# MachinaIO/mxx

Measured on AMD Instinct MI355X. Metric: dcrt_ring_ops_per_s, higher is better.
Workload: dtype u32

## Files before the change

include/gpupoly.h:

```cpp
#ifndef GPUPOLY_H
#define GPUPOLY_H

#include <stddef.h>
#include <stdint.h>

#ifdef __cplusplus
extern "C" {
#endif

typedef struct GpuContext GpuContext;
typedef struct GpuMatrix GpuMatrix;
typedef struct GpuEventSet GpuEventSet;
typedef struct GpuP1CovarianceCache GpuP1CovarianceCache;
typedef struct GpuComm GpuComm;

typedef struct GpuRngSeed {
    uint64_t words[4];
} GpuRngSeed;

#define GPU_POLY_FORMAT_COEFF 0
#define GPU_POLY_FORMAT_EVAL 1
#define GPU_MATRIX_DIST_UNIFORM 0
#define GPU_MATRIX_DIST_GAUSS 1
#define GPU_MATRIX_DIST_BIT 2
// ... 119 lines not shown
int gpupoly_matrix_decompose_rows(const GpuMatrix *src, uint32_t base_bits, int small, size_t row_start, GpuMatrix *out);
int gpupoly_matrix_sample_decomposed_window(GpuMatrix *out, int dist_type, double sigma, GpuRngSeed seed,
                                            uint32_t base_bits, int small, size_t src_rows, size_t full_ncol,
                                            size_t col_offset, size_t row_start);
int gpupoly_timer_start(GpuContext *ctx);
int gpupoly_timer_stop(GpuContext *ctx, float *out_ms);
int gpupoly_timer_mark(GpuContext *ctx, uint32_t slot);
int gpupoly_timer_elapsed(GpuContext *ctx, uint32_t slot_begin, uint32_t slot_end, float *out_ms);
int gpupoly_matrix_device_ptr(const GpuMatrix *mat, void **out_ptr, size_t *out_bytes);
int gpupoly_matrix_layout(const GpuMatrix *mat, int *out);
int gpupoly_matrix_copy_to_context(GpuContext *dst_ctx, const GpuMatrix *src, GpuMatrix **out);
int gpupoly_context_device(const GpuContext *ctx, int *out_device);
int gpupoly_context_word_bytes(const GpuContext *ctx, int *out_bytes);
const char *gpupoly_context_last_kernel(const GpuContext *ctx);
int gpupoly_context_stream(const GpuContext *ctx, void **out_stream);
int gpupoly_comm_create(GpuContext *const *ctxs, size_t n, GpuComm **out_comm);
void gpupoly_comm_destroy(GpuComm *comm);
int gpupoly_comm_size(const GpuComm *comm, int *out_size);
const char *gpupoly_comm_backend(const GpuComm *comm);
int gpupoly_matrix_all_gather_columns(GpuComm *comm, const GpuMatrix *const *local_blocks, GpuMatrix *const *full);
int gpupoly_matrix_sample_distribution_segments(GpuMatrix *out, int dist_type, double sigma, const GpuRngSeed *seeds,
                                                const size_t *seg_cols, size_t nseg);
int gpupoly_matrix_sample_p1_full_cached_segments(const GpuP1CovarianceCache *cache, const GpuMatrix *tp2,
                                                  const GpuRngSeed *seeds, const size_t *seg_cols, size_t nseg,
                                                  GpuMatrix *out);
int gpupoly_matrix_gauss_samp_gq_arb_base_segments(GpuMatrix *src, uint32_t base_bits, double c, double dgg_stddev,
                                                   const GpuRngSeed *seeds, const size_t *seg_cols, size_t nseg,
                                                   GpuMatrix *out);
#define GPUPOLY_BLOCKS_STACKED 0
#define GPUPOLY_BLOCKS_COLUMNS 1
int gpupoly_matrix_sample_distribution_blocks(GpuMatrix *out, int dist_type, const GpuRngSeed *seeds, size_t nblk,
                                              int layout, const size_t *seg_cols);
#define GPUPOLY_HASH_KECCAK256 0
#define GPUPOLY_HASH_SHA3_256 1
#define GPUPOLY_TAGS_TABLE 0
#define GPUPOLY_TAGS_INDEXED_LE64 1
#define GPUPOLY_TAGS_INDEXED_DECIMAL 2
typedef struct GpuHashTags {
    int hash;
    int form;
    uint8_t key[32];
    const uint8_t *tags;
    const size_t *tag_offsets;
    size_t prefix_len;
    uint64_t first_index;
} GpuHashTags;
int gpupoly_hash_seeds(GpuContext *ctx, const GpuHashTags *tags, size_t ntags, GpuRngSeed *seeds_out);
int gpupoly_matrix_sample_hash_blocks(GpuMatrix *out, int dist_type, const GpuHashTags *tags, size_t nblk, int layout,
                                      const size_t *seg_cols);
int gpupoly_matrix_sample_gauss_blocks(GpuMatrix *out, double sigma, const GpuRngSeed *seeds, size_t nblk, int layout,
                                       const size_t *seg_cols);
int gpupoly_matrix_sample_hash_gauss_blocks(GpuMatrix *out, double sigma, const GpuHashTags *tags, size_t nblk, int layout,
                                            const size_t *seg_cols);
int gpupoly_matrix_concat_columns(GpuMatrix *out, const GpuMatrix *const *blocks, size_t n);
int gpupoly_matrix_split_columns(const GpuMatrix *src, GpuMatrix *const *blocks, size_t n);
int gpupoly_trapdoor_preimage_many(const GpuMatrix *re, const GpuP1CovarianceCache *cache, const GpuMatrix *public_matrix,
                                   uint32_t base_bits, const GpuMatrix *const *targets, size_t n, const GpuRngSeed *seeds,
                                   GpuMatrix *const *outs);
int gpupoly_trapdoor_preimage_keyed(const GpuMatrix *const *res, const GpuP1CovarianceCache *const *caches,
                                    const GpuMatrix *const *public_matrices, size_t nkeys, uint32_t base_bits,
                                    const uint32_t *key_of, const GpuMatrix *const *targets, size_t n,
                                    const GpuRngSeed *seeds, GpuMatrix *const *outs);
int gpupoly_matrix_sample_decomposed_blocks(GpuMatrix *out, int dist_type, const GpuRngSeed *seeds, size_t nblk,
                                            uint32_t base_bits, int small, size_t src_rows, size_t full_ncol,
                                            size_t col_offset);
int gpupoly_matrix_sample_hash_decomposed_blocks(GpuMatrix *out, int dist_type, const GpuHashTags *tags, size_t nblk,
                                                 uint32_t base_bits, int small, size_t src_rows, size_t full_ncol,
                                                 size_t col_offset);
int gpupoly_matrix_lut_targets(GpuMatrix *const *outs, size_t nrows_T, const GpuMatrix *w_identity, const GpuMatrix *w_gy,
                               const GpuMatrix *w_v, const GpuMatrix *w_vx, size_t col_start, uint32_t base_bits,
                               const uint64_t *y_words, size_t words_per_y, const uint64_t *idx, const GpuHashTags *tags);
int gpupoly_matrix_lut_targets_combine(GpuMatrix *const *outs, size_t nrows_T, const GpuMatrix *w_identity,
                                       const GpuMatrix *w_gy, const GpuMatrix *product, size_t col_start, uint32_t base_bits,
                                       const uint64_t *y_words, size_t words_per_y, const uint64_t *idx);
int gpupoly_matrix_lwe_targets(GpuMatrix *const *outs, size_t nrows_T, const GpuMatrix *a_z, const GpuMatrix *a_lt,
                               size_t col_start, uint32_t base_bits, const uint64_t *y_words, size_t words_per_y,
                               const uint64_t *x, const GpuHashTags *tags);
int gpupoly_matrix_lwe_targets_combine(GpuMatrix *const *outs, size_t nrows_T, const GpuMatrix *a_lt,
                                       const GpuMatrix *digits, const GpuMatrix *product, size_t col_start,
                                       uint32_t base_bits, const uint64_t *y_words, size_t words_per_y, const uint64_t *x);
int gpupoly_matrix_wee25_targets(GpuMatrix *const *outs, size_t nblocks_T, size_t nparts_P, const GpuMatrix *t_bottom,
                                 size_t part_start, size_t secret_size, uint32_t base_bits, const uint64_t *idx,
                                 const GpuHashTags *tags);
int gpupoly_matrix_wee25_targets_product(GpuMatrix *const *outs, size_t nblocks_T, size_t nparts_P, const GpuMatrix *w_stacked,
                                         const GpuMatrix *t_bottom, size_t part_start, size_t secret_size,
                                         uint32_t base_bits, const uint64_t *idx);
int gpupoly_matrix_ggh15_lookup(GpuMatrix *const *outs, size_t nslots_S, const GpuMatrix *mid_identity,
                                const GpuMatrix *mid_gy, const GpuMatrix *mid_v, const GpuMatrix *mid_vx,
                                const GpuMatrix *mid_rand, const GpuMatrix *mid_gate1,
                                const GpuMatrix *const *lut_preimages, const GpuMatrix *const *xs, size_t col_start,
                                uint32_t base_bits, const uint64_t *y_words, size_t words_per_y, const GpuHashTags *tags);
int gpupoly_matrix_ggh15_lookup_combine(GpuMatrix *const *outs, size_t nslots_S, const GpuMatrix *mid_identity,
                                        const GpuMatrix *mid_gy, const GpuMatrix *mid_v, const GpuMatrix *mid_vx,
                                        const GpuMatrix *mid_rand, const GpuMatrix *mid_gate1,
                                        const GpuMatrix *const *lut_preimages, const GpuMatrix *const *xs, size_t col_start,
                                        uint32_t base_bits, const uint64_t *y_words, size_t words_per_y,
                                        const GpuMatrix *digits);
int gpupoly_matrix_lwe_lookup(GpuMatrix *const *outs, size_t nslots_S, size_t dst_col, const GpuMatrix *const *c_bs,
                              const GpuMatrix *const *k_highs, const GpuMatrix *const *c_zs, size_t col_start,
                              uint32_t base_bits, const GpuHashTags *tags);
int gpupoly_matrix_lwe_lookup_combine(GpuMatrix *const *outs, size_t nslots_S, size_t dst_col,
                                      const GpuMatrix *const *c_bs, const GpuMatrix *const *k_highs,
                                      const GpuMatrix *const *c_zs, size_t col_start, uint32_t base_bits,
                                      const GpuMatrix *digits);
typedef struct {
    const GpuMatrix *c_in;
    const GpuMatrix *mid;
    uint64_t shift;
    uint64_t scalar;
} GpuSlotTerm;
int gpupoly_matrix_slot_transfer_eval(GpuMatrix *const *outs, size_t nouts_S, size_t dst_col, const GpuMatrix *c_b0,
                                      const GpuMatrix *const *gate_preimages, const GpuMatrix *const *b1_preimages,
                                      const GpuSlotTerm *terms, const size_t *term_offsets, const uint64_t *mu_words,
                                      size_t words_per_mu, size_t col_start, uint32_t base_bits, const GpuHashTags *tags);
int gpupoly_matrix_slot_transfer_eval_combine(GpuMatrix *const *outs, size_t nouts_S, size_t dst_col, const GpuMatrix *c_b0,
                                              const GpuMatrix *const *gate_preimages,
                                              const GpuMatrix *const *b1_preimages, const GpuSlotTerm *terms,
                                              const size_t *term_offsets, const uint64_t *mu_words, size_t words_per_mu,
                                              size_t col_start, uint32_t base_bits, const GpuMatrix *digits);
int gpupoly_matrix_bgg_encode_slots(GpuMatrix *const *outs, size_t ninputs_P, const GpuMatrix *secrets,
                                    const GpuMatrix *const *pubkeys, const GpuMatrix *plaintexts, uint32_t base_bits,
                                    double sigma, const GpuRngSeed *seeds);
int gpupoly_matrix_bgg_encode_slots_combine(GpuMatrix *const *outs, size_t ninputs_P, const GpuMatrix *secrets,
                                            const GpuMatrix *const *pubkeys, const GpuMatrix *plaintexts,
                                            uint32_t base_bits, const GpuMatrix *errors);
int gpupoly_matrix_scale_round(GpuMatrix *out, const GpuMatrix *in, uint64_t t, int round_half);
int gpupoly_matrix_crt_recompose_rounded(GpuMatrix *out, const GpuMatrix *const *terms, const int *signs,
                                         size_t terms_per_level, size_t num_slots);
int gpupoly_matrix_nested_rns_decompose(GpuMatrix *out, const GpuMatrix *src, const uint64_t *p_moduli, size_t p_count,
                                        uint64_t scale, size_t level_offset, size_t active_levels, int out_format);
int gpupoly_matrix_fill_nested_rns_gadget(GpuMatrix *out, const uint64_t *p_moduli, size_t p_count, uint64_t scale,
                                          size_t level_offset, size_t active_levels, int out_format);
int gpupoly_matrix_nested_rns_residues(GpuMatrix *out, const GpuMatrix *src, const uint64_t *p_moduli, size_t p_count,
                                       size_t level_offset, size_t active_levels);
int gpupoly_matrix_store_coeff_words(const GpuMatrix *mat, uint64_t *out, size_t words_per_coeff);
int gpupoly_matrix_load_coeff_words(GpuMatrix *mat, const uint64_t *words, size_t words_per_coeff, size_t coeffs_per_poly,
                                    int out_format);
int gpupoly_matrix_centered_max_abs(const GpuMatrix *mat, uint64_t *out, size_t words_per_value);
int gpupoly_matrix_extract_bits(const GpuMatrix *mat, const uint64_t *lo, const uint64_t *hi, size_t words_per_bound,
                                uint8_t *out, size_t bytes_per_poly);
int gpupoly_matrix_store_coeff_ints(const GpuMatrix *mat, void *out, int elem_bytes, int centred, size_t coeffs_per_poly,
                                    uint64_t *out_misfit_count, uint64_t *out_first_misfit);
int gpupoly_matrix_store_compact_bytes_many(GpuMatrix *const *mats, size_t n, uint8_t *payload_out, size_t payload_capacity,
                                            uint16_t *out_max_coeff_bits, uint16_t *out_bytes_per_coeff,
                                            size_t *out_payload_offsets, size_t *out_payload_lens, size_t *out_total_len);
int gpupoly_matrix_load_compact_bytes_many(GpuMatrix *const *mats, size_t n, const uint8_t *const *payloads,
                                           const size_t *payload_lens, const uint16_t *max_coeff_bits);
int gpupoly_matrix_fill_monomial(GpuMatrix *out, uint64_t shift, int format);
int gpupoly_matrix_mul_monomial(GpuMatrix *out, const GpuMatrix *in, uint64_t shift);
int gpupoly_matrix_monomial_sum(GpuMatrix *out, const GpuMatrix *addend, const GpuMatrix *const *mats,
                                const uint64_t *shifts, size_t n, int negate);
int gpupoly_matrix_mul_sum(GpuMatrix *out, size_t dst_col, size_t cols, const GpuMatrix *addend,
                           const GpuMatrix *const *lhss, const GpuMatrix *const *rhss, size_t n, int negate);
int gpupoly_matrix_mul_acc(GpuMatrix *out, const GpuMatrix *lhs, const GpuMatrix *rhs, int negate);
int gpupoly_matrix_mul_gadget(GpuMatrix *out, size_t dst_col, const GpuMatrix *lhs, const GpuMatrix *scalar_1x1,
                              size_t gadget_col, size_t cols, const GpuMatrix *addend, int negate, uint32_t base_bits,
                              int small);
int gpupoly_matrix_gadget_mul(GpuMatrix *out, const GpuMatrix *rhs, const GpuMatrix *addend, int negate,
                              uint32_t base_bits, int small);
int gpupoly_matrix_mul_decompose_gadget_scalar_many(GpuMatrix *const *outs, const GpuMatrix *const *lhss,
                                                    const GpuMatrix *const *addends, size_t n, const GpuMatrix *scalar_1x1,
                                                    int negate, uint32_t base_bits);
int gpupoly_matrix_mul_decompose_gadget_const_many(GpuMatrix *const *outs, const GpuMatrix *const *lhss,
                                                   const GpuMatrix *const *addends, size_t n, const uint64_t *const_words,
                                                   size_t words_per_const, int negate, uint32_t base_bits);
uint64_t gpupoly_launch_count(void);
int gpupoly_detmath_eval(GpuContext *ctx, int fn, const double *host_in, double *host_out, size_t n);
int gpupoly_device_can_access_peer(int device, int peer, int *out_can);
int gpupoly_marker_launch(GpuContext *ctx, uint32_t id);
int gpupoly_trace_begin(void);
const char *gpupoly_trace_end(void);
const char *gpupoly_version(void);
int gpupoly_reload_env(void);

#ifdef __cplusplus
}
#endif
#endif
```

mxx_amd/_ffi.py:

```python
from __future__ import annotations

import ctypes as C
import os

_HERE = os.path.dirname(os.path.abspath(__file__))
LIB_PATH = os.environ.get("MXX_GPUPOLY_LIB") or os.path.join(_HERE, "libgpupoly.so")

GPU_POLY_FORMAT_COEFF = 0
GPU_POLY_FORMAT_EVAL = 1
GPU_MATRIX_DIST_UNIFORM = 0
GPU_MATRIX_DIST_GAUSS = 1
GPU_MATRIX_DIST_BIT = 2
GPU_MATRIX_DIST_TERNARY = 3
GPUPOLY_BLOCKS_STACKED = 0
GPUPOLY_BLOCKS_COLUMNS = 1
GPUPOLY_HASH_KECCAK256 = 0
GPUPOLY_HASH_SHA3_256 = 1
GPUPOLY_TAGS_TABLE = 0
GPUPOLY_TAGS_INDEXED_LE64 = 1
GPUPOLY_TAGS_INDEXED_DECIMAL = 2


class GpuPolyError(RuntimeError):
    """Raised where the reference's Rust wrapper panics (`check_status`, gpu.rs:259-263)."""
# ... 28 lines not shown


class GpuBatchOp(C.Structure):

    _fields_ = [("kind", C.c_int), ("out", C.c_void_p), ("lhs", C.c_void_p), ("rhs", C.c_void_p)]


GPUPOLY_OP_MUL, GPUPOLY_OP_ADD, GPUPOLY_OP_SUB, GPUPOLY_OP_MUL_SCALAR, GPUPOLY_OP_NEG, GPUPOLY_OP_DECOMPOSE, GPUPOLY_OP_MUL_DECOMPOSE = range(7)

_vp = C.c_void_p
_sz = C.c_size_t
_u8p = C.POINTER(C.c_uint8)

SIGNATURES = {
    "gpu_context_create": (C.c_int, [C.c_uint32, C.c_uint32, C.c_uint32, C.POINTER(C.c_uint64), _sz, C.POINTER(C.c_int), _sz, C.POINTER(_vp)]),
    "gpu_context_destroy": (None, [_vp]),
    "gpu_context_get_N": (C.c_int, [_vp, C.POINTER(C.c_int)]),
    "gpu_event_set_wait": (C.c_int, [_vp]),
    "gpu_event_set_destroy": (None, [_vp]),
    "gpu_device_count": (C.c_int, [C.POINTER(C.c_int)]),
    "gpu_device_mem_info": (C.c_int, [C.c_int, C.POINTER(_sz), C.POINTER(_sz)]),
    "gpu_device_synchronize": (C.c_int, []),
    "gpu_device_reset": (C.c_int, []),
    "gpu_last_error": (C.c_char_p, []),
    "gpu_set_last_error": (C.c_int, [C.c_char_p]),
    "gpu_pinned_alloc": (_vp, [_sz]),
    "gpu_pinned_free": (None, [_vp]),
    "gpu_matrix_create": (C.c_int, [_vp, C.c_int, _sz, _sz, C.c_int, C.POINTER(_vp)]),
    "gpu_matrix_destroy": (None, [_vp]),
    "gpu_matrix_copy": (C.c_int, [_vp, _vp]),
    "gpu_matrix_copy_block": (C.c_int, [_vp, _vp, _sz, _sz, _sz, _sz, _sz, _sz]),
    "gpu_matrix_add": (C.c_int, [_vp, _vp, _vp]),
    "gpu_matrix_sub": (C.c_int, [_vp, _vp, _vp]),
    "gpu_matrix_add_block": (C.c_int, [_vp, _vp, _sz, _sz, _sz, _sz, _sz, _sz]),
    "gpu_matrix_mul": (C.c_int, [_vp, _vp, _vp]),
    "gpu_matrix_mul_scalar": (C.c_int, [_vp, _vp, _vp]),
    "gpu_matrix_equal": (C.c_int, [_vp, _vp, C.POINTER(C.c_int)]),
    "gpu_matrix_ntt_all": (C.c_int, [_vp]),
    "gpu_matrix_intt_all": (C.c_int, [_vp]),
    "gpu_matrix_fill_gadget": (C.c_int, [_vp, C.c_uint32]),
    "gpu_matrix_fill_small_gadget": (C.c_int, [_vp, C.c_uint32]),
    "gpu_matrix_fill_small_decomposed_identity_chunk": (C.c_int, [_vp, _vp, _sz]),
    "gpu_matrix_decompose_base": (C.c_int, [_vp, C.c_uint32, _vp]),
    "gpu_matrix_decompose_base_small": (C.c_int, [_vp, C.c_uint32, _vp]),
    "gpu_matrix_sample_distribution": (C.c_int, [_vp, C.c_int, C.c_double, GpuRngSeed]),
    "gpu_matrix_sample_distribution_columns": (C.c_int, [_vp, C.c_int, C.c_double, GpuRngSeed, _sz, _sz]),
    "gpu_matrix_gauss_samp_gq_arb_base": (C.c_int, [_vp, C.c_uint32, C.c_double, C.c_double, GpuRngSeed, _vp]),
    "gpu_matrix_sample_p1_full": (C.c_int, [_vp, _vp, _vp, _vp, C.c_double, C.c_double, C.c_double, GpuRngSeed, _vp]),
    "gpu_matrix_create_p1_covariance_cache": (C.c_int, [_vp, _vp, _vp, C.c_double, C.c_double, C.c_double, C.POINTER(_vp)]),
    "gpu_matrix_destroy_p1_covariance_cache": (None, [_vp]),
    "gpu_matrix_sample_p1_full_cached": (C.c_int, [_vp, _vp, GpuRngSeed, _vp]),
    "gpu_matrix_load_rns_batch": (C.c_int, [_vp, _vp, _sz, C.c_int, C.POINTER(_vp)]),
    "gpu_matrix_store_rns_batch": (C.c_int, [_vp, _vp, _sz, C.c_int, C.POINTER(_vp)]),
    "gpu_matrix_store_const_coeff_batch": (C.c_int, [_vp, _vp, _sz, C.POINTER(_vp)]),
    "gpu_matrix_store_compact_bytes": (C.c_int, [_vp, _vp, _sz, C.POINTER(C.c_uint16), C.POINTER(C.c_uint16), C.POINTER(_sz)]),
    "gpu_matrix_load_compact_bytes": (C.c_int, [_vp, _vp, _sz, C.c_uint16]),
    "gpu_poly_store_compact_bytes": (C.c_int, [_vp, _vp, _sz, C.POINTER(C.c_uint16), C.POINTER(C.c_uint16), C.POINTER(_sz)]),
    "gpu_poly_load_compact_bytes": (C.c_int, [_vp, _vp, _sz, C.c_uint16]),
    "gpupoly_matrix_mul_decompose": (C.c_int, [_vp, _vp, _vp, C.c_uint32]),
    "gpupoly_matrix_mul_decompose_many": (C.c_int, [C.POINTER(C.c_void_p), C.POINTER(C.c_void_p), C.POINTER(C.c_void_p), C.POINTER(C.c_void_p), C.c_size_t, _vp, C.c_uint32]),
    "gpupoly_matrix_mul_decompose_pairs": (C.c_int, [C.POINTER(C.c_void_p), C.POINTER(C.c_void_p), C.POINTER(C.c_void_p), C.POINTER(C.c_void_p), C.POINTER(C.c_void_p), _sz, _sz, C.c_uint32, C.c_int]),
    "gpupoly_matrix_mul_batch":(C.c_int, [C.POINTER(C.c_void_p), C.POINTER(C.c_void_p), C.POINTER(C.c_void_p), C.c_size_t]),
    "gpupoly_batch": (C.c_int, [C.POINTER(GpuBatchOp), C.c_size_t, C.c_uint32]),
    "gpupoly_matrix_mul_decompose_small": (C.c_int, [_vp, _vp, _vp, C.c_uint32]),
    "gpupoly_matrix_mul_tensor_identity": (C.c_int, [_vp, _vp, _vp, C.c_size_t]),
    "gpupoly_matrix_mul_tensor_identity_decompose": (C.c_int, [_vp, _vp, _vp, C.c_size_t, C.c_uint32]),
    "gpupoly_matrix_mul_scalar_intt": (C.c_int, [_vp, _vp, _vp]),
    "gpupoly_matrix_transpose": (C.c_int, [_vp, _vp]),
    "gpupoly_matrix_tensor": (C.c_int, [_vp, _vp, _vp]),
    "gpupoly_matrix_add_rows": (C.c_int, [_vp, C.c_size_t, _vp, _vp]),
    "gpupoly_matrix_ntt_add_rows": (C.c_int, [_vp, C.c_size_t, _vp, _vp, C.c_int]),
    "gpupoly_matrix_row_view": (C.c_int, [_vp, C.c_size_t, C.c_size_t, C.POINTER(C.c_void_p)]),
    "gpupoly_matrix_reshape_view": (C.c_int, [_vp, C.c_size_t, C.c_size_t, C.POINTER(C.c_void_p)]),
    "gpupoly_matrix_neg": (C.c_int, [_vp, _vp]),
    "gpupoly_matrix_fill_zero": (C.c_int, [_vp]),
    "gpupoly_matrix_fill_identity": (C.c_int, [_vp, _vp]),
    "gpupoly_matrix_sample_decomposed": (C.c_int, [_vp, C.c_int, C.c_double, GpuRngSeed, C.c_uint32, C.c_int]),
    "gpupoly_matrix_decompose_rows": (C.c_int, [_vp, C.c_uint32, C.c_int, _sz, _vp]),
    "gpupoly_matrix_sample_decomposed_window": (C.c_int, [_vp, C.c_int, C.c_double, GpuRngSeed, C.c_uint32, C.c_int, _sz, _sz, _sz, _sz]),
    "gpupoly_timer_start": (C.c_int, [_vp]),
    "gpupoly_timer_stop": (C.c_int, [_vp, C.POINTER(C.c_float)]),
    "gpupoly_timer_mark": (C.c_int, [_vp, C.c_uint32]),
    "gpupoly_timer_elapsed": (C.c_int, [_vp, C.c_uint32, C.c_uint32, C.POINTER(C.c_float)]),
    "gpupoly_matrix_device_ptr": (C.c_int, [_vp, C.POINTER(_vp), C.POINTER(_sz)]),
    "gpupoly_matrix_layout": (C.c_int, [_vp, C.POINTER(C.c_int)]),
    "gpupoly_matrix_copy_to_context": (C.c_int, [_vp, _vp, C.POINTER(_vp)]),
    "gpupoly_context_device": (C.c_int, [_vp, C.POINTER(C.c_int)]),
    "gpupoly_context_word_bytes": (C.c_int, [_vp, C.POINTER(C.c_int)]),
    "gpupoly_context_last_kernel": (C.c_char_p, [_vp]),
    "gpupoly_context_stream": (C.c_int, [_vp, C.POINTER(C.c_void_p)]),
    "gpupoly_comm_create": (C.c_int, [C.POINTER(C.c_void_p), C.c_size_t, C.POINTER(_vp)]),
    "gpupoly_comm_destroy": (None, [_vp]),
    "gpupoly_comm_size": (C.c_int, [_vp, C.POINTER(C.c_int)]),
    "gpupoly_comm_backend": (C.c_char_p, [_vp]),
    "gpupoly_matrix_all_gather_columns": (C.c_int, [_vp, C.POINTER(C.c_void_p), C.POINTER(C.c_void_p)]),
    "gpupoly_matrix_sample_distribution_segments": (C.c_int, [_vp, C.c_int, C.c_double, C.POINTER(GpuRngSeed), C.POINTER(_sz), _sz]),
    "gpupoly_matrix_sample_distribution_blocks": (C.c_int, [_vp, C.c_int, C.POINTER(GpuRngSeed), _sz, C.c_int, C.POINTER(_sz)]),
    "gpupoly_hash_seeds": (C.c_int, [_vp, C.POINTER(GpuHashTags), _sz, C.POINTER(GpuRngSeed)]),
    "gpupoly_matrix_sample_hash_blocks": (C.c_int, [_vp, C.c_int, C.POINTER(GpuHashTags), _sz, C.c_int, C.POINTER(_sz)]),
    "gpupoly_matrix_sample_gauss_blocks": (C.c_int, [_vp, C.c_double, C.POINTER(GpuRngSeed), _sz, C.c_int, C.POINTER(_sz)]),
    "gpupoly_matrix_sample_hash_gauss_blocks": (C.c_int, [_vp, C.c_double, C.POINTER(GpuHashTags), _sz, C.c_int, C.POINTER(_sz)]),
    "gpupoly_matrix_sample_decomposed_blocks": (C.c_int, [_vp, C.c_int, C.POINTER(GpuRngSeed), _sz, C.c_uint32, C.c_int, _sz, _sz, _sz]),
    "gpupoly_matrix_sample_hash_decomposed_blocks": (C.c_int, [_vp, C.c_int, C.POINTER(GpuHashTags), _sz, C.c_uint32, C.c_int, _sz, _sz, _sz]),
    "gpupoly_matrix_lut_targets": (C.c_int, [C.POINTER(C.c_void_p), _sz, _vp, _vp, _vp, _vp, _sz, C.c_uint32, C.POINTER(C.c_uint64), _sz,
                                   C.POINTER(C.c_uint64), C.POINTER(GpuHashTags)]),
    "gpupoly_matrix_lut_targets_combine": (C.c_int, [C.POINTER(C.c_void_p), _sz, _vp, _vp, _vp, _sz, C.c_uint32, C.POINTER(C.c_uint64), _sz,
                                           C.POINTER(C.c_uint64)]),
    "gpupoly_matrix_lwe_targets": (C.c_int, [C.POINTER(C.c_void_p), _sz, _vp, _vp, _sz, C.c_uint32, C.POINTER(C.c_uint64), _sz,
                                   C.POINTER(C.c_uint64), C.POINTER(GpuHashTags)]),
    "gpupoly_matrix_lwe_targets_combine": (C.c_int, [C.POINTER(C.c_void_p), _sz, _vp, _vp, _vp, _sz, C.c_uint32, C.POINTER(C.c_uint64), _sz,
                                           C.POINTER(C.c_uint64)]),
    "gpupoly_matrix_wee25_targets": (C.c_int, [C.POINTER(C.c_void_p), _sz, _sz, _vp, _sz, _sz, C.c_uint32, C.POINTER(C.c_uint64),
                                     C.POINTER(GpuHashTags)]),
    "gpupoly_matrix_wee25_targets_product": (C.c_int, [C.POINTER(C.c_void_p), _sz, _sz, _vp, _vp, _sz, _sz, C.c_uint32,
                                             C.POINTER(C.c_uint64)]),
    "gpupoly_matrix_ggh15_lookup": (C.c_int, [C.POINTER(C.c_void_p), _sz, _vp, _vp, _vp, _vp, _vp, _vp, C.POINTER(C.c_void_p),
                                    C.POINTER(C.c_void_p), _sz, C.c_uint32, C.POINTER(C.c_uint64), _sz, C.POINTER(GpuHashTags)]),
    "gpupoly_matrix_ggh15_lookup_combine": (C.c_int, [C.POINTER(C.c_void_p), _sz, _vp, _vp, _vp, _vp, _vp, _vp, C.POINTER(C.c_void_p),
                                            C.POINTER(C.c_void_p), _sz, C.c_uint32, C.POINTER(C.c_uint64), _sz, _vp]),
    "gpupoly_matrix_lwe_lookup": (C.c_int, [C.POINTER(C.c_void_p), _sz, _sz, C.POINTER(C.c_void_p), C.POINTER(C.c_void_p), C.POINTER(C.c_void_p),
                                  _sz, C.c_uint32, C.POINTER(GpuHashTags)]),
    "gpupoly_matrix_lwe_lookup_combine": (C.c_int, [C.POINTER(C.c_void_p), _sz, _sz, C.POINTER(C.c_void_p), C.POINTER(C.c_void_p),
                                          C.POINTER(C.c_void_p), _sz, C.c_uint32, _vp]),
    "gpupoly_matrix_slot_transfer_eval": (C.c_int, [C.POINTER(C.c_void_p), _sz, _sz, _vp, C.POINTER(C.c_void_p), C.POINTER(C.c_void_p),
                                          C.POINTER(GpuSlotTerm), C.POINTER(_sz), C.POINTER(C.c_uint64), _sz, _sz, C.c_uint32,
                                          C.POINTER(GpuHashTags)]),
    "gpupoly_matrix_slot_transfer_eval_combine": (C.c_int, [C.POINTER(C.c_void_p), _sz, _sz, _vp, C.POINTER(C.c_void_p), C.POINTER(C.c_void_p),
                                                  C.POINTER(GpuSlotTerm), C.POINTER(_sz), C.POINTER(C.c_uint64), _sz, _sz, C.c_uint32, _vp]),
    "gpupoly_matrix_bgg_encode_slots": (C.c_int, [C.POINTER(C.c_void_p), _sz, _vp, C.POINTER(C.c_void_p), _vp, C.c_uint32, C.c_double,
                                        C.POINTER(GpuRngSeed)]),
    "gpupoly_matrix_bgg_encode_slots_combine": (C.c_int, [C.POINTER(C.c_void_p), _sz, _vp, C.POINTER(C.c_void_p), _vp, C.c_uint32, _vp]),
    "gpupoly_matrix_sample_p1_full_cached_segments":(C.c_int, [_vp, _vp, C.POINTER(GpuRngSeed), C.POINTER(_sz), _sz, _vp]),
    "gpupoly_matrix_gauss_samp_gq_arb_base_segments": (C.c_int, [_vp, C.c_uint32, C.c_double, C.c_double, C.POINTER(GpuRngSeed), C.POINTER(_sz), _sz, _vp]),
    "gpupoly_matrix_concat_columns": (C.c_int, [_vp, C.POINTER(C.c_void_p), _sz]),
    "gpupoly_matrix_split_columns": (C.c_int, [_vp, C.POINTER(C.c_void_p), _sz]),
    "gpupoly_trapdoor_preimage_many": (C.c_int, [_vp, _vp, _vp, C.c_uint32, C.POINTER(C.c_void_p), _sz, C.POINTER(GpuRngSeed), C.POINTER(C.c_void_p)]),
    "gpupoly_trapdoor_preimage_keyed": (C.c_int, [C.POINTER(C.c_void_p), C.POINTER(C.c_void_p), C.POINTER(C.c_void_p), _sz, C.c_uint32,
                                        C.POINTER(C.c_uint32), C.POINTER(C.c_void_p), _sz, C.POINTER(GpuRngSeed), C.POINTER(C.c_void_p)]),
    "gpupoly_launch_count": (C.c_uint64, []),
    "gpupoly_matrix_scale_round": (C.c_int, [_vp, _vp, C.c_uint64, C.c_int]),
    "gpupoly_matrix_crt_recompose_rounded": (C.c_int, [_vp, C.POINTER(C.c_void_p), C.POINTER(C.c_int), _sz, _sz]),
    "gpupoly_matrix_nested_rns_decompose": (C.c_int, [_vp, _vp, C.POINTER(C.c_uint64), _sz, C.c_uint64, _sz, _sz, C.c_int]),
    "gpupoly_matrix_fill_nested_rns_gadget": (C.c_int, [_vp, C.POINTER(C.c_uint64), _sz, C.c_uint64, _sz, _sz, C.c_int]),
    "gpupoly_matrix_nested_rns_residues": (C.c_int, [_vp, _vp, C.POINTER(C.c_uint64), _sz, _sz, _sz]),
    "gpupoly_matrix_store_coeff_words": (C.c_int, [_vp, C.POINTER(C.c_uint64), _sz]),
    "gpupoly_matrix_load_coeff_words": (C.c_int, [_vp, C.POINTER(C.c_uint64), _sz, _sz, C.c_int]),
    "gpupoly_matrix_centered_max_abs": (C.c_int, [_vp, C.POINTER(C.c_uint64), _sz]),
    "gpupoly_matrix_extract_bits": (C.c_int, [_vp, C.POINTER(C.c_uint64), C.POINTER(C.c_uint64), _sz, _u8p, _sz]),
    "gpupoly_matrix_store_coeff_ints": (C.c_int, [_vp, _vp, C.c_int, C.c_int, _sz, C.POINTER(C.c_uint64), C.POINTER(C.c_uint64)]),
    "gpupoly_matrix_fill_monomial": (C.c_int, [_vp, C.c_uint64, C.c_int]),
    "gpupoly_matrix_mul_monomial": (C.c_int, [_vp, _vp, C.c_uint64]),
    "gpupoly_matrix_monomial_sum": (C.c_int, [_vp, _vp, C.POINTER(C.c_void_p), C.POINTER(C.c_uint64), _sz, C.c_int]),
    "gpupoly_matrix_mul_sum": (C.c_int, [_vp, _sz, _sz, _vp, C.POINTER(C.c_void_p), C.POINTER(C.c_void_p), _sz, C.c_int]),
    "gpupoly_matrix_mul_acc": (C.c_int, [_vp, _vp, _vp, C.c_int]),
    "gpupoly_matrix_mul_gadget": (C.c_int, [_vp, _sz, _vp, _vp, _sz, _sz, _vp, C.c_int, C.c_uint32, C.c_int]),
    "gpupoly_matrix_gadget_mul": (C.c_int, [_vp, _vp, _vp, C.c_int, C.c_uint32, C.c_int]),
    "gpupoly_matrix_mul_decompose_gadget_scalar_many": (C.c_int, [C.POINTER(C.c_void_p), C.POINTER(C.c_void_p), C.POINTER(C.c_void_p), _sz, _vp, C.c_int, C.c_uint32]),
    "gpupoly_matrix_mul_decompose_gadget_const_many": (C.c_int, [C.POINTER(C.c_void_p), C.POINTER(C.c_void_p), C.POINTER(C.c_void_p), _sz, C.POINTER(C.c_uint64), _sz, C.c_int, C.c_uint32]),
    "gpupoly_matrix_store_compact_bytes_many": (C.c_int, [C.POINTER(C.c_void_p), _sz, _vp, _sz, C.POINTER(C.c_uint16), C.POINTER(C.c_uint16), C.POINTER(_sz), C.POINTER(_sz), C.POINTER(_sz)]),
    "gpupoly_matrix_load_compact_bytes_many": (C.c_int, [C.POINTER(C.c_void_p), _sz, C.POINTER(C.c_void_p), C.POINTER(_sz), C.POINTER(C.c_uint16)]),
    "gpupoly_detmath_eval": (C.c_int, [_vp, C.c_int, C.POINTER(C.c_double), C.POINTER(C.c_double), _sz]),
    "gpupoly_device_can_access_peer": (C.c_int, [C.c_int, C.c_int, C.POINTER(C.c_int)]),
    "gpupoly_marker_launch": (C.c_int, [_vp, C.c_uint32]),
    "gpupoly_trace_begin": (C.c_int, []),
    "gpupoly_trace_end": (C.c_char_p, []),
    "gpupoly_version": (C.c_char_p, []),
    "gpupoly_reload_env": (C.c_int, []),
}

_lib = None


def lib() -> C.CDLL:
    global _lib
    if _lib is None:
        if not os.path.exists(LIB_PATH):
            raise GpuPolyError(
                f"{LIB_PATH} is missing: build it with `python -c 'import __graft_entry__ as g; g.build()'` "
                "(or `make -C mxx_amd/csrc`). mxx_amd has no CPU fallback."
            )
        handle = C.CDLL(LIB_PATH)
        for name, (res, args) in SIGNATURES.items():
            fn = getattr(handle, name)
            fn.restype = res
            fn.argtypes = args
        _lib = handle
    return _lib


def last_error_string() -> str:
    msg = lib().gpu_last_error()
    return msg.decode("utf-8", "replace") if msg else "unknown GPU error"


def check_status(code: int, context: str) -> None:
    if code != 0:
        raise GpuPolyError(f"{context} failed: {last_error_string()}")


def reload_env() -> None:
    check_status(lib().gpupoly_reload_env(), "gpupoly_reload_env")


def trace_begin() -> None:
    check_status(lib().gpupoly_trace_begin(), "gpupoly_trace_begin")


def trace_end() -> list[dict]:
    text = lib().gpupoly_trace_end()
    if text is None:
        raise GpuPolyError(f"gpupoly_trace_end failed: {last_error_string()}")
    out = []
    for ln in text.decode().splitlines():
        name, blocks, threads, nbytes, ms = ln.split("\t")
        out.append({"kernel": name.strip("()"), "blocks": int(blocks), "threads": int(threads), "bytes": float(nbytes), "ms": float(ms)})
    return out


def gpu_device_sync() -> None:
    check_status(lib().gpu_device_synchronize(), "gpu_device_synchronize")


def detected_gpu_device_ids() -> list[int]:
    n = C.c_int(0)
    if lib().gpu_device_count(C.byref(n)) != 0 or n.value <= 0:
        return []
    return list(range(n.value))


def peer_access_matrix(devices=None) -> list[list[int]]:
    devs = detected_gpu_device_ids() if devices is None else list(devices)
    out = []
    for a in devs:
        row = []
        for b in devs:
            can = C.c_int(0)
            check_status(lib().gpupoly_device_can_access_peer(a, b, C.byref(can)), "gpupoly_device_can_access_peer")
            row.append(int(can.value))
        out.append(row)
    return out


def detected_gpu_device_count() -> int:
    return len(detected_gpu_device_ids())


def wait_and_destroy_events(events: _vp) -> None:
    if events:
        st = lib().gpu_event_set_wait(events)
        lib().gpu_event_set_destroy(events)
        check_status(st, "gpu_event_set_wait")
```

mxx_amd/csrc/common.h:

```cpp
#pragma once

#include <hip/hip_runtime.h>

#include <atomic>
#include <cstddef>
#include <cstdint>
#include <cstdio>
#include <exception>
#include <map>
#include <unordered_map>
#include <mutex>
#include <string>
#include <vector>

#include "../../include/gpupoly.h"
#include "grid_plan.h"

constexpr size_t GPUPOLY_MAX_LIMBS = 64;

struct LimbConst {
    uint64_t q;
    uint64_t mu;
    uint64_t mu64;
    uint64_t n_inv;
    uint64_t n_inv_sh;
    uint64_t mu32;
    uint64_t inv_last_w;
    uint64_t inv_last_w_sh;
    uint32_t kbits;
    uint32_t lazy_terms;
};

struct EnvSwitches {
    int ntt_path = 0;
    int ntt14 = 0;
    bool decompose_fused = true;
    char matmul_path = 0;
    int matmul_tile = 0;
    bool gsamp_simple = false;
    bool gsamp_no_uni = false;
    bool p1_simple = false;
    int sampler_per_lane = 0;
    int sampler_fill_every = 0;
    bool ntt64_int = false;
    int ntt_phase = 0;
    bool serde_general = false;
    bool rng_compat = false;
    bool pack24 = true;
    int skinny24 = 0;
    int skinny24_shape = 0;
    size_t mul_decompose_many_budget = 0;
    size_t mul_decompose_pairs_budget = 0;
    size_t gadget_scalar_budget = 0;
    size_t ggh15_lookup_budget = 0;
    size_t lwe_lookup_budget = 0;
    size_t slot_eval_budget = 0;
    size_t bgg_encode_budget = 0;
    char mul_sum_path = 0;
    size_t crt_recompose_chunk_bytes = size_t(256) << 20;
    void load();
};

struct GpuContext {
    EnvSwitches env;
    int device = 0;
    std::vector<int> gpu_ids;
    uint32_t logN = 0;
    int N = 0;
    int level = 0;
    uint32_t dnum = 0;
    int limb_count = 0;
    bool wide = false;
    int word_bytes = 4;
    uint32_t crt_bits = 0;
    std::vector<uint64_t> moduli;
    hipStream_t stream = nullptr;
    LimbConst *d_limbs = nullptr;
    LimbConst *d_limbs_r = nullptr;
    void *d_tw_fwd = nullptr;
    void *d_tw_fwd_sh = nullptr;
    void *d_tw_inv = nullptr;
    void *d_tw_inv_sh = nullptr;
    void *d_tw2_fwd = nullptr;
    void *d_tw2_inv = nullptr;
    bool lazy_ok = false;
    bool tight_ok = false;
    void *d_tw2s_inv = nullptr;
    bool signed_ok = false;
    void *d_twf_fwd = nullptr, *d_twf_inv = nullptr;
    void *d_flimbs = nullptr;
    bool f64_ok = false;
    uint64_t *d_garner = nullptr;
    std::vector<uint64_t> garner_inv;
    std::vector<LimbConst> limbs;
    hipEvent_t timer_start = nullptr, timer_stop = nullptr;
    std::vector<hipEvent_t> marks;
    std::mutex mutex;
    bool pool_ok = false;
    std::mutex alloc_mutex;
    std::multimap<size_t, void *> free_blocks;
    std::unordered_map<void *, size_t> live_blocks;
    size_t cached_bytes = 0, cache_limit = 0;
    std::atomic<const char *> last_kernel{""};
    bool pack24_ok = false;
    std::mutex layout_mutex;
    std::map<uint32_t, void *> gadget_weights;
    std::map<std::vector<uint64_t>, void *> gadget_const_tables;
    std::map<std::vector<uint64_t>, void *> nested_rns_tables;
};

struct LayoutTag {
    std::atomic<int> v{GPU_MATRIX_LAYOUT_WORDS};
    LayoutTag() = default;
    LayoutTag(const LayoutTag &o) : v(o.v.load(std::memory_order_acquire)) {}
    LayoutTag &operator=(const LayoutTag &o) {
        v.store(o.v.load(std::memory_order_acquire), std::memory_order_release);
        return *this;
    }
};

struct GpuMatrix {
    GpuContext *ctx = nullptr;
    int level = 0;
    size_t rows = 0, cols = 0;
    int format = GPU_POLY_FORMAT_EVAL;
    void *storage = nullptr;
    size_t bytes = 0;
    LayoutTag layout;
    bool borrowed = false;
    GpuMatrix *parent = nullptr;
    int views = 0;
};

struct GpuEventSet {
    std::vector<hipEvent_t> events;
    int device = 0;
    void *staging = nullptr;
    GpuContext *ctx = nullptr;
    void *dev_staging = nullptr;
};

struct GpuP1CovarianceCache {
    GpuContext *ctx = nullptr;
    int level = 0;
    size_t d = 0, m = 0, n = 0;
    double sigma = 0, s = 0, dgg_stddev = 0;
    double *sqrt_var = nullptr;
    double *update_coeff = nullptr;
    void *karney_div = nullptr;
};

struct P1KeyEntry {
    const double *sqrt_var;
    const double *update_coeff;
    const void *karney_div;
};

#if defined(__HIPCC__)
__device__ __forceinline__ size_t item_index() {
    return (static_cast<size_t>(blockIdx.y) * gridDim.x + blockIdx.x) * blockDim.x + threadIdx.x;
}
#endif

extern std::atomic<uint64_t> g_kernel_launches;
extern std::atomic<int> g_trace_on;
void trace_launch_begin(const char *name, hipStream_t stream, dim3 grid, dim3 block);
void trace_launch_end(hipStream_t stream);
void trace_set_bytes(double bytes);
#define MXX_TRACE_BYTES(b)                                                                        \
    do {                                                                                          \
        if (g_trace_on.load(std::memory_order_relaxed)) trace_set_bytes(static_cast<double>(b)); \
    } while (0)
#define MXX_LAUNCH(kern, grid, block, lds, strm, ...)                          \
    do {                                                                       \
        g_kernel_launches.fetch_add(1, std::memory_order_relaxed);             \
        const bool mxx_tr_ = g_trace_on.load(std::memory_order_relaxed) != 0;  \
        if (mxx_tr_) trace_launch_begin(#kern, strm, grid, block);             \
        hipLaunchKernelGGL(kern, grid, block, lds, strm, __VA_ARGS__);         \
        if (mxx_tr_) trace_launch_end(strm);                                   \
    } while (0)
#define MXX_TRACED_COPY(name, strm, bytes, stmt)                               \
    do {                                                                       \
        const bool mxx_tr_ = g_trace_on.load(std::memory_order_relaxed) != 0;  \
        if (mxx_tr_) {                                                         \
            trace_set_bytes(static_cast<double>(bytes));                       \
            trace_launch_begin(name, strm, dim3(0), dim3(0));                  \
        }                                                                      \
        stmt;                                                                  \
        if (mxx_tr_) trace_launch_end(strm);                                   \
    } while (0)

int set_error(const char *msg);
int set_error(const std::string &msg);
int set_error(hipError_t err, const char *what);

#define HIP_TRY(expr)                                          \
    do {                                                       \
        hipError_t _e = (expr);                                \
        if (_e != hipSuccess) return set_error(_e, #expr);     \
    } while (0)

template <auto... KERNELS>
static int lds_opt_in(const GpuContext *ctx, size_t lds) {
    static std::atomic<uint64_t> configured{0};
    const uint64_t bit = 1ull << (ctx->device & 63);
    if (lds <= 64 * 1024 || (configured.load() & bit)) return 0;
    for (const void *f : {reinterpret_cast<const void *>(KERNELS)...})
        HIP_TRY(hipFuncSetAttribute(f, hipFuncAttributeMaxDynamicSharedMemorySize, static_cast<int>(lds)));
    configured.fetch_or(bit);
    return 0;
}

extern int (*g_roctx_push)(const char *);
extern int (*g_roctx_pop)();
void roctx_init_once();
struct RoctxScope {
    bool on;
    explicit RoctxScope(const char *name) {
        roctx_init_once();
        on = g_roctx_push != nullptr;
        if (on) g_roctx_push(name);
    }
    ~RoctxScope() {
        if (on) g_roctx_pop();
    }
};

#define ABI_GUARD_BEGIN try { RoctxScope roctx_scope_(__func__);
#define ABI_GUARD_END                                                         \
    }                                                                         \
    catch (const std::exception &e) { return set_error(e.what()); }           \
    catch (...) { return set_error("unknown exception in libgpupoly"); }

inline size_t matrix_polys(const GpuMatrix *m) { return m->rows * m->cols; }
inline size_t matrix_limbs(const GpuMatrix *m) { return static_cast<size_t>(m->level) + 1; }
inline size_t matrix_words(const GpuMatrix *m) { return matrix_polys(m) * matrix_limbs(m) * static_cast<size_t>(m->ctx->N); }

void *words_ptr(const GpuMatrix *m);
const void *packed24_ptr(const GpuMatrix *m, bool *packed);
inline size_t packed24_bytes(const GpuMatrix *m) { return m->bytes / 4 * 3; }
inline bool storage_overlaps(const GpuMatrix *x, const GpuMatrix *y) {
    if (x == y) return true;
    if (!x->storage || !y->storage || x->bytes == 0 || y->bytes == 0) return false;
    const size_t xb = x->layout.v.load(std::memory_order_acquire) == GPU_MATRIX_LAYOUT_PACKED24 ? packed24_bytes(x) : x->bytes;
    const size_t yb = y->layout.v.load(std::memory_order_acquire) == GPU_MATRIX_LAYOUT_PACKED24 ? packed24_bytes(y) : y->bytes;
    const char *xs = static_cast<const char *>(x->storage), *ys = static_cast<const char *>(y->storage);
    return xs < ys + yb && ys < xs + xb;
}
inline bool same_block(const GpuMatrix *x, const GpuMatrix *y) {
    return x == y || (x->storage == y->storage && x->bytes == y->bytes);
}
inline bool partial_overlap(const GpuMatrix *out, const GpuMatrix *operand) {
    return storage_overlaps(out, operand) && !same_block(out, operand);
}
inline bool row_block_overlaps(const GpuMatrix *m, size_t row, size_t rows, const GpuMatrix *y) {
    if (m->layout.v.load(std::memory_order_acquire) == GPU_MATRIX_LAYOUT_PACKED24) return rows && m->cols && storage_overlaps(m, y);
    if (!m->storage) return false;
    const size_t poly_bytes = matrix_limbs(m) * static_cast<size_t>(m->ctx->N) * m->ctx->word_bytes;
    GpuMatrix block;
    block.storage = static_cast<char *>(m->storage) + row * m->cols * poly_bytes;
    block.bytes = rows * m->cols * poly_bytes;
// ... 69 lines not shown
```

mxx_amd/csrc/matmul_sum.hip:

```cpp
#include "matmul_tile.h"

#include <algorithm>
#include <string>
#include <vector>

struct MulSumItem {
    const void *a;
    const void *b;
    uint32_t k;
    uint32_t pad;
};
constexpr size_t kMulSumMax = 64;
struct MulSumArgs {
    MulSumItem item[kMulSumMax];
};
static_assert(sizeof(MulSumArgs) <= 4096 - 128, "descriptor table must fit the kernel-argument segment");

template <typename W, int TR, int TC, int SV, bool NTB>
__global__ void __launch_bounds__(256)
    matmul_sum_kernel(MulSumArgs args, uint32_t terms, W *out, const W *addend, const LimbConst *__restrict__ limbs, uint32_t rows,
                      uint32_t cols, uint32_t out_cols, uint32_t dst_col, uint32_t L, uint32_t N, uint32_t row_tiles, int negate) {
    const uint32_t limb = blockIdx.z;
    const uint32_t ct = blockIdx.y / row_tiles, rt = blockIdx.y - ct * row_tiles;
    const uint32_t r0 = rt * TR, c0 = ct * TC;
    const uint32_t i = (blockIdx.x * blockDim.x + threadIdx.x) * SV;
    if (i >= N) return;
    const LimbConst lc = limbs[limb];
    const W q = static_cast<W>(lc.q);
    typedef typename TileTypes<W, SV>::VT VT;
    typedef typename TileTypes<W, SV>::wxs wxs;
    typedef typename TileTypes<W, SV>::D D;

    const size_t poly = static_cast<size_t>(L) * N;
    const size_t in_poly = static_cast<size_t>(limb) * N + i;
    uint32_t row[TR];
#pragma unroll
    for (int r = 0; r < TR; ++r) row[r] = min(r0 + r, rows - 1);
    size_t b_off[TC];
#pragma unroll
    for (int c = 0; c < TC; ++c) b_off[c] = static_cast<size_t>(min(c0 + c, cols - 1)) * poly + in_poly;
    const size_t strideBk = static_cast<size_t>(cols) * poly;

    D acc[TR][TC][SV];
    MXX_TILE_CLEAR(acc);
    const uint32_t lazy = lc.lazy_terms;
    uint32_t pending = 0;
    for (uint32_t t = 0; t < terms; ++t) {
        const MulSumItem it = args.item[t];
        const W *A = static_cast<const W *>(it.a), *B = static_cast<const W *>(it.b);
        const uint32_t inner = it.k;
        size_t a_off[TR];
#pragma unroll
        for (int r = 0; r < TR; ++r) a_off[r] = static_cast<size_t>(row[r]) * inner * poly + in_poly;
#define MXX_TILE_A(r, k) (A + a_off[r] + (k) * poly)
#define MXX_TILE_B(c, k) (B + b_off[c] + (k) * strideBk)
#include "matmul_tile_loop.inc"
    }
#pragma unroll
    for (int r = 0; r < TR; ++r) {
        if (r0 + r >= rows) continue;
#pragma unroll
        for (int c = 0; c < TC; ++c) {
            if (c0 + c >= cols) continue;
            const size_t off = (static_cast<size_t>(r0 + r) * out_cols + dst_col + c0 + c) * poly + in_poly;
            W o[SV];
#pragma unroll
            for (int s = 0; s < SV; ++s) {
                o[s] = tile_reduce<W>(acc[r][c][s], q, lc);
                if (negate) o[s] = o[s] ? static_cast<W>(q - o[s]) : static_cast<W>(0);
            }
            if (addend) {
                W ad[SV];
                *reinterpret_cast<VT *>(ad) = *reinterpret_cast<const VT *>(addend + off);
#pragma unroll
                for (int s = 0; s < SV; ++s) o[s] = add_mod<W>(ad[s], o[s], q);
            }
            *reinterpret_cast<VT *>(out + off) = *reinterpret_cast<const VT *>(o);
        }
    }
}

template <typename W, int VN>
__global__ void __launch_bounds__(256)
    mul_sum_combine_kernel(W *out, const W *src, const W *__restrict__ prod, const LimbConst *__restrict__ limbs, size_t vecs, uint32_t cols,
                           uint32_t out_cols, uint32_t dst_col, uint32_t L, uint32_t N, int negate) {
    const size_t v = item_index();
    if (v >= vecs) return;
    typedef typename std::conditional<sizeof(W) * VN == 16, uint4, W>::type VT;
    static_assert(sizeof(VT) == sizeof(W) * VN, "vector width");
    const size_t per_limb = N / VN, per_poly = per_limb * L;
    const size_t p = v / per_poly, rem = v - p * per_poly;
    const uint32_t limb = static_cast<uint32_t>(rem / per_limb);
    const size_t r = p / cols, c = p - r * cols;
    const size_t off = ((r * out_cols + dst_col + c) * per_poly + rem) * VN;
    const W q = static_cast<W>(limbs[limb].q);
    W x[VN], o[VN];
    *reinterpret_cast<VT *>(x) = *reinterpret_cast<const VT *>(prod + v * VN);
    if (src) *reinterpret_cast<VT *>(o) = *reinterpret_cast<const VT *>(src + off);
#pragma unroll
    for (int s = 0; s < VN; ++s) {
        if (negate) x[s] = x[s] ? static_cast<W>(q - x[s]) : static_cast<W>(0);
        o[s] = src ? add_mod<W>(o[s], x[s], q) : x[s];
    }
    *reinterpret_cast<VT *>(out + off) = *reinterpret_cast<const VT *>(o);
}

namespace {

struct SumBlock {
    uint32_t rows, cols, out_cols, dst_col, L;
};

template <typename W, int TR, int TC, int SV>
int launch_sum_cfg(GpuContext *ctx, const MulSumArgs &args, uint32_t terms, size_t b_bytes, void *out, const void *addend,
                   const SumBlock &blk, int negate) {
    const uint32_t N = static_cast<uint32_t>(ctx->N);
    const TileGrid g = tile_grid<TR, TC, SV>(ctx, blk.rows, blk.cols, blk.L, b_bytes);
    W *o = static_cast<W *>(out);
    const W *ad = static_cast<const W *>(addend);
    bool streamed = false;
    if constexpr (sizeof(W) == 4) {
        if (g.streamed) {
            streamed = true;
            MXX_LAUNCH((matmul_sum_kernel<W, TR, TC, SV, true>), g.grid, dim3(g.threads), 0, ctx->stream, args, terms, o, ad, ctx->d_limbs,
                       blk.rows, blk.cols, blk.out_cols, blk.dst_col, blk.L, N, g.row_tiles, negate);
        }
    }
    if (!streamed)
        MXX_LAUNCH((matmul_sum_kernel<W, TR, TC, SV, false>), g.grid, dim3(g.threads), 0, ctx->stream, args, terms, o, ad, ctx->d_limbs,
                   blk.rows, blk.cols, blk.out_cols, blk.dst_col, blk.L, N, g.row_tiles, negate);
    HIP_TRY(hipGetLastError());
    return 0;
}

int launch_sum(GpuContext *ctx, const MulSumArgs &args, uint32_t terms, size_t b_bytes, void *out, const void *addend, const SumBlock &blk,
               int negate) {
    return dispatch_stacked_tile(ctx, stacked_tile(ctx, blk.rows, blk.cols, blk.L), [&](auto cfg) {
        typedef decltype(cfg) T;
        return launch_sum_cfg<typename T::W, T::TR, T::TC, T::SV>(ctx, args, terms, b_bytes, out, addend, blk, negate);
    });
}

template <typename W>
int launch_combine(GpuContext *ctx, void *out, const void *src, const void *prod, const SumBlock &blk, int negate) {
    const uint32_t N = static_cast<uint32_t>(ctx->N);
    constexpr int VN = 16 / sizeof(W);
    const size_t words = static_cast<size_t>(blk.rows) * blk.cols * blk.L * N;
    MXX_TRACE_BYTES(static_cast<double>(words) * sizeof(W) * (src ? 3 : 2));
    if (N >= static_cast<uint32_t>(VN))
        MXX_LAUNCH((mul_sum_combine_kernel<W, VN>), item_grid(words / VN, 256), dim3(256), 0, ctx->stream, static_cast<W *>(out),
                   static_cast<const W *>(src), static_cast<const W *>(prod), ctx->d_limbs, words / VN, blk.cols, blk.out_cols, blk.dst_col, blk.L,
                   N, negate);
    else
        MXX_LAUNCH((mul_sum_combine_kernel<W, 1>), item_grid(words, 256), dim3(256), 0, ctx->stream, static_cast<W *>(out),
                   static_cast<const W *>(src), static_cast<const W *>(prod), ctx->d_limbs, words, blk.cols, blk.out_cols, blk.dst_col, blk.L, N,
                   negate);
    HIP_TRY(hipGetLastError());
    return 0;
}

int mul_sum_impl(const char *who, GpuMatrix *out, size_t dst_col, size_t cols, const GpuMatrix *addend, const GpuMatrix *const *lhss,
                 const GpuMatrix *const *rhss, size_t n, int negate) {
    auto refuse = [&](const std::string &what) { return set_error(std::string(who) + ": " + what); };
    if (!out) return refuse("null output");
    if (n > 0 && (!lhss || !rhss)) return refuse("null array");
    for (size_t t = 0; t < n; ++t)
        if (!lhss[t] || !rhss[t]) return refuse("null matrix (term " + std::to_string(t) + ")");
    GpuContext *ctx = out->ctx;
    const int level = out->level;
    auto same_ring = [&](const GpuMatrix *m, const std::string &at) -> int {
        if (m->ctx != ctx) return refuse("context mismatch" + at);
        if (m->level != level) return refuse("level mismatch" + at);
        return 0;
    };
    if (addend && same_ring(addend, " (addend)")) return 1;
    for (size_t t = 0; t < n; ++t) {
        const std::string at = " (term " + std::to_string(t) + ")";
        if (same_ring(lhss[t], at) || same_ring(rhss[t], at)) return 1;
    }
    if (dst_col > out->cols || cols > out->cols - dst_col) return refuse("column block out of range");
    for (size_t t = 0; t < n; ++t)
        if (lhss[t]->cols != rhss[t]->rows || lhss[t]->rows != out->rows || rhss[t]->cols != cols)
            return refuse("shape mismatch (term " + std::to_string(t) + ")");
    if (addend && (addend->rows != out->rows || addend->cols != out->cols)) return refuse("addend shape mismatch");
    if (addend && addend->format != GPU_POLY_FORMAT_EVAL) return refuse("requires Eval format (addend)");
    for (size_t t = 0; t < n; ++t)
        if (lhss[t]->format != GPU_POLY_FORMAT_EVAL || rhss[t]->format != GPU_POLY_FORMAT_EVAL)
            return refuse("requires Eval format (term " + std::to_string(t) + ")");
    const bool whole = dst_col == 0 && cols == out->cols;
    if (!whole && out->format != GPU_POLY_FORMAT_EVAL) return refuse("a partial column block needs an output already in Eval format");
    if (addend && partial_overlap(out, addend)) return refuse("the addend overlaps the output without being the same block");
    for (size_t t = 0; t < n; ++t)
        if (storage_overlaps(out, lhss[t]) || storage_overlaps(out, rhss[t]))
            return refuse("the output overlaps an operand (term " + std::to_string(t) + ")");
    const size_t L = matrix_limbs(out);
    bool any_inner = false;
    for (size_t t = 0; t < n; ++t) {
        if (lhss[t]->cols > 0xffffffffull) return refuse("matrix too large");
        any_inner = any_inner || lhss[t]->cols > 0;
    }
    if (out->rows > 0xffffffffull || out->cols > 0xffffffffull) return refuse("matrix too large");
    if (out->rows && cols) {
        const TileShape tl = stacked_tile(ctx, out->rows, cols, L);
        if (!tile_grid_fits(out->rows, cols, tl.tr, tl.tc)) return refuse("matrix too large");
    }
    out->format = GPU_POLY_FORMAT_EVAL;
    if (out->rows == 0 || cols == 0) return 0;
    if (ctx_activate(ctx)) return 1;
    void *const o = words_ptr(out);
    const void *src = addend ? words_ptr(addend) : nullptr;
    std::vector<const void *> a(n), b(n);
    for (size_t t = 0; t < n; ++t) {
        a[t] = words_ptr(lhss[t]);
        b[t] = words_ptr(rhss[t]);
    }
    if (n == 0 && src == o) return 0;
    const SumBlock blk{static_cast<uint32_t>(out->rows), static_cast<uint32_t>(cols), static_cast<uint32_t>(out->cols), static_cast<uint32_t>(dst_col),
                       static_cast<uint32_t>(L)};
    const double block_bytes = static_cast<double>(out->rows) * cols * L * ctx->N * ctx->word_bytes;

    if (out->rows > 8 && any_inner && ctx->env.mul_sum_path != 't') {
        GpuMatrix *tmp = nullptr;
        int rc = gpu_matrix_create(ctx, level, out->rows, cols, GPU_POLY_FORMAT_EVAL, &tmp);
        for (size_t t = 0; !rc && t < n; ++t) {
            if (lhss[t]->cols == 0) continue;
            rc = gpu_matrix_mul(tmp, lhss[t], rhss[t]);
            if (!rc) rc = ctx->wide ? launch_combine<uint64_t>(ctx, o, src, words_ptr(tmp), blk, negate)
                                    : launch_combine<uint32_t>(ctx, o, src, words_ptr(tmp), blk, negate);
            src = o;
        }
        gpu_matrix_destroy(tmp);
        return rc;
    }
    size_t t0 = 0;
    do {
        MulSumArgs args = {};
        const uint32_t terms = static_cast<uint32_t>(std::min(kMulSumMax, n - t0));
        double bytes = block_bytes * (src ? 2 : 1);
        size_t b_bytes = 0;
        for (uint32_t t = 0; t < terms; ++t) {
            args.item[t].a = a[t0 + t];
            args.item[t].b = b[t0 + t];
            args.item[t].k = static_cast<uint32_t>(lhss[t0 + t]->cols);
            bytes += static_cast<double>(lhss[t0 + t]->bytes) + static_cast<double>(rhss[t0 + t]->bytes);
            b_bytes += rhss[t0 + t]->bytes;
        }
        MXX_TRACE_BYTES(bytes);
        const int rc = launch_sum(ctx, args, terms, b_bytes, o, src, blk, negate);
        if (rc) return rc;
        src = o;
        t0 += terms;
    } while (t0 < n);
    return 0;
}

}

extern "C" int gpupoly_matrix_mul_sum(GpuMatrix *out, size_t dst_col, size_t cols, const GpuMatrix *addend, const GpuMatrix *const *lhss,
                                      const GpuMatrix *const *rhss, size_t n, int negate) {
    ABI_GUARD_BEGIN
    return mul_sum_impl("gpupoly_matrix_mul_sum", out, dst_col, cols, addend, lhss, rhss, n, negate);
    ABI_GUARD_END
}

extern "C" int gpupoly_matrix_mul_acc(GpuMatrix *out, const GpuMatrix *lhs, const GpuMatrix *rhs, int negate) {
    ABI_GUARD_BEGIN
    if (!out || !lhs || !rhs) return set_error("gpupoly_matrix_mul_acc: null matrix");
    return mul_sum_impl("gpupoly_matrix_mul_acc", out, 0, out->cols, out, &lhs, &rhs, 1, negate);
    ABI_GUARD_END
}
```

mxx_amd/csrc/runtime.hip:

```cpp
#include "common.h"

#include <algorithm>
#include <cstdlib>
#include <iterator>
#include <map>
#include <cstring>
#include <dlfcn.h>

typedef unsigned __int128 u128h;

static thread_local std::string g_last_error;

int set_error(const char *msg) {
    g_last_error = msg ? msg : "unknown error";
    return 1;
}
int set_error(const std::string &msg) {
    g_last_error = msg;
    return 1;
}
int set_error(hipError_t err, const char *what) {
    g_last_error = std::string(what ? what : "hip call") + ": " + hipGetErrorString(err);
    (void)hipGetLastError();
    return 1;
// ... 311 lines not shown
        *out = it->second;
        ctx->live_blocks[*out] = it->first;
        ctx->cached_bytes -= it->first;
        ctx->free_blocks.erase(it);
        return 0;
    }
    hipError_t e = hipMalloc(out, want);
    if (e != hipSuccess) {
        (void)hipGetLastError();
        cache_trim(ctx, 0);
        e = hipMalloc(out, want);
    }
    if (e != hipSuccess) {
        (void)hipGetLastError();
        {
            std::lock_guard<std::mutex> reg(g_registry_mutex);
            for (GpuContext *other : g_contexts) {
                if (other == ctx || other->device != ctx->device) continue;
                if (!other->alloc_mutex.try_lock()) continue;
                cache_trim(other, 0);
                other->alloc_mutex.unlock();
            }
        }
        e = hipMalloc(out, want);
        if (e != hipSuccess) {
            *out = nullptr;
            return set_error(e, "hipMalloc");
        }
    }
    ctx->live_blocks[*out] = want;
    return 0;
}

void ctx_free(GpuContext *ctx, void *ptr) {
    if (!ptr) return;
    std::lock_guard<std::mutex> lk(ctx->alloc_mutex);
    auto it = ctx->live_blocks.find(ptr);
    if (it == ctx->live_blocks.end()) {
        (void)hipFree(ptr);
        return;
    }
    const size_t size = it->second;
    ctx->live_blocks.erase(it);
    if (!ctx->pool_ok) {
        (void)hipFree(ptr);
        return;
    }
    ctx->free_blocks.emplace(size, ptr);
    ctx->cached_bytes += size;
    cache_trim(ctx, ctx->cache_limit);
}

template <typename W>
static int upload_tables(GpuContext *ctx, const std::vector<std::vector<uint64_t>> &fwd,
                         const std::vector<std::vector<uint64_t>> &inv) {
    const size_t N = ctx->N, L = ctx->limb_count;
    const unsigned shift = sizeof(W) * 8;
    std::vector<W> h_f(L * N), h_fs(L * N), h_i(L * N), h_is(L * N);
    for (size_t l = 0; l < L; ++l) {
        uint64_t q = ctx->moduli[l];
        for (size_t j = 0; j < N; ++j) {
            h_f[l * N + j] = (W)fwd[l][j];
            h_fs[l * N + j] = (W)(((u128h)fwd[l][j] << shift) / q);
            h_i[l * N + j] = (W)inv[l][j];
            h_is[l * N + j] = (W)(((u128h)inv[l][j] << shift) / q);
        }
    }
    size_t bytes = L * N * sizeof(W);
    HIP_TRY(hipMalloc(&ctx->d_tw_fwd, bytes));
    HIP_TRY(hipMalloc(&ctx->d_tw_fwd_sh, bytes));
    HIP_TRY(hipMalloc(&ctx->d_tw_inv, bytes));
    HIP_TRY(hipMalloc(&ctx->d_tw_inv_sh, bytes));
    HIP_TRY(hipMemcpy(ctx->d_tw_fwd, h_f.data(), bytes, hipMemcpyHostToDevice));
    HIP_TRY(hipMemcpy(ctx->d_tw_fwd_sh, h_fs.data(), bytes, hipMemcpyHostToDevice));
    HIP_TRY(hipMemcpy(ctx->d_tw_inv, h_i.data(), bytes, hipMemcpyHostToDevice));
    HIP_TRY(hipMemcpy(ctx->d_tw_inv_sh, h_is.data(), bytes, hipMemcpyHostToDevice));
    std::vector<W> h_pf(2 * L * N), h_pi(2 * L * N);
    for (size_t i = 0; i < L * N; ++i) {
        h_pf[2 * i] = static_cast<W>(0) - h_f[i];
        h_pf[2 * i + 1] = h_fs[i];
        h_pi[2 * i] = h_i[i];
        h_pi[2 * i + 1] = h_is[i];
    }
    HIP_TRY(hipMalloc(&ctx->d_tw2_fwd, 2 * bytes));
    HIP_TRY(hipMalloc(&ctx->d_tw2_inv, 2 * bytes));
    HIP_TRY(hipMemcpy(ctx->d_tw2_fwd, h_pf.data(), 2 * bytes, hipMemcpyHostToDevice));
    HIP_TRY(hipMemcpy(ctx->d_tw2_inv, h_pi.data(), 2 * bytes, hipMemcpyHostToDevice));
    if (sizeof(W) == 8 && ctx->crt_bits <= 51 && N >= 2) {
        struct HostTwF { double w, wi; };
        struct HostF64Limb { double q, qinv; HostTwF n_inv, last_w; };
        std::vector<HostTwF> tf(L * N), ti(L * N);
        std::vector<HostF64Limb> fl(L);
        for (size_t l = 0; l < L; ++l) {
            const double qd = static_cast<double>(ctx->moduli[l]);
            for (size_t j = 0; j < N; ++j) {
                tf[l * N + j] = {static_cast<double>(fwd[l][j]), static_cast<double>(fwd[l][j]) / qd};
                ti[l * N + j] = {static_cast<double>(inv[l][j]), static_cast<double>(inv[l][j]) / qd};
            }
            const LimbConst &lc = ctx->limbs[l];
            fl[l] = {qd, 1.0 / qd, {static_cast<double>(lc.n_inv), static_cast<double>(lc.n_inv) / qd},
                     {static_cast<double>(lc.inv_last_w), static_cast<double>(lc.inv_last_w) / qd}};
        }
        HIP_TRY(hipMalloc(&ctx->d_twf_fwd, sizeof(HostTwF) * L * N));
        HIP_TRY(hipMalloc(&ctx->d_twf_inv, sizeof(HostTwF) * L * N));
        HIP_TRY(hipMalloc(&ctx->d_flimbs, sizeof(HostF64Limb) * L));
        HIP_TRY(hipMemcpy(ctx->d_twf_fwd, tf.data(), sizeof(HostTwF) * L * N, hipMemcpyHostToDevice));
        HIP_TRY(hipMemcpy(ctx->d_twf_inv, ti.data(), sizeof(HostTwF) * L * N, hipMemcpyHostToDevice));
        HIP_TRY(hipMemcpy(ctx->d_flimbs, fl.data(), sizeof(HostF64Limb) * L, hipMemcpyHostToDevice));
        ctx->f64_ok = true;
    }
    if (ctx->signed_ok && sizeof(W) == 4) {
        auto signed_pair = [](uint64_t w, uint64_t q, W *dst) {
            const int64_t c = w > q / 2 ? static_cast<int64_t>(w) - static_cast<int64_t>(q) : static_cast<int64_t>(w);
            __int128 num = static_cast<__int128>(c) << 32;
            __int128 fl = num / static_cast<__int128>(q);
            if (num % static_cast<__int128>(q) < 0) fl -= 1;
            dst[0] = static_cast<W>(static_cast<uint32_t>(static_cast<int32_t>(c)));
            dst[1] = static_cast<W>(static_cast<uint32_t>(static_cast<int32_t>(fl)));
        };
        for (size_t l = 0; l < L; ++l)
            for (size_t j = 0; j < N; ++j) signed_pair(inv[l][j], ctx->moduli[l], &h_pi[2 * (l * N + j)]);
        HIP_TRY(hipMalloc(&ctx->d_tw2s_inv, 2 * bytes));
        HIP_TRY(hipMemcpy(ctx->d_tw2s_inv, h_pi.data(), 2 * bytes, hipMemcpyHostToDevice));
    }
    return 0;
}

static void context_release(GpuContext *ctx) {
    if (!ctx) return;
    {
        std::lock_guard<std::mutex> reg(g_registry_mutex);
        g_contexts.erase(std::remove(g_contexts.begin(), g_contexts.end(), ctx), g_contexts.end());
    }
    (void)hipSetDevice(ctx->device);
    if (ctx->stream) (void)hipStreamSynchronize(ctx->stream);
    for (auto &kv : ctx->free_blocks) (void)hipFree(kv.second);
    for (auto &kv : ctx->live_blocks) (void)hipFree(kv.first);
    if (ctx->d_limbs) (void)hipFree(ctx->d_limbs);
    if (ctx->d_limbs_r) (void)hipFree(ctx->d_limbs_r);
    if (ctx->d_twf_fwd) (void)hipFree(ctx->d_twf_fwd);
    if (ctx->d_twf_inv) (void)hipFree(ctx->d_twf_inv);
    if (ctx->d_flimbs) (void)hipFree(ctx->d_flimbs);
    if (ctx->d_tw_fwd) (void)hipFree(ctx->d_tw_fwd);
    if (ctx->d_tw_fwd_sh) (void)hipFree(ctx->d_tw_fwd_sh);
    if (ctx->d_tw_inv) (void)hipFree(ctx->d_tw_inv);
    if (ctx->d_tw_inv_sh) (void)hipFree(ctx->d_tw_inv_sh);
    if (ctx->d_garner) (void)hipFree(ctx->d_garner);
    if (ctx->d_tw2_fwd) (void)hipFree(ctx->d_tw2_fwd);
    if (ctx->d_tw2_inv) (void)hipFree(ctx->d_tw2_inv);
    if (ctx->d_tw2s_inv) (void)hipFree(ctx->d_tw2s_inv);
    for (auto &kv : ctx->gadget_weights) (void)hipFree(kv.second);
    for (auto &kv : ctx->gadget_const_tables) (void)hipFree(kv.second);
    for (auto &kv : ctx->nested_rns_tables) (void)hipFree(kv.second);
    if (ctx->timer_start) (void)hipEventDestroy(ctx->timer_start);
    if (ctx->timer_stop) (void)hipEventDestroy(ctx->timer_stop);
    for (hipEvent_t ev : ctx->marks)
        if (ev) (void)hipEventDestroy(ev);
    if (ctx->stream) (void)hipStreamDestroy(ctx->stream);
    delete ctx;
}

extern "C" int gpu_context_create(uint32_t logN, uint32_t L, uint32_t dnum, const uint64_t *moduli,
                                  size_t moduli_len, const int *gpu_ids, size_t gpu_ids_len, GpuContext **out_ctx) {
    ABI_GUARD_BEGIN
    if (!out_ctx) return set_error("gpu_context_create: null out_ctx");
    *out_ctx = nullptr;
    if (!moduli || moduli_len == 0) return set_error("gpu_context_create: empty moduli");
    if (moduli_len != static_cast<size_t>(L) + 1) return set_error("gpu_context_create: moduli_len must equal L+1");
    if (moduli_len > GPUPOLY_MAX_LIMBS) return set_error("gpu_context_create: too many limbs");
    if (!gpu_ids || gpu_ids_len == 0) return set_error("gpu_context_create: empty gpu_ids");
    if (logN < 1 || logN > 17) return set_error("gpu_context_create: logN out of range [1,17]");
    int dev_count = 0;
    HIP_TRY(hipGetDeviceCount(&dev_count));
    for (size_t i = 0; i < gpu_ids_len; ++i) {
        if (gpu_ids[i] < 0 || gpu_ids[i] >= dev_count) return set_error("gpu_context_create: invalid gpu id");
        for (size_t j = 0; j < i; ++j)
            if (gpu_ids[j] == gpu_ids[i]) return set_error("gpu_context_create: duplicate gpu id");
    }
    const uint64_t N = 1ull << logN;
    bool wide = false;
    for (size_t i = 0; i < moduli_len; ++i) {
        uint64_t q = moduli[i];
        if (q < 3 || (q - 1) % (2 * N) != 0) return set_error("gpu_context_create: modulus must be = 1 (mod 2N)");
        if (!h_is_prime(q)) return set_error("gpu_context_create: modulus is not prime");
        if (q >> 62) return set_error("gpu_context_create: modulus must be < 2^62");
        if (q >> 31) wide = true;
        for (size_t j = 0; j < i; ++j)
            if (moduli[j] == q) return set_error("gpu_context_create: duplicate modulus");
    }

    GpuContext *ctx = new GpuContext();
    ctx->device = gpu_ids[0];
    ctx->gpu_ids.assign(gpu_ids, gpu_ids + gpu_ids_len);
    ctx->logN = logN;
    ctx->N = static_cast<int>(N);
    ctx->level = static_cast<int>(L);
    ctx->dnum = dnum;
    ctx->limb_count = static_cast<int>(moduli_len);
    ctx->wide = wide;
    ctx->word_bytes = wide ? 8 : 4;
    ctx->moduli.assign(moduli, moduli + moduli_len);

    hipError_t e = hipSetDevice(ctx->device);
    if (e != hipSuccess) { delete ctx; return set_error(e, "hipSetDevice"); }
    e = hipStreamCreateWithFlags(&ctx->stream, hipStreamNonBlocking);
    if (e != hipSuccess) { delete ctx; return set_error(e, "hipStreamCreate"); }

    ctx->env.load();
    {
        ctx->pool_ok = true;
        size_t free_b = 0, total_b = 0;
        ctx->cache_limit = size_t(64) << 30;
        if (hipMemGetInfo(&free_b, &total_b) == hipSuccess && free_b) ctx->cache_limit = free_b / 2;
        else (void)hipGetLastError();
        const char *env = std::getenv("MXX_HIP_MEMPOOL_RELEASE_THRESHOLD_BYTES");
        if (!env) env = std::getenv("MXX_CUDA_MEMPOOL_RELEASE_THRESHOLD_BYTES");
        if (env && *env) ctx->cache_limit = std::strtoull(env, nullptr, 10);
        const char *nopool = std::getenv("MXX_HIP_DISABLE_MEMPOOL");
        if (nopool && *nopool == '1') ctx->pool_ok = false;
    }

    std::vector<std::vector<uint64_t>> fwd(moduli_len), inv(moduli_len);
    ctx->limbs.resize(moduli_len);
    uint32_t crt_bits = 0;
    for (size_t l = 0; l < moduli_len; ++l) {
        uint64_t q = moduli[l];
        uint64_t psi = h_min_primitive_root(q, 2 * N);
        uint64_t ipsi = h_invmod_prime(psi, q);
        fwd[l].resize(N);
        inv[l].resize(N);
        uint64_t p = 1, ip = 1;
        for (uint64_t i = 0; i < N; ++i) {
            uint32_t r = h_bitrev(static_cast<uint32_t>(i), logN);
            fwd[l][r] = p;
            inv[l][r] = ip;
            p = h_mulmod(p, psi, q);
            ip = h_mulmod(ip, ipsi, q);
        }
        LimbConst &lc = ctx->limbs[l];
        lc.q = q;
        lc.kbits = h_bits(q);
        crt_bits = std::max(crt_bits, lc.kbits);
        lc.mu = static_cast<uint64_t>((((u128h)1) << (2 * lc.kbits)) / q);
        lc.mu64 = static_cast<uint64_t>((((u128h)1) << 64) / q);
        lc.n_inv = h_invmod_prime(N % q, q);
        lc.n_inv_sh = static_cast<uint64_t>(((u128h)lc.n_inv << (wide ? 64 : 32)) / q);
        lc.mu32 = (((uint64_t)1) << 32) / q;
        lc.inv_last_w = h_mulmod(inv[l][1 % N], lc.n_inv, q);
        lc.inv_last_w_sh = static_cast<uint64_t>(((u128h)lc.inv_last_w << (wide ? 64 : 32)) / q);
        if (!wide) {
            u128h q2 = (u128h)(q - 1) * (q - 1);
            u128h terms = ((((u128h)1) << 64) - q) / q2;
            lc.lazy_terms = terms > (1u << 20) ? (1u << 20) : static_cast<uint32_t>(terms);
        } else {
            u128h q2 = (u128h)(q - 1) * (q - 1);
            u128h terms = (~(u128h)0 - q) / q2;
            lc.lazy_terms = terms > (1u << 20) ? (1u << 20) : static_cast<uint32_t>(terms);
        }
    }
    ctx->crt_bits = crt_bits;
    ctx->lazy_ok = crt_bits + 7 <= (wide ? 64u : 32u);
    ctx->tight_ok = !wide && !ctx->lazy_ok && crt_bits + 4 <= 32u;
    ctx->signed_ok = !wide && crt_bits <= 24;
    ctx->pack24_ok = !wide && crt_bits <= 24 && ctx->N % 4 == 0;

    ctx->garner_inv.assign(moduli_len * moduli_len, 0);
    for (size_t i = 0; i < moduli_len; ++i)
        for (size_t j = 0; j < i; ++j)
            ctx->garner_inv[i * moduli_len + j] = h_invmod_prime(moduli[j] % moduli[i], moduli[i]);

    int rc = 0;
    e = hipMalloc(&ctx->d_limbs, sizeof(LimbConst) * moduli_len);
    if (e == hipSuccess)
        e = hipMemcpy(ctx->d_limbs, ctx->limbs.data(), sizeof(LimbConst) * moduli_len, hipMemcpyHostToDevice);
    if (e == hipSuccess) e = hipMalloc(&ctx->d_garner, sizeof(uint64_t) * moduli_len * moduli_len);
    if (e == hipSuccess)
        e = hipMemcpy(ctx->d_garner, ctx->garner_inv.data(), sizeof(uint64_t) * moduli_len * moduli_len,
                      hipMemcpyHostToDevice);
    if (e == hipSuccess && !wide) {
        std::vector<LimbConst> lr = ctx->limbs;
        for (LimbConst &c : lr) {
            const uint64_t r = (1ull << 32) % c.q;
            c.n_inv = h_mulmod(c.n_inv, r, c.q);
            c.n_inv_sh = static_cast<uint64_t>(((u128h)c.n_inv << 32) / c.q);
            c.inv_last_w = h_mulmod(c.inv_last_w, r, c.q);
            c.inv_last_w_sh = static_cast<uint64_t>(((u128h)c.inv_last_w << 32) / c.q);
        }
        e = hipMalloc(&ctx->d_limbs_r, sizeof(LimbConst) * moduli_len);
        if (e == hipSuccess) e = hipMemcpy(ctx->d_limbs_r, lr.data(), sizeof(LimbConst) * moduli_len, hipMemcpyHostToDevice);
    }
    if (e != hipSuccess) rc = set_error(e, "context constant upload");
    if (!rc) rc = wide ? upload_tables<uint64_t>(ctx, fwd, inv) : upload_tables<uint32_t>(ctx, fwd, inv);
    if (!rc) {
        e = hipEventCreate(&ctx->timer_start);
        if (e == hipSuccess) e = hipEventCreate(&ctx->timer_stop);
        if (e != hipSuccess) rc = set_error(e, "hipEventCreate");
    }
    if (rc) {
        std::string keep = g_last_error;
        context_release(ctx);
        g_last_error = keep;
        return rc;
    }
    {
        std::lock_guard<std::mutex> reg(g_registry_mutex);
        g_contexts.push_back(ctx);
// ... 180 lines not shown
```

mxx_amd/csrc/trapdoor.hip:

```cpp
#include "common.h"
#include "modarith.h"
#include "rng.h"

#include <algorithm>
#include <cstdlib>

static constexpr uint64_t kTagGadget = 0x6761646765746731ull;
static constexpr uint64_t kTagP1 = 0x7065727475726231ull;
static constexpr int kGaussMaxDigits = 64;

__host__ __device__ __forceinline__ uint64_t gadget_stream0(uint32_t i, uint32_t t) {
    return ((static_cast<uint64_t>(i) + 1) << 8) | (static_cast<uint64_t>(t) + 1);
}

template <typename W, int MAXD>
__global__ void __launch_bounds__(128) gauss_samp_gq_kernel(W *__restrict__ out, const W *__restrict__ src,
                                     const LimbConst *__restrict__ limbs, size_t src_polys, uint32_t src_cols,
                                     uint32_t L, uint32_t N, uint32_t dpt, uint32_t base_bits, double c, size_t k,
                                     GpuRngSeed seed) {
    __shared__ uint32_t ring[128 * RNG_RING_SLOTS];
    const size_t idx = item_index();
    const size_t total = src_polys * L * N;
    if (idx >= total) return;
    const uint32_t i = static_cast<uint32_t>(idx % N);
    const size_t pt = idx / N;
    const uint32_t t = static_cast<uint32_t>(pt % L);
    const size_t p = pt / L;
    const uint64_t qt = limbs[t].q;
    uint64_t value = static_cast<uint64_t>(src[(p * L + t) * N + i]) % qt;

    const uint64_t base = 1ull << base_bits;
    const double base_f = static_cast<double>(base);
    const double sigma = c / (base_f + 1.0);
    const double kf = static_cast<double>(dpt);

    int64_t m_digits[MAXD], v_digits[MAXD], z[MAXD];
    double a[MAXD], zf[MAXD], cvec[MAXD];
    {
        uint64_t mq = qt, vv = value;
#pragma unroll
        for (int d = 0; d < MAXD; ++d) {
            if (d < (int)dpt) {
                m_digits[d] = static_cast<int64_t>(mq % base);
                mq /= base;
                v_digits[d] = static_cast<int64_t>(vv % base);
                vv /= base;
            } else {
                m_digits[d] = 0;
                v_digits[d] = 0;
            }
        }
    }
    ChaChaRng rng;
    rng_init(rng, ring, seed, gadget_stream0(i, t), static_cast<uint64_t>(p) + 1, 0, kTagGadget);
#pragma unroll
    for (int d = 0; d < MAXD; ++d) {
        if ((d & 3) == 0) rng_fill_lane(rng);
        zf[d] = d < (int)dpt ? sigma * rng_standard_normal(rng) : 0.0;
    }

    {
        double prev_c = 0.0;
#pragma unroll
        for (int d = 0; d < MAXD; ++d) {
            if (d < (int)dpt) {
                cvec[d] = (prev_c + static_cast<double>(m_digits[d])) / base_f;
                prev_c = cvec[d];
            } else {
                cvec[d] = 0.0;
            }
        }
        double prev_a = 0.0;
#pragma unroll
        for (int d = 0; d < MAXD; ++d) {
            if (d < (int)dpt) {
                const double ld = d == 0 ? sqrt(base_f * (1.0 + 1.0 / kf) + 1.0)
                                         : sqrt(base_f * (1.0 + 1.0 / (kf - static_cast<double>(d))));
                double pd;
                if (d + 1 < (int)dpt) {
                    const double hn = sqrt(base_f * (1.0 - 1.0 / (kf - static_cast<double>(d))));
                    pd = ld * zf[d] + hn * zf[d + 1 < MAXD ? d + 1 : d];
                } else {
                    const double hd = d == 0 ? 0.0 : sqrt(base_f * (1.0 - 1.0 / (kf - static_cast<double>(d - 1))));
                    pd = hd * zf[d];
                }
                a[d] = (prev_a + static_cast<double>(v_digits[d]) - pd) / base_f;
                prev_a = a[d];
            } else {
                a[d] = 0.0;
            }
        }
    }
    const int last = static_cast<int>(dpt) - 1;
    double a_last = 0.0, c_last = 1.0;
#pragma unroll
    for (int d = 0; d < MAXD; ++d)
        if (d == last) {
            a_last = a[d];
            c_last = cvec[d];
        }
    const int64_t z_last = sample_integer_karney(rng, -a_last / c_last, sigma / c_last);
#pragma unroll
    for (int d = 0; d < MAXD; ++d) a[d] += static_cast<double>(z_last) * cvec[d];
#pragma unroll
    for (int d = 0; d < MAXD; ++d) {
        if (d < last) z[d] = sample_integer_karney(rng, -a[d], sigma);
        else z[d] = z_last;
    }

    const size_t r = p / src_cols, col = p - r * src_cols;
    int64_t z_prev = 0;
#pragma unroll
    for (int d = 0; d < MAXD; ++d) {
        if (d < (int)dpt) {
            int64_t digit;
            if (dpt == 1) digit = static_cast<int64_t>(base) * z[0] + m_digits[0] * z[0] + v_digits[0];
            else if (d == 0) digit = static_cast<int64_t>(base) * z[0] + m_digits[0] * z_last + v_digits[0];
            else if (d < last) digit = static_cast<int64_t>(base) * z[d] - z_prev + m_digits[d] * z_last + v_digits[d];
            else digit = m_digits[d] * z_last - z_prev + v_digits[d];
            z_prev = z[d];
            const size_t orow = r * k + static_cast<size_t>(t) * dpt + d;
            const size_t opoly = orow * src_cols + col;
            for (uint32_t l = 0; l < L; ++l)
                out[(opoly * L + l) * N + i] = signed_to_residue_mu<W>(digit, limbs[l].q, limbs[l].mu64);
        }
    }
}

struct GqTower {
    double c_last, sd;
    KarneyDivisor div;
    double cvec[4];
};

__global__ void gq_tower_kernel(GqTower *__restrict__ towers, const LimbConst *__restrict__ limbs, uint32_t L,
                                uint32_t dpt, uint32_t base_bits, double c) {
    const uint32_t t = blockIdx.x * blockDim.x + threadIdx.x;
    if (t >= L) return;
    const uint64_t base = 1ull << base_bits;
    const double base_f = static_cast<double>(base);
    const double sigma = c / (base_f + 1.0);
    const uint64_t qt = limbs[t].q;
    double c_last = 0.0;
    GqTower g;
    for (uint32_t d = 0; d < 4; ++d) g.cvec[d] = 0.0;
    for (uint32_t d = 0; d < dpt; ++d) {
        c_last = (c_last + static_cast<double>(static_cast<int64_t>((qt >> (base_bits * d)) & (base - 1)))) / base_f;
        if (d < 4) g.cvec[d] = c_last;
    }
    g.c_last = c_last;
    g.sd = sigma / c_last;
    g.div = karney_divisor(g.sd);
    towers[t] = g;
}

struct GqPertConsts {
    double ld[4], hn[4];
};

static inline GqPertConsts gq_pert_consts(uint32_t dpt, uint32_t base_bits) {
    GqPertConsts k{};
    const double base_f = static_cast<double>(1ull << base_bits), kf = static_cast<double>(dpt);
    for (uint32_t d = 0; d < 4 && d < dpt; ++d) {
        k.ld[d] = d == 0 ? sqrt(base_f * (1.0 + 1.0 / kf) + 1.0) : sqrt(base_f * (1.0 + 1.0 / (kf - static_cast<double>(d))));
        k.hn[d] = sqrt(base_f * (1.0 - 1.0 / (kf - static_cast<double>(d))));
    }
    return k;
}

template <typename W, int MAXD, bool SEG = false>
__global__ void __launch_bounds__(256) gauss_samp_prep_kernel(double *__restrict__ a_out, uint64_t *__restrict__ left_out,
                                       const W *__restrict__ src, const LimbConst *__restrict__ limbs,
                                       ChaChaKey key, size_t total, uint32_t L, uint32_t logN,
                                       uint32_t dpt, uint32_t base_bits, double c, GqPertConsts pc,
                                       uint32_t src_cols, SegArg<SEG> segs) {
    static_assert(MAXD <= 4, "GqPertConsts holds four digits");
    const size_t idx = item_index();
    if (idx >= total) return;
    const uint32_t i = static_cast<uint32_t>(idx & ((1u << logN) - 1));
    const uint32_t pt = static_cast<uint32_t>(idx >> logN);
    uint32_t p = pt / L;
    const uint32_t t = pt - p * L;
    if constexpr (SEG) {
        const uint32_t p_u = static_cast<uint32_t>(__builtin_amdgcn_readfirstlane(p));
        const uint32_t row = p_u / src_cols, col = p_u - row * src_cols;
        const uint32_t j = rng_segment_of(segs, col);
        key = segs.key[j];
        p = row * (segs.start[j + 1] - segs.start[j]) + (col - segs.start[j]);
    }
    const uint64_t qt = limbs[t].q;
    uint64_t value = static_cast<uint64_t>(src[idx]);
    if (value >= qt) value %= qt;
    const uint64_t base = 1ull << base_bits;
    const double base_f = static_cast<double>(base);
    const double sigma = c / (base_f + 1.0);

    uint64_t w[8];
    chacha_block_words(key, gadget_stream0(i, t), static_cast<uint64_t>(p) + 1, 0, w);
    double zf[MAXD];
#pragma unroll
    for (int d = 0; d < MAXD; ++d)
        zf[d] = d < (int)dpt ? sigma * (sqrt(-2.0 * det_log(u64_to_open01(w[2 * d]))) * det_cos2pi(u64_to_open01(w[2 * d + 1]))) : 0.0;
#pragma unroll
    for (int j = 0; j < 8; ++j)
        if (j >= 2 * (int)dpt) left_out[static_cast<size_t>(j - 2 * (int)dpt) * total + idx] = w[j];
    double prev_a = 0.0;
#pragma unroll
    for (int d = 0; d < MAXD; ++d) {
        if (d < (int)dpt) {
            double pd;
            if (d + 1 < (int)dpt) pd = pc.ld[d] * zf[d] + pc.hn[d] * zf[d + 1 < MAXD ? d + 1 : d];
            else pd = (d == 0 ? 0.0 : pc.hn[d - 1 < 0 ? 0 : d - 1]) * zf[d];
            const double vd = static_cast<double>(static_cast<int64_t>((value >> (base_bits * d)) & (base - 1)));
            const double ad = (prev_a + vd - pd) / base_f;
            prev_a = ad;
            a_out[static_cast<size_t>(d) * total + idx] = ad;
        }
    }
}

template <typename W, int MAXD, int SV, bool UNI = false, bool SEG = false>
__global__ void __launch_bounds__(SAMPLER_THREADS, 4) gauss_samp_lanes_kernel(int64_t *__restrict__ stage,
                                        const LimbConst *__restrict__ limbs, ChaChaKey key,
                                        const GqTower *__restrict__ towers, const double *__restrict__ a_in,
                                        const uint64_t *__restrict__ left_in, size_t total, uint32_t src_cols,
                                        uint32_t L, uint32_t logN, uint32_t dpt, uint32_t base_bits, double c,
                                        KarneyDivisor div_sigma, uint32_t per_lane, uint32_t fill_every,
                                        SegArg<SEG> segs) {
    static_assert(!SEG || UNI, "segments need a wave's chunk inside one polynomial");
    __shared__ uint32_t ring[SAMPLER_THREADS * RNG_RING_SLOTS];
    const uint64_t base = 1ull << base_bits;
    const double base_f = static_cast<double>(base);
    const double sigma = c / (base_f + 1.0);
    const int last = static_cast<int>(dpt) - 1;
    const uint32_t nleft = 8 - 2 * dpt;
    WaveChunk chunk = wave_chunk(total, per_lane);
    const uint32_t pt_u = static_cast<uint32_t>(__builtin_amdgcn_readfirstlane(static_cast<uint32_t>(chunk.base >> logN)));
    uint32_t p_u = pt_u / L;
    const uint32_t t_u = pt_u - p_u * L;
    const GqTower tw_u = towers[UNI ? t_u : 0];
    if constexpr (SEG) {
        const uint32_t row = p_u / src_cols, col = p_u - row * src_cols;
        const uint32_t j = rng_segment_of(segs, col);
        key = segs.key[j];
        p_u = row * (segs.start[j + 1] - segs.start[j]) + (col - segs.start[j]);
    }

    ChaChaRng rng;
    rng_init_keyed(rng, ring, key, 0, 0, SAMPLER_THREADS);
    KarneyFsm f;
    karney_reset(f);
    bool fin = true, have = false;
    uint32_t ph = 0;
    size_t idx = 0;
    uint32_t tower = 0;
    double a[MAXD];
    int64_t z[MAXD];
    int64_t z_last = 0;
#pragma unroll
    for (int d = 0; d < MAXD; ++d) { a[d] = 0.0; z[d] = 0; }

    auto integer_ready = [&]() {
        if (f.st == KS_DONE && !fin) {
            if (ph == 0) {
                z_last = f.result;
                const double zl = static_cast<double>(z_last);
#pragma unroll
                for (int d = 0; d < MAXD; ++d)
                    if (d < (int)dpt) a[d] += zl * (UNI ? tw_u.cvec[d] : towers[tower].cvec[d]);
            } else {
#pragma unroll
                for (int d = 0; d < MAXD; ++d)
                    if (d == (int)ph - 1) z[d] = f.result;
            }
            ++ph;
            if (ph == dpt) {
                fin = true;
            } else {
                double an = 0.0;
#pragma unroll
                for (int d = 0; d < MAXD; ++d)
                    if (d == (int)ph - 1) an = a[d];
                karney_begin(f, -an, sigma, div_sigma);
            }
        }
    };
    auto element_done = [&]() {
        const bool take = f.st == KS_DONE && fin;
        if (take && have) {
#pragma unroll
            for (int d = 0; d < MAXD; ++d) {
                if (d < (int)dpt) {
                    stage[idx * dpt + d] = d < last ? z[d] : z_last;
                }
            }
        }
        const uint32_t e = wave_take(chunk, take);
        if (take) {
            have = e < chunk.len;
            if (have) {
                idx = chunk.base + e;
                const uint32_t i = static_cast<uint32_t>(idx & ((1u << logN) - 1));
                uint32_t p, t;
                if constexpr (UNI) {
                    p = p_u;
                    t = t_u;
                } else {
                    const uint32_t pt = static_cast<uint32_t>(idx >> logN);
                    p = pt / L;
                    t = pt - p * L;
                }
                tower = t;
                rng_reopen(rng, gadget_stream0(i, t), static_cast<uint64_t>(p) + 1, 1);
                const uint32_t slot0 = (rng.tail >> RNG_DRAW_LOG) & (RNG_RING_SLOTS - 1);
                for (uint32_t w = 0; w < nleft; ++w) {
                    const uint64_t lw = left_in[static_cast<size_t>(w) * total + idx];
                    rng.ring[(slot0 + 4 * dpt + 2 * w) * rng.ring_stride] = static_cast<uint32_t>(lw);
                    rng.ring[(slot0 + 4 * dpt + 2 * w + 1) * rng.ring_stride] = static_cast<uint32_t>(lw >> 32);
                }
                rng.head = rng.tail + 2 * RNG_U64_DRAWS * dpt;
                rng.tail += RNG_BLOCK_DRAWS;
                double a_last = 0.0;
#pragma unroll
                for (int d = 0; d < MAXD; ++d) {
                    if (d < (int)dpt) {
                        a[d] = a_in[static_cast<size_t>(d) * total + idx];
                        a_last = a[d];
                    }
                }
                ph = 0;
                fin = false;
                if constexpr (UNI) {
                    karney_begin(f, -a_last / tw_u.c_last, tw_u.sd, tw_u.div);
                } else {
                    const GqTower tw = towers[t];
                    karney_begin(f, -a_last / tw.c_last, tw.sd, tw.div);
                }
            } else {
                f.st = KS_IDLE;
            }
        }
    };
    for (uint32_t step = 0;; ++step) {
        integer_ready();
        element_done();
        if (__all(f.st == KS_IDLE)) break;
        rng_fill_wave(rng, f.st != KS_IDLE, step % fill_every == 0, 16, karney_urgent(SV));
        karney_heavy(f, rng);
#pragma unroll
        for (int s4 = 0; s4 < KARNEY_SUPERSTEP / SV; ++s4) karney_light(f, rng);
#pragma unroll
        for (int sv = 1; sv < SV; ++sv) {
            integer_ready();
            karney_heavy(f, rng);
#pragma unroll
            for (int s4 = 0; s4 < KARNEY_SUPERSTEP / SV; ++s4) karney_light(f, rng);
        }
    }
}

template <typename W>
__global__ void __launch_bounds__(256) gauss_samp_expand_kernel(W *__restrict__ out, const int64_t *__restrict__ stage,
                                         const W *__restrict__ src, const LimbConst *__restrict__ limbs, size_t total,
                                         uint32_t src_cols, uint32_t L, uint32_t logN, uint32_t dpt, uint32_t k,
                                         uint32_t base_bits) {
    const size_t idx = item_index();
    if (idx >= total) return;
    const uint32_t i = static_cast<uint32_t>(idx & ((1u << logN) - 1));
    const uint32_t pt = static_cast<uint32_t>(idx >> logN);
    const uint32_t p = pt / L, t = pt - p * L;
    const uint32_t r = p / src_cols, col = p - r * src_cols;
    const uint64_t qt = limbs[t].q, base = 1ull << base_bits;
    uint64_t value = static_cast<uint64_t>(src[idx]);
    if (value >= qt) value %= qt;
    const int last = static_cast<int>(dpt) - 1;
    const int64_t z_last = stage[idx * dpt + last];
    int64_t z_prev = 0;
    for (uint32_t d = 0; d < dpt; ++d) {
        const int64_t md = static_cast<int64_t>((qt >> (base_bits * d)) & (base - 1));
        const int64_t vd = static_cast<int64_t>((value >> (base_bits * d)) & (base - 1));
        const int64_t zd = stage[idx * dpt + d];
        int64_t digit;
        if (dpt == 1) digit = static_cast<int64_t>(base) * zd + md * zd + vd;
        else if (d == 0) digit = static_cast<int64_t>(base) * zd + md * z_last + vd;
        else if (static_cast<int>(d) < last) digit = static_cast<int64_t>(base) * zd - z_prev + md * z_last + vd;
        else digit = md * z_last - z_prev + vd;
        z_prev = zd;
        const size_t orow = static_cast<size_t>(r) * k + t * dpt + d;
        W *dst = out + (((orow * src_cols + col) * L) << logN) + i;
        for (uint32_t l = 0; l < L; ++l)
            dst[static_cast<size_t>(l) << logN] = signed_to_residue_mu<W>(digit, limbs[l].q, limbs[l].mu64);
    }
}

template <typename W, int MAXD>
static int launch_gauss_samp_lanes(GpuContext *ctx, W *out, const W *src, size_t total, uint32_t src_cols, uint32_t L,
                                   uint32_t dpt, uint32_t base_bits, double c, size_t k, GpuRngSeed seed,
                                   const RngSegments *segs = nullptr) {
    if ((total >> ctx->logN) >> 32 || k >> 32) return set_error("gpu_matrix_gauss_samp_gq_arb_base: matrix too large");
    CtxBlock stage(ctx), a_buf(ctx), towers(ctx);
    if (towers.alloc(static_cast<size_t>(L) * sizeof(GqTower)) || a_buf.alloc(total * 8 * sizeof(uint64_t)) ||
        stage.alloc(total * dpt * sizeof(int64_t)))
        return 1;
    double *a_words = static_cast<double *>(a_buf.ptr);
    uint64_t *left_words = static_cast<uint64_t *>(a_buf.ptr) + total * dpt;
    const ChaChaKey key = chacha_subkey(seed, 0, kTagGadget);
    MXX_LAUNCH(gq_tower_kernel, dim3(1), dim3(64), 0, ctx->stream, static_cast<GqTower *>(towers.ptr), ctx->d_limbs,
                       L, dpt, base_bits, c);
    MXX_TRACE_BYTES(static_cast<double>(total) * (sizeof(W) + 8.0 * (8 - dpt)));
    if (segs)
        MXX_LAUNCH((gauss_samp_prep_kernel<W, MAXD, true>), item_grid(total, 256), dim3(256), 0,
                           ctx->stream, a_words, left_words, src, ctx->d_limbs, key, total, L,
                           ctx->logN, dpt, base_bits, c, gq_pert_consts(dpt, base_bits), src_cols, *segs);
    else
        MXX_LAUNCH((gauss_samp_prep_kernel<W, MAXD>), item_grid(total, 256), dim3(256), 0,
                           ctx->stream, a_words, left_words, src, ctx->d_limbs, key, total, L,
                           ctx->logN, dpt, base_bits, c, gq_pert_consts(dpt, base_bits), src_cols, NoSegments{});
    const LanePlan plan = lane_plan(total, static_cast<size_t>(ctx->N),
                                    sampler_per_lane(total, reinterpret_cast<const void *>(gauss_samp_lanes_kernel<W, MAXD, KARNEY_SERVICES>), ctx->device, ctx->env.sampler_per_lane),
                                    segs != nullptr, ctx->env.sampler_fill_every, kCadenceGadget, !ctx->env.gsamp_no_uni);
    const double sigma = c / (static_cast<double>(1ull << base_bits) + 1.0);
    MXX_TRACE_BYTES(static_cast<double>(total) * (8.0 * (8 - dpt) + 8.0 * dpt));
    int64_t *digits = static_cast<int64_t *>(stage.ptr);
    const GqTower *d_towers = static_cast<const GqTower *>(towers.ptr);
    const KarneyDivisor div = karney_divisor(sigma);
    if (segs)
        MXX_LAUNCH_LANES(plan, ctx->stream, (gauss_samp_lanes_kernel<W, MAXD, 1, true, true>),
                         (gauss_samp_lanes_kernel<W, MAXD, KARNEY_SERVICES, true, true>), digits, ctx->d_limbs, key, d_towers, a_words,
                         left_words, total, src_cols, L, ctx->logN, dpt, base_bits, c, div, plan.per_lane, plan.fill_every, *segs);
    else
        MXX_LAUNCH_LANES_UNI(plan, ctx->stream, (gauss_samp_lanes_kernel<W, MAXD, 1, true>), (gauss_samp_lanes_kernel<W, MAXD, 1, false>),
                             (gauss_samp_lanes_kernel<W, MAXD, KARNEY_SERVICES, true>), (gauss_samp_lanes_kernel<W, MAXD, KARNEY_SERVICES, false>),
                             digits, ctx->d_limbs, key, d_towers, a_words, left_words, total, src_cols, L, ctx->logN, dpt, base_bits, c, div,
                             plan.per_lane, plan.fill_every, NoSegments{});
    MXX_TRACE_BYTES(static_cast<double>(total) * (8.0 * dpt + sizeof(W) + static_cast<double>(dpt) * L * sizeof(W)));
    MXX_LAUNCH(gauss_samp_expand_kernel<W>, item_grid(total, 256), dim3(256), 0,
                       ctx->stream, out, digits, src, ctx->d_limbs, total, src_cols, L, ctx->logN,
                       dpt, static_cast<uint32_t>(k), base_bits);
    const hipError_t err = hipGetLastError();
    HIP_TRY(err);
    return 0;
}

template <typename W>
static int launch_gauss_samp(GpuContext *ctx, W *out, const W *src, size_t polys, uint32_t src_cols, uint32_t L,
                             uint32_t dpt, uint32_t base_bits, double c, size_t k, GpuRngSeed seed,
                             const RngSegments *segs = nullptr) {
    const size_t total = polys * L * static_cast<size_t>(ctx->N);
    const bool simple = ctx->env.gsamp_simple && !segs;
    if (!simple && dpt <= 2) return launch_gauss_samp_lanes<W, 2>(ctx, out, src, total, src_cols, L, dpt, base_bits, c, k, seed, segs);
    if (!simple && dpt <= 4) return launch_gauss_samp_lanes<W, 4>(ctx, out, src, total, src_cols, L, dpt, base_bits, c, k, seed, segs);
    if (segs) return set_error("gpupoly_matrix_gauss_samp_gq_arb_base_segments: unsupported: more than four digits per tower");
    const dim3 blocks = item_grid(total, 128);
    const uint32_t N = static_cast<uint32_t>(ctx->N);
    MXX_TRACE_BYTES(static_cast<double>(total) * (sizeof(W) + static_cast<double>(dpt) * L * sizeof(W)));
#define LAUNCH_GS(MAXD)                                                                                        \
    MXX_LAUNCH((gauss_samp_gq_kernel<W, MAXD>), dim3(blocks), dim3(128), 0, ctx->stream, out, src,      \
                       ctx->d_limbs, polys, src_cols, L, N, dpt, base_bits, c, k, seed)
    if (dpt <= 2) LAUNCH_GS(2);
    else if (dpt <= 4) LAUNCH_GS(4);
    else if (dpt <= 8) LAUNCH_GS(8);
    else if (dpt <= 20) LAUNCH_GS(20);
    else LAUNCH_GS(64);
#undef LAUNCH_GS
    HIP_TRY(hipGetLastError());
    return 0;
}

static int gauss_samp_impl(GpuMatrix *src, uint32_t base_bits, double c, GpuRngSeed seed, GpuMatrix *out, const RngSegments *segs);

extern "C" int gpu_matrix_gauss_samp_gq_arb_base(GpuMatrix *src, uint32_t base_bits, double c, double dgg_stddev,
                                                 GpuRngSeed seed, GpuMatrix *out) {
    ABI_GUARD_BEGIN
    (void)dgg_stddev;
    return gauss_samp_impl(src, base_bits, c, seed, out, nullptr);
    ABI_GUARD_END
}

extern "C" int gpupoly_matrix_gauss_samp_gq_arb_base_segments(GpuMatrix *src, uint32_t base_bits, double c, double dgg_stddev,
                                                              const GpuRngSeed *seeds, const size_t *seg_cols, size_t nseg,
                                                              GpuMatrix *out) {
    ABI_GUARD_BEGIN
    (void)dgg_stddev;
    if (!src || !out) return set_error("invalid gpupoly_matrix_gauss_samp_gq_arb_base_segments arguments");
    if (static_cast<size_t>(src->ctx->N) % SAMPLER_THREADS)
        return set_error("gpupoly_matrix_gauss_samp_gq_arb_base_segments: unsupported: ring too small for a wave per polynomial chunk");
    RngSegments segs;
    if (!rng_segments_build(segs, seeds, seg_cols, nseg, kTagGadget, src->cols))
        return set_error("gpupoly_matrix_gauss_samp_gq_arb_base_segments: segments must be 1..64, non-empty and cover the source's columns");
    return gauss_samp_impl(src, base_bits, c, GpuRngSeed{}, out, &segs);
    ABI_GUARD_END
}

static int gauss_samp_impl(GpuMatrix *src, uint32_t base_bits, double c, GpuRngSeed seed, GpuMatrix *out, const RngSegments *segs) {
    {
    if (!src || !out) return set_error("invalid gpu_matrix_gauss_samp_gq_arb_base arguments");
    if (base_bits == 0 || base_bits >= 63) return set_error("invalid base_bits in gpu_matrix_gauss_samp_gq_arb_base");
    if (!(c > 0.0)) return set_error("c must be positive in gpu_matrix_gauss_samp_gq_arb_base");
    if (src->ctx != out->ctx || src->level != out->level)
        return set_error("context mismatch in gpu_matrix_gauss_samp_gq_arb_base");
    GpuContext *ctx = src->ctx;
    const int requested = out->format;
    const size_t L = matrix_limbs(src);
    const uint32_t dpt = (ctx->crt_bits + base_bits - 1) / base_bits;
    if (dpt == 0 || dpt > kGaussMaxDigits)
        return set_error("invalid digits_per_tower in gpu_matrix_gauss_samp_gq_arb_base");
    const size_t k = static_cast<size_t>(dpt) * L;
    if (out->rows != src->rows * k || out->cols != src->cols)
        return set_error("output size mismatch in gpu_matrix_gauss_samp_gq_arb_base");
    if (storage_overlaps(src, out)) return set_error("gpu_matrix_gauss_samp_gq_arb_base: output must not alias the source");
    const size_t polys = matrix_polys(src);
    if (polys == 0) {
        out->format = GPU_POLY_FORMAT_EVAL;
        return 0;
    }
    if (ctx_activate(ctx)) return 1;
    if (src->format == GPU_POLY_FORMAT_EVAL) {
        int rc = gpu_matrix_intt_all(src);
        if (rc) return rc;
    }
    int rc = ctx->wide ? launch_gauss_samp<uint64_t>(ctx, static_cast<uint64_t *>(words_ptr(out)),
                                                     static_cast<const uint64_t *>(words_ptr(src)), polys,
                                                     (uint32_t)src->cols, (uint32_t)L, dpt, base_bits, c, k, seed, segs)
                       : launch_gauss_samp<uint32_t>(ctx, static_cast<uint32_t *>(words_ptr(out)),
                                                     static_cast<const uint32_t *>(words_ptr(src)), polys,
                                                     (uint32_t)src->cols, (uint32_t)L, dpt, base_bits, c, k, seed, segs);
    if (rc) return rc;
    out->format = GPU_POLY_FORMAT_COEFF;
    if (requested == GPU_POLY_FORMAT_EVAL) {
        rc = launch_ntt(ctx, words_ptr(out), matrix_polys(out) * L, static_cast<int>(L), false);
        if (rc) return rc;
        out->format = GPU_POLY_FORMAT_EVAL;
    }
    return 0;
    }
}

struct P1KeyedSegments {
    RngSegments segs;
    const P1KeyEntry *keys;
};
template <typename W>
__global__ void p1_covariance_kernel(const W *__restrict__ a_mat, const W *__restrict__ b_mat,
                                     const W *__restrict__ d_mat, uint32_t d, uint32_t L, uint32_t N, uint64_t q0,
                                     double sigma, double s, double dgg_stddev, double *__restrict__ cov_ws,
                                     double *__restrict__ sqrt_var_out, double *__restrict__ update_out) {
    const uint32_t i = blockIdx.x * blockDim.x + threadIdx.x;
    if (i >= N) return;
    const uint32_t m = 2 * d;
    double *cov = cov_ws + static_cast<size_t>(i) * m * m;
    double *sqrt_var = sqrt_var_out + static_cast<size_t>(i) * m;
    double *upd = update_out + static_cast<size_t>(i) * m * m;
    const double sigma2 = sigma * sigma, s2 = s * s, fallback = dgg_stddev * dgg_stddev, eps = 1e-9;
    for (uint32_t r = 0; r < d; ++r)
        for (uint32_t c = 0; c < d; ++c) {
            const size_t rc = (static_cast<size_t>(r) * d + c) * L * N + i;
            const size_t cr = (static_cast<size_t>(c) * d + r) * L * N + i;
            const double a_rc = static_cast<double>(centered_residue(a_mat[rc], q0));
            const double d_rc = static_cast<double>(centered_residue(d_mat[rc], q0));
            const double b_rc = static_cast<double>(centered_residue(b_mat[rc], q0));
            const double b_cr = static_cast<double>(centered_residue(b_mat[cr], q0));
            cov[r * m + c] = -sigma2 * a_rc + (r == c ? s2 : 0.0);
            cov[(r + d) * m + (c + d)] = -sigma2 * d_rc + (r == c ? s2 : 0.0);
            cov[r * m + (c + d)] = -sigma2 * b_rc;
            cov[(r + d) * m + c] = -sigma2 * b_cr;
        }
    for (int t = static_cast<int>(m) - 1; t >= 0; --t) {
        double var = cov[t * m + t];
        if (!(var > eps)) var = fallback;
        sqrt_var[t] = sqrt(var);
        for (int r = 0; r < t; ++r) upd[t * m + r] = cov[r * m + t] / var;
        if (t == 0) break;
        for (int r = 0; r < t; ++r) {
            const double cr = upd[t * m + r];
            for (int c = 0; c <= r; ++c) {
                const double colc = upd[t * m + c] * var;
                const double v = cov[r * m + c] - cr * colc;
// ... 180 lines not shown
    if (!(sigma > 0.0) || !(s > sigma)) return set_error(std::string("invalid sigma/s in ") + who);
    if (!(dgg_stddev > 0.0)) return set_error(std::string("dgg_stddev must be positive in ") + who);
    if (a->ctx != b->ctx || a->ctx != d->ctx) return set_error(std::string("context mismatch in ") + who);
    if (a->level != b->level || a->level != d->level) return set_error(std::string("level mismatch in ") + who);
    const size_t dr = a->rows;
    if (a->cols != dr || b->rows != dr || b->cols != dr || d->rows != dr || d->cols != dr)
        return set_error(std::string("A/B/D must be dxd in ") + who);
    if (a->format != GPU_POLY_FORMAT_COEFF || b->format != GPU_POLY_FORMAT_COEFF || d->format != GPU_POLY_FORMAT_COEFF)
        return set_error(std::string("A/B/D must be in Coeff format in ") + who);
    return 0;
}

extern "C" int gpu_matrix_create_p1_covariance_cache(const GpuMatrix *a_mat, const GpuMatrix *b_mat,
                                                     const GpuMatrix *d_mat, double sigma, double s, double dgg_stddev,
                                                     GpuP1CovarianceCache **out_cache) {
    ABI_GUARD_BEGIN
    if (!out_cache) return set_error("gpu_matrix_create_p1_covariance_cache: null out_cache");
    *out_cache = nullptr;
    if (check_p1_inputs(a_mat, b_mat, d_mat, sigma, s, dgg_stddev, "gpu_matrix_create_p1_covariance_cache")) return 1;
    GpuContext *ctx = a_mat->ctx;
    const size_t d = a_mat->rows, m = 2 * d, n = static_cast<size_t>(ctx->N);
    GpuP1CovarianceCache *cache = new GpuP1CovarianceCache();
    cache->ctx = ctx;
    cache->level = a_mat->level;
    cache->d = d;
    cache->m = m;
    cache->n = n;
    cache->sigma = sigma;
    cache->s = s;
    cache->dgg_stddev = dgg_stddev;
    if (d == 0) {
        *out_cache = cache;
        return 0;
    }
    if (ctx_activate(ctx)) {
        delete cache;
        return 1;
    }
    void *cov_ws = nullptr, *sv = nullptr, *uc = nullptr, *kd = nullptr;
    if (ctx_alloc(ctx, n * m * m * sizeof(double), &cov_ws) || ctx_alloc(ctx, n * m * sizeof(double), &sv) ||
        ctx_alloc(ctx, n * m * m * sizeof(double), &uc) || ctx_alloc(ctx, n * m * sizeof(KarneyDivisor), &kd)) {
        ctx_free(ctx, cov_ws);
        ctx_free(ctx, sv);
        ctx_free(ctx, uc);
        delete cache;
        return 1;
    }
    cache->sqrt_var = static_cast<double *>(sv);
    cache->update_coeff = static_cast<double *>(uc);
    cache->karney_div = kd;
    {
        const hipError_t me = hipMemsetAsync(uc, 0, n * m * m * sizeof(double), ctx->stream);
        if (me != hipSuccess) {
            ctx_free(ctx, cov_ws);
            gpu_matrix_destroy_p1_covariance_cache(cache);
            return set_error(me, "hipMemsetAsync");
        }
    }
    const uint32_t L = static_cast<uint32_t>(matrix_limbs(a_mat));
    const unsigned blocks = static_cast<unsigned>((n + 127) / 128);
    if (ctx->wide)
        MXX_LAUNCH(p1_covariance_kernel<uint64_t>, dim3(blocks), dim3(128), 0, ctx->stream,
                           static_cast<const uint64_t *>(words_ptr(a_mat)), static_cast<const uint64_t *>(words_ptr(b_mat)),
                           static_cast<const uint64_t *>(words_ptr(d_mat)), (uint32_t)d, L, (uint32_t)n, ctx->moduli[0],
                           sigma, s, dgg_stddev, static_cast<double *>(cov_ws), cache->sqrt_var, cache->update_coeff);
    else
        MXX_LAUNCH(p1_covariance_kernel<uint32_t>, dim3(blocks), dim3(128), 0, ctx->stream,
                           static_cast<const uint32_t *>(words_ptr(a_mat)), static_cast<const uint32_t *>(words_ptr(b_mat)),
                           static_cast<const uint32_t *>(words_ptr(d_mat)), (uint32_t)d, L, (uint32_t)n, ctx->moduli[0],
                           sigma, s, dgg_stddev, static_cast<double *>(cov_ws), cache->sqrt_var, cache->update_coeff);
    MXX_LAUNCH(p1_divisor_kernel, dim3(static_cast<unsigned>((n * m + 255) / 256)), dim3(256), 0, ctx->stream,
                       static_cast<KarneyDivisor *>(kd), cache->sqrt_var, n * m);
    hipError_t e = hipGetLastError();
    ctx_free(ctx, cov_ws);
    if (e != hipSuccess) {
        gpu_matrix_destroy_p1_covariance_cache(cache);
        return set_error(e, "p1_covariance_kernel");
    }
    *out_cache = cache;
    return 0;
    ABI_GUARD_END
}

extern "C" void gpu_matrix_destroy_p1_covariance_cache(GpuP1CovarianceCache *cache) {
    if (!cache) return;
    if (cache->ctx) {
        (void)hipSetDevice(cache->ctx->device);
        ctx_free(cache->ctx, cache->sqrt_var);
        ctx_free(cache->ctx, cache->update_coeff);
        ctx_free(cache->ctx, cache->karney_div);
    }
    delete cache;
}

static int sample_p1_impl(const GpuP1CovarianceCache *cache, const GpuMatrix *tp2, GpuRngSeed seed, GpuMatrix *out, const RngSegments *segs,
                          const P1KeyEntry *d_keys = nullptr);

extern "C" int gpu_matrix_sample_p1_full_cached(const GpuP1CovarianceCache *cache, const GpuMatrix *tp2,
                                                GpuRngSeed seed, GpuMatrix *out) {
    ABI_GUARD_BEGIN
    return sample_p1_impl(cache, tp2, seed, out, nullptr);
    ABI_GUARD_END
}

extern "C" int gpupoly_matrix_sample_p1_full_cached_segments(const GpuP1CovarianceCache *cache, const GpuMatrix *tp2,
                                                             const GpuRngSeed *seeds, const size_t *seg_cols, size_t nseg,
                                                             GpuMatrix *out) {
    ABI_GUARD_BEGIN
    if (!cache || !tp2 || !out) return set_error("invalid gpupoly_matrix_sample_p1_full_cached_segments arguments");
    if (cache->m > 8)
        return set_error("gpupoly_matrix_sample_p1_full_cached_segments: unsupported: trapdoor dimension above 4 (no lane kernel)");
    if (cache->ctx->env.p1_simple)
        return set_error("gpupoly_matrix_sample_p1_full_cached_segments: unsupported under MXX_HIP_P1=simple (the lane kernel is switched off)");
    if (static_cast<size_t>(cache->ctx->N) % SAMPLER_THREADS)
        return set_error("gpupoly_matrix_sample_p1_full_cached_segments: unsupported: ring too small for a wave per column chunk");
    RngSegments segs;
    if (!rng_segments_build(segs, seeds, seg_cols, nseg, kTagP1, tp2->cols))
        return set_error("gpupoly_matrix_sample_p1_full_cached_segments: segments must be 1..64, non-empty and cover tp2's columns");
    return sample_p1_impl(cache, tp2, GpuRngSeed{}, out, &segs);
    ABI_GUARD_END
}

int sample_p1_keyed_segments(const GpuP1CovarianceCache *cache, const P1KeyEntry *d_keys, const GpuMatrix *tp2,
                             const GpuRngSeed *seeds, const size_t *seg_cols, size_t nseg, GpuMatrix *out) {
    if (!cache || !d_keys || !tp2 || !out) return set_error("invalid sample_p1_keyed_segments arguments");
    if (cache->m > 8)
        return set_error("sample_p1_keyed_segments: unsupported: trapdoor dimension above 4 (no lane kernel)");
    if (cache->ctx->env.p1_simple)
        return set_error("sample_p1_keyed_segments: unsupported under MXX_HIP_P1=simple (the lane kernel is switched off)");
    if (static_cast<size_t>(cache->ctx->N) % SAMPLER_THREADS)
        return set_error("sample_p1_keyed_segments: unsupported: ring too small for a wave per column chunk");
    RngSegments segs;
    if (!rng_segments_build(segs, seeds, seg_cols, nseg, kTagP1, tp2->cols))
        return set_error("sample_p1_keyed_segments: segments must be 1..64, non-empty and cover tp2's columns");
    return sample_p1_impl(cache, tp2, GpuRngSeed{}, out, &segs, d_keys);
}

static int sample_p1_impl(const GpuP1CovarianceCache *cache, const GpuMatrix *tp2, GpuRngSeed seed, GpuMatrix *out,
                          const RngSegments *segs, const P1KeyEntry *d_keys) {
    {
    if (!cache || !tp2 || !out) return set_error("invalid gpu_matrix_sample_p1_full_cached arguments");
    GpuContext *ctx = cache->ctx;
    if (tp2->ctx != ctx || out->ctx != ctx) return set_error("context mismatch in gpu_matrix_sample_p1_full_cached");
    if (tp2->level != cache->level || out->level != cache->level)
        return set_error("level mismatch in gpu_matrix_sample_p1_full_cached");
    const size_t m = cache->m, cols = tp2->cols;
    if (tp2->rows != m || out->rows != m || out->cols != cols)
        return set_error("tp2/out shape mismatch in gpu_matrix_sample_p1_full_cached");
    if (storage_overlaps(tp2, out)) return set_error("gpu_matrix_sample_p1_full_cached: output must not alias tp2");
    if (cols == 0 || m == 0) {
        out->format = GPU_POLY_FORMAT_EVAL;
        return 0;
    }
    if (tp2->format != GPU_POLY_FORMAT_COEFF)
        return set_error("tp2 must be in Coeff format in gpu_matrix_sample_p1_full_cached");
    const double denom = cache->s * cache->s - cache->sigma * cache->sigma;
    if (!(denom > 0.0)) return set_error("invalid cached Gaussian denominator");
    const double c_scale = -(cache->sigma * cache->sigma) / denom;
    if (ctx_activate(ctx)) return 1;
    const uint32_t L = static_cast<uint32_t>(matrix_limbs(out)), N = static_cast<uint32_t>(ctx->N);
    const size_t total = cols * static_cast<size_t>(N);
    if (m <= 8 && !ctx->env.p1_simple) {
        CtxBlock stage(ctx);
        if (stage.alloc(total * m * sizeof(int64_t))) return 1;
        const ChaChaKey key = chacha_subkey(seed, 0, kTagP1);
        MXX_TRACE_BYTES(static_cast<double>(total) * m * (ctx->word_bytes + 8.0) +
                        static_cast<double>(N) * m * (8.0 + sizeof(KarneyDivisor) + 8.0 * m));
        const bool keyed = segs && d_keys;
        const double *sqrt_var = keyed ? nullptr : cache->sqrt_var, *update = keyed ? nullptr : cache->update_coeff;
        const KarneyDivisor *kdiv = keyed ? nullptr : static_cast<const KarneyDivisor *>(cache->karney_div);
#define P1_LANES(WT, MAXM, SEGARG, ...)                                                                                            \
    MXX_LAUNCH_LANES(plan, ctx->stream, (p1_sample_lanes_kernel<WT, MAXM, 1, __VA_ARGS__>),                                        \
                     (p1_sample_lanes_kernel<WT, MAXM, KARNEY_SERVICES, __VA_ARGS__>), static_cast<int64_t *>(stage.ptr),          \
                     static_cast<const WT *>(words_ptr(tp2)), sqrt_var, update, kdiv, (uint32_t)m, (uint32_t)cols, L, ctx->logN,   \
                     ctx->moduli[0], c_scale, key, total, plan.per_lane, plan.fill_every, SEGARG)
#define LAUNCH_P1L(WT, MAXM)                                                                                                       \
    do {                                                                                                                           \
        const LanePlan plan = lane_plan(total, N,                                                                                  \
                                        sampler_per_lane(total, reinterpret_cast<const void *>(p1_sample_lanes_kernel<WT, MAXM, KARNEY_SERVICES>), ctx->device, ctx->env.sampler_per_lane), \
                                        segs != nullptr, ctx->env.sampler_fill_every, kCadenceP1, false);                          \
        if (keyed) P1_LANES(WT, MAXM, (P1KeyedSegments{*segs, d_keys}), true, true);                                               \
        else if (segs) P1_LANES(WT, MAXM, *segs, true);                                                                            \
        else P1_LANES(WT, MAXM, NoSegments{}, false);                                                                              \
    } while (0)
        if (ctx->wide) {
            if (m <= 2) LAUNCH_P1L(uint64_t, 2);
            else if (m <= 4) LAUNCH_P1L(uint64_t, 4);
            else LAUNCH_P1L(uint64_t, 8);
        } else {
            if (m <= 2) LAUNCH_P1L(uint32_t, 2);
            else if (m <= 4) LAUNCH_P1L(uint32_t, 4);
            else LAUNCH_P1L(uint32_t, 8);
        }
#undef LAUNCH_P1L
#undef P1_LANES
        return finish_staged_i64(out, stage, hipGetLastError(), "p1_sample_lanes_kernel");
    }
    const dim3 blocks = item_grid(total, 128);
    void *mean_ws = nullptr;
    if (m > 8 && ctx_alloc(ctx, total * m * sizeof(double), &mean_ws)) return 1;
#define LAUNCH_P1(WT, MAXM)                                                                                       \
    MXX_LAUNCH((p1_sample_kernel<WT, MAXM>), dim3(blocks), dim3(128), 0, ctx->stream,                      \
                       static_cast<WT *>(words_ptr(out)), static_cast<const WT *>(words_ptr(tp2)), ctx->d_limbs,             \
                       cache->sqrt_var, cache->update_coeff, (uint32_t)m, (uint32_t)cols, L, N, ctx->moduli[0],    \
                       c_scale, seed, static_cast<double *>(mean_ws))
    if (ctx->wide) {
        if (m <= 2) LAUNCH_P1(uint64_t, 2);
        else if (m <= 4) LAUNCH_P1(uint64_t, 4);
        else if (m <= 8) LAUNCH_P1(uint64_t, 8);
        else LAUNCH_P1(uint64_t, 0);
    } else {
        if (m <= 2) LAUNCH_P1(uint32_t, 2);
        else if (m <= 4) LAUNCH_P1(uint32_t, 4);
        else if (m <= 8) LAUNCH_P1(uint32_t, 8);
        else LAUNCH_P1(uint32_t, 0);
    }
#undef LAUNCH_P1
    hipError_t e = hipGetLastError();
    if (mean_ws) ctx_free(ctx, mean_ws);
    if (e != hipSuccess) return set_error(e, "p1_sample_kernel");
    int rc = launch_ntt(ctx, words_ptr(out), matrix_polys(out) * L, static_cast<int>(L), false);
    if (rc) return rc;
    out->format = GPU_POLY_FORMAT_EVAL;
    return 0;
    }
}

extern "C" int gpu_matrix_sample_p1_full(const GpuMatrix *a_mat, const GpuMatrix *b_mat, const GpuMatrix *d_mat,
                                         const GpuMatrix *tp2, double sigma, double s, double dgg_stddev,
                                         GpuRngSeed seed, GpuMatrix *out) {
    ABI_GUARD_BEGIN
    if (out && ((tp2 && storage_overlaps(tp2, out)) || (a_mat && storage_overlaps(a_mat, out)) ||
                (b_mat && storage_overlaps(b_mat, out)) || (d_mat && storage_overlaps(d_mat, out))))
        return set_error("gpu_matrix_sample_p1_full: output must not alias an input");
    if (check_p1_inputs(a_mat, b_mat, d_mat, sigma, s, dgg_stddev, "gpu_matrix_sample_p1_full")) return 1;
    if (tp2 && out && (tp2->ctx != a_mat->ctx || out->ctx != a_mat->ctx)) return set_error("context mismatch in gpu_matrix_sample_p1_full");
    if (tp2 && out && (tp2->level != a_mat->level || out->level != a_mat->level))
        return set_error("level mismatch in gpu_matrix_sample_p1_full");
    GpuP1CovarianceCache *cache = nullptr;
    int rc = gpu_matrix_create_p1_covariance_cache(a_mat, b_mat, d_mat, sigma, s, dgg_stddev, &cache);
    if (rc) return rc;
    rc = gpu_matrix_sample_p1_full_cached(cache, tp2, seed, out);
    gpu_matrix_destroy_p1_covariance_cache(cache);
    return rc;
    ABI_GUARD_END
}
```

mxx_amd/matrix.py:

```python
from __future__ import annotations

import ctypes as C
import os
import threading
import weakref

import numpy as np

from . import _ffi
from ._ffi import GPU_POLY_FORMAT_COEFF, GPU_POLY_FORMAT_EVAL, GpuRngSeed, check_status
from .params import GpuDCRTPolyParams


def mul_decompose_column_chunk_width_is_set() -> bool:
    return bool(os.environ.get("MXX_MUL_DECOMPOSE_COLUMN_CHUNK_WIDTH"))


def mul_decompose_column_chunk_width() -> int:
    try:
        return max(1, int(os.environ.get("MXX_MUL_DECOMPOSE_COLUMN_CHUNK_WIDTH", "1")))
    except ValueError:
        return 1


# ... 1142 lines not shown
    def _same_domain(self, others):
        for o in others:
            assert o.params == self.params and o.level == self.level, "concat requires same params/level"
        return [o.ensure_eval() if self.is_ntt else o.ensure_coeff() for o in others]

    def concat_columns(self, others) -> "GpuDCRTPolyMatrix":
        others = self._same_domain(others)
        for o in others:
            assert o.nrow == self.nrow, "concat_columns requires same row count"
        ncol = self.ncol + sum(o.ncol for o in others)
        out = GpuDCRTPolyMatrix(self.params, self.nrow, ncol, self.level, self.is_ntt)
        off = 0
        for m in [self] + others:
            out.copy_block_from(m, 0, off, 0, 0, m.nrow, m.ncol)
            off += m.ncol
        out.is_ntt = self.is_ntt
        return out

    def concat_rows(self, others) -> "GpuDCRTPolyMatrix":
        others = self._same_domain(others)
        for o in others:
            assert o.ncol == self.ncol, "concat_rows requires same column count"
        nrow = self.nrow + sum(o.nrow for o in others)
        out = GpuDCRTPolyMatrix(self.params, nrow, self.ncol, self.level, self.is_ntt)
        off = 0
        for m in [self] + others:
            out.copy_block_from(m, off, 0, 0, 0, m.nrow, m.ncol)
            off += m.nrow
        out.is_ntt = self.is_ntt
        return out

    def concat_diag(self, others) -> "GpuDCRTPolyMatrix":
        others = self._same_domain(others)
        nrow = self.nrow + sum(o.nrow for o in others)
        ncol = self.ncol + sum(o.ncol for o in others)
        out = GpuDCRTPolyMatrix._new_zero_with_state(self.params, nrow, ncol, self.level, self.is_ntt)
        ro = co = 0
        for m in [self] + others:
            out.copy_block_from(m, ro, co, 0, 0, m.nrow, m.ncol)
            ro += m.nrow
            co += m.ncol
        out.is_ntt = self.is_ntt
        return out

    def tensor(self, other) -> "GpuDCRTPolyMatrix":
        assert self.params == other.params and self.level == other.level and self.is_ntt == other.is_ntt
        out = GpuDCRTPolyMatrix(self.params, self.nrow * other.nrow, self.ncol * other.ncol, self.level, self.is_ntt)
        if 0 in (self.nrow, self.ncol, other.nrow, other.ncol):
            return out
        lhs, rhs = self.ensure_eval(), other.ensure_eval()
        st = _ffi.lib().gpupoly_matrix_tensor(out.raw, lhs.raw, rhs.raw)
        check_status(st, "gpupoly_matrix_tensor")
        out.is_ntt = True
        return out

    def vectorize_columns(self) -> "GpuDCRTPolyMatrix":
        out = GpuDCRTPolyMatrix(self.params, self.nrow * self.ncol, 1, self.level, self.is_ntt)
        for j in range(self.ncol):
            out.copy_block_from(self, j * self.nrow, 0, 0, j, self.nrow, 1)
        return out

    def _check_binop(self, rhs, what):
        assert self.params == rhs.params, f"{what} requires same params"
        assert self.level == rhs.level, f"{what} requires same level"
        assert self.is_ntt == rhs.is_ntt, f"{what} requires same domain"
        assert (self.nrow, self.ncol) == (rhs.nrow, rhs.ncol), f"{what} requires same dimensions"

    def add_in_place(self, rhs) -> None:
        self._check_binop(rhs, "add_in_place")
        if self.nrow == 0 or self.ncol == 0:
            return
        self._touch()
        check_status(_ffi.lib().gpu_matrix_add(self.raw, self.raw, rhs.raw), "gpu_matrix_add")
        self.is_ntt = rhs.is_ntt

    def sub_in_place(self, rhs) -> None:
        self._check_binop(rhs, "sub_in_place")
        if self.nrow == 0 or self.ncol == 0:
            return
        self._touch()
        check_status(_ffi.lib().gpu_matrix_sub(self.raw, self.raw, rhs.raw), "gpu_matrix_sub")
        self.is_ntt = rhs.is_ntt

    def _binop(self, rhs, fn, what):
        self._check_binop(rhs, what)
        out = GpuDCRTPolyMatrix(self.params, self.nrow, self.ncol, self.level, self.is_ntt)
        if self.nrow == 0 or self.ncol == 0:
            return out
        check_status(fn(out.raw, self.raw, rhs.raw), what)
        out.is_ntt = rhs.is_ntt
        return out

    def __add__(self, rhs):
        return self._binop(rhs, _ffi.lib().gpu_matrix_add, "gpu_matrix_add")

    def __sub__(self, rhs):
        return self._binop(rhs, _ffi.lib().gpu_matrix_sub, "gpu_matrix_sub")

    def __neg__(self):
        out = GpuDCRTPolyMatrix(self.params, self.nrow, self.ncol, self.level, self.is_ntt)
        if self.nrow == 0 or self.ncol == 0:
            return out
        check_status(_ffi.lib().gpupoly_matrix_neg(out.raw, self.raw), "gpupoly_matrix_neg")
        return out

    def mul_scalar(self, scalar) -> "GpuDCRTPolyMatrix":
        s = scalar.inner if hasattr(scalar, "inner") else scalar
        lhs = self.ensure_eval()
        s = s.ensure_eval()
        out = GpuDCRTPolyMatrix(self.params, self.nrow, self.ncol, self.level, True)
        if self.nrow == 0 or self.ncol == 0:
            return out
        check_status(_ffi.lib().gpu_matrix_mul_scalar(out.raw, lhs.raw, s.raw), "gpu_matrix_mul_scalar")
        return out

    @classmethod
    def monomial(cls, params, nrow, ncol, shift, eval_format: bool = True, level=None) -> "GpuDCRTPolyMatrix":
        out = cls(params, nrow, ncol, params.crt_depth() - 1 if level is None else level, eval_format)
        fmt = GPU_POLY_FORMAT_EVAL if eval_format else GPU_POLY_FORMAT_COEFF
        shift = int(shift) % (2 * params.ring_dimension())
        check_status(_ffi.lib().gpupoly_matrix_fill_monomial(out.raw, shift, fmt), "gpupoly_matrix_fill_monomial")
        return out

    def mul_monomial(self, shift) -> "GpuDCRTPolyMatrix":
        out = GpuDCRTPolyMatrix(self.params, self.nrow, self.ncol, self.level, self.is_ntt)
        shift = int(shift) % (2 * self.params.ring_dimension())
        check_status(_ffi.lib().gpupoly_matrix_mul_monomial(out.raw, self.raw, shift), "gpupoly_matrix_mul_monomial")
        return out

    @staticmethod
    def monomial_sum(mats, shifts, addend=None, negate: bool = False, out=None) -> "GpuDCRTPolyMatrix":
        mats, shifts = list(mats), list(shifts)
        n = len(mats)
        assert len(shifts) == n, "monomial_sum: one shift per matrix"
        first = addend if addend is not None else (mats[0] if n else out)
        if first is None:
            raise ValueError("monomial_sum: no operand to take the shape from")
        for m in mats + ([addend] if addend is not None else []):
            first._check_binop(m, "monomial_sum")
        if out is None:
            out = GpuDCRTPolyMatrix(first.params, first.nrow, first.ncol, first.level, first.is_ntt)
        else:
            out._touch()
        two_n = 2 * first.params.ring_dimension()
        marr = (C.c_void_p * max(n, 1))(*[m.raw.value for m in mats])
        sarr = (C.c_uint64 * max(n, 1))(*[int(s) % two_n for s in shifts])
        st = _ffi.lib().gpupoly_matrix_monomial_sum(out.raw, None if addend is None else addend.raw, marr, sarr, n, 1 if negate else 0)
        check_status(st, "gpupoly_matrix_monomial_sum")
        if n or addend is not None:
            out.is_ntt = first.is_ntt
        return out

    @staticmethod
    def mul_sum(lhss, rhss, addend=None, negate: bool = False, out=None, dst_col: int = 0) -> "GpuDCRTPolyMatrix":
        lhss, rhss = list(lhss), list(rhss)
        n = len(lhss)
        assert len(rhss) == n, "mul_sum: one right operand per left operand"
        first = out if out is not None else (addend if addend is not None else (lhss[0] if n else None))
        if first is None:
            raise ValueError("mul_sum: no operand to take the shape from")
        cols = rhss[0].ncol if n else first.ncol - dst_col
        for l_, r_ in zip(lhss, rhss):
            assert l_.params == first.params and r_.params == first.params, "mul_sum requires same params"
            assert l_.level == first.level and r_.level == first.level, "mul_sum requires same level"
            assert l_.is_ntt and r_.is_ntt, "mul_sum requires NTT domain"
            assert l_.ncol == r_.nrow and l_.nrow == first.nrow and r_.ncol == cols, "mul_sum: term shape mismatch"
        if out is None:
            assert dst_col == 0, "mul_sum: dst_col needs an `out` to place the block in"
            out = GpuDCRTPolyMatrix(first.params, first.nrow, cols, first.level, True)
        else:
            out._touch()
        if addend is not None:
            assert addend.is_ntt and (addend.nrow, addend.ncol) == (out.nrow, out.ncol), "mul_sum: the addend has out's shape, NTT domain"
        larr = (C.c_void_p * max(n, 1))(*[m.raw.value for m in lhss])
        rarr = (C.c_void_p * max(n, 1))(*[m.raw.value for m in rhss])
        st = _ffi.lib().gpupoly_matrix_mul_sum(out.raw, dst_col, cols, None if addend is None else addend.raw, larr, rarr, n, 1 if negate else 0)
        check_status(st, "gpupoly_matrix_mul_sum")
        out.is_ntt = True
        return out

    def _mul_acc(self, lhs, rhs, negate: bool) -> None:
        assert self.params == lhs.params == rhs.params, "mul_acc requires same params"
        assert self.level == lhs.level == rhs.level, "mul_acc requires same level"
        assert self.is_ntt and lhs.is_ntt and rhs.is_ntt, "mul_acc requires NTT domain"
        assert lhs.ncol == rhs.nrow and (lhs.nrow, rhs.ncol) == (self.nrow, self.ncol), "mul_acc: shape mismatch"
        self._touch()
        check_status(_ffi.lib().gpupoly_matrix_mul_acc(self.raw, lhs.raw, rhs.raw, 1 if negate else 0), "gpupoly_matrix_mul_acc")

    def mul_add_in_place(self, lhs, rhs) -> None:
        self._mul_acc(lhs, rhs, False)

    def mul_sub_in_place(self, lhs, rhs) -> None:
        self._mul_acc(lhs, rhs, True)

    @staticmethod
    def _gadget_digits(params, level, small: bool) -> int:
        dpt = -(-params.crt_bits() // params.base_bits())
        return dpt if small else dpt * (level + 1)

    @staticmethod
    def _scalar_raw(scalar):
        if scalar is None:
            return None, None
        s = scalar.inner if hasattr(scalar, "inner") else scalar
        s = s.ensure_eval()
        return s, s.raw

    def mul_gadget(self, scalar=None, col_start: int = 0, col_end=None, addend=None, negate: bool = False, out=None, dst_col: int = 0,
                   small: bool = False) -> "GpuDCRTPolyMatrix":
        assert self.is_ntt, "mul_gadget requires NTT domain"
        k = self._gadget_digits(self.params, self.level, small)
        col_end = self.ncol * k if col_end is None else col_end
        cols = col_end - col_start
        assert 0 <= col_start <= col_end <= self.ncol * k, "mul_gadget: gadget window out of range"
        s, s_raw = self._scalar_raw(scalar)
        if out is None:
            assert dst_col == 0, "mul_gadget: dst_col needs an `out` to place the block in"
            out = GpuDCRTPolyMatrix(self.params, self.nrow, cols, self.level, True)
        else:
            out._touch()
        if addend is not None:
            assert addend.is_ntt and (addend.nrow, addend.ncol) == (out.nrow, out.ncol), "mul_gadget: the addend has out's shape, NTT domain"
        st = _ffi.lib().gpupoly_matrix_mul_gadget(out.raw, dst_col, self.raw, s_raw, col_start, cols, None if addend is None else addend.raw,
                                                  1 if negate else 0, self.params.base_bits(), 1 if small else 0)
        check_status(st, "gpupoly_matrix_mul_gadget")
        out.is_ntt = True
        return out

    def add_scaled_gadget(self, scalar=None, negate: bool = False, gadget_col: int = 0, small: bool = False) -> None:
        assert self.is_ntt, "add_scaled_gadget requires NTT domain"
        s, s_raw = self._scalar_raw(scalar)
        self._touch()
        st = _ffi.lib().gpupoly_matrix_mul_gadget(self.raw, 0, None, s_raw, gadget_col, self.ncol, self.raw, 1 if negate else 0,
                                                  self.params.base_bits(), 1 if small else 0)
        check_status(st, "gpupoly_matrix_mul_gadget")

    @classmethod
    def gadget_block(cls, params, size, col_start, col_end, scalar=None, negate: bool = False, small: bool = False, level=None) -> "GpuDCRTPolyMatrix":
        level = params.crt_depth() - 1 if level is None else level
        out = cls(params, size, col_end - col_start, level, True)
        s, s_raw = cls._scalar_raw(scalar)
        st = _ffi.lib().gpupoly_matrix_mul_gadget(out.raw, 0, None, s_raw, col_start, col_end - col_start, None, 1 if negate else 0,
                                                  params.base_bits(), 1 if small else 0)
        check_status(st, "gpupoly_matrix_mul_gadget")
        return out

    @staticmethod
    def gadget_mul(rhs, addend=None, negate: bool = False, small: bool = False) -> "GpuDCRTPolyMatrix":
        k = GpuDCRTPolyMatrix._gadget_digits(rhs.params, rhs.level, small)
        assert rhs.nrow % k == 0, "gadget_mul: rhs rows must be a multiple of the digit count"
        out = GpuDCRTPolyMatrix(rhs.params, rhs.nrow // k, rhs.ncol, rhs.level, rhs.is_ntt)
        if addend is not None:
            assert addend.is_ntt == rhs.is_ntt and (addend.nrow, addend.ncol) == (out.nrow, out.ncol), "gadget_mul: addend shape / domain mismatch"
        st = _ffi.lib().gpupoly_matrix_gadget_mul(out.raw, rhs.raw, None if addend is None else addend.raw, 1 if negate else 0,
                                                  rhs.params.base_bits(), 1 if small else 0)
        check_status(st, "gpupoly_matrix_gadget_mul")
        return out

    def mul_scalar_intt(self, scalar) -> "GpuDCRTPolyMatrix":
        s = scalar.inner if hasattr(scalar, "inner") else scalar
        lhs = self.ensure_eval()
        s = s.ensure_eval()
        out = GpuDCRTPolyMatrix(self.params, self.nrow, self.ncol, self.level, False)
        if self.nrow == 0 or self.ncol == 0:
            return out
        check_status(_ffi.lib().gpupoly_matrix_mul_scalar_intt(out.raw, lhs.raw, s.raw), "gpupoly_matrix_mul_scalar_intt")
        return out

    def __mul__(self, rhs):
        from .poly import GpuDCRTPoly

        if isinstance(rhs, GpuDCRTPoly):
            return self.mul_scalar(rhs)
        return self._mul_internal(rhs)

    __matmul__ = __mul__

    def _mul_internal(self, rhs) -> "GpuDCRTPolyMatrix":
        assert self.ncol == rhs.nrow, f"matrix multiply shape mismatch: ({self.nrow},{self.ncol}) x ({rhs.nrow},{rhs.ncol})"
        assert self.params == rhs.params, "mul requires same params"
        assert self.level == rhs.level, "mul requires same level"
        assert self.is_ntt and rhs.is_ntt, "mul requires NTT domain"
        out = GpuDCRTPolyMatrix(self.params, self.nrow, rhs.ncol, self.level, True)
        if self.nrow == 0 or rhs.ncol == 0:
            return out
        check_status(_ffi.lib().gpu_matrix_mul(out.raw, self.raw, rhs.raw), "gpu_matrix_mul")
        return out

    def __eq__(self, other):
        if not isinstance(other, GpuDCRTPolyMatrix):
            return NotImplemented
        if (
            self.params != other.params
            or (self.nrow, self.ncol) != (other.nrow, other.ncol)
            or self.level != other.level
            or self.is_ntt != other.is_ntt
        ):
            return False
        if self.raw.value == other.raw.value:
            return True
        eq = C.c_int(0)
        check_status(_ffi.lib().gpu_matrix_equal(self.raw, other.raw, C.byref(eq)), "gpu_matrix_equal")
        return eq.value != 0

    __hash__ = None

    def _decompose_from(self, src, out_nrow, small) -> "GpuDCRTPolyMatrix":
        out = GpuDCRTPolyMatrix.new_empty(self.params, out_nrow, self.ncol)
        fn = _ffi.lib().gpu_matrix_decompose_base_small if small else _ffi.lib().gpu_matrix_decompose_base
        check_status(fn(src.raw, self.params.base_bits(), out.raw), "gpu_matrix_decompose_base")
        return out

    def decompose(self) -> "GpuDCRTPolyMatrix":
        return self._decompose_from(self, self.nrow * self.params.modulus_digits(), False)

    def decompose_owned(self) -> "GpuDCRTPolyMatrix":
        self.intt_all_in_place()
        return self._decompose_from(self, self.nrow * self.params.modulus_digits(), False)

    def small_decompose(self) -> "GpuDCRTPolyMatrix":
        k = -(-self.params.crt_bits() // self.params.base_bits())
        return self._decompose_from(self, self.nrow * k, True)

    def small_decompose_owned(self) -> "GpuDCRTPolyMatrix":
        self.intt_all_in_place()
        k = -(-self.params.crt_bits() // self.params.base_bits())
        return self._decompose_from(self, self.nrow * k, True)

    @classmethod
    def small_decomposed_identity_chunk(cls, params, size, chunk_idx, chunk_count, scalar_by_digit):
# ... 271 lines not shown
                arr[0, 0, i, : len(w)] = w
            return None, GpuDCRTPolyMatrix.from_coeff_words(first.params, arr, True, level=first.level)
        s = scalar.inner if hasattr(scalar, "inner") else scalar
        assert s.size() == (1, 1), "large_scalar_mul: the scalar is a polynomial or a 1 x 1 matrix"
        return None, s

    def large_scalar_mul(self, scalar) -> "GpuDCRTPolyMatrix":
        return GpuDCRTPolyMatrix.large_scalar_mul_many([self], scalar)[0]

    @staticmethod
    def large_scalar_mul_many(lhss, scalar, addends=None, negate: bool = False) -> list:
        lhss = list(lhss)
        n = len(lhss)
        addends = [None] * n if addends is None else list(addends)
        assert len(addends) == n, "large_scalar_mul_many: one addend slot per operand"
        if n == 0:
            return []
        first = lhss[0]
        k = GpuDCRTPolyMatrix._gadget_digits(first.params, first.level, False)
        for l_, a_ in zip(lhss, addends):
            assert l_.params == first.params and l_.level == first.level, "large_scalar_mul_many: one context and level per call"
            assert l_.ncol % k == 0, "large_scalar_mul_many: lhs columns must be a multiple of the digit count"
            assert a_ is None or (a_.nrow, a_.ncol) == (l_.nrow, l_.ncol), "large_scalar_mul_many: addend shape"
        const, sc = GpuDCRTPolyMatrix._large_scalar(first, scalar)
        if mul_decompose_column_chunk_width_is_set():
            outs = []
            for l_, a_ in zip(lhss, addends):
                prod = l_._large_scalar_mul_host(const if sc is None else sc)
                if a_ is None:
                    outs.append(-prod if negate else prod)
                else:
                    outs.append(a_.ensure_eval() - prod if negate else a_.ensure_eval() + prod)
            return outs
        ls = [m.ensure_eval() for m in lhss]
        ads = [None if m is None else m.ensure_eval() for m in addends]
        outs = [GpuDCRTPolyMatrix(first.params, l_.nrow, l_.ncol, l_.level, True) for l_ in ls]
        raw = lambda m: None if m is None else (m.raw.value if hasattr(m.raw, "value") else m.raw)
        arr = lambda ms: (C.c_void_p * n)(*[raw(m) for m in ms])
        base = first.params.base_bits()
        if sc is None:
            words = GpuDCRTPolyMatrix._int_words(const)
            st = _ffi.lib().gpupoly_matrix_mul_decompose_gadget_const_many(
                arr(outs), arr(ls), arr(ads), n, words.ctypes.data_as(C.POINTER(C.c_uint64)), len(words), 1 if negate else 0, base)
            check_status(st, "gpupoly_matrix_mul_decompose_gadget_const_many")
        else:
            st = _ffi.lib().gpupoly_matrix_mul_decompose_gadget_scalar_many(arr(outs), arr(ls), arr(ads), n, sc.raw, 1 if negate else 0, base)
            check_status(st, "gpupoly_matrix_mul_decompose_gadget_scalar_many")
        return outs

    def _large_scalar_mul_host(self, scalar) -> "GpuDCRTPolyMatrix":
        k = self._gadget_digits(self.params, self.level, False)
        assert self.ncol % k == 0
        d = self.ncol // k
        out = GpuDCRTPolyMatrix(self.params, self.nrow, self.ncol, self.level, True)
        if self.nrow == 0 or d == 0:
            return out
        if isinstance(scalar, (int, np.integer)):
            words = self._int_words(scalar).reshape(1, 1, 1, -1)
            scalar = GpuDCRTPolyMatrix.from_coeff_words(self.params, words, True, level=self.level)
        s = (scalar.inner if hasattr(scalar, "inner") else scalar).ensure_eval()
        g = GpuDCRTPolyMatrix(self.params, d, d * k, self.level, True)
        check_status(_ffi.lib().gpu_matrix_fill_gadget(g.raw, self.params.base_bits()), "gpu_matrix_fill_gadget")
        gs = GpuDCRTPolyMatrix(self.params, d, d * k, self.level, True)
        check_status(_ffi.lib().gpu_matrix_mul_scalar(gs.raw, g.raw, s.raw), "gpu_matrix_mul_scalar")
        lhs = self.ensure_eval()
        st = _ffi.lib().gpupoly_matrix_mul_decompose(out.raw, lhs.raw, gs.raw, self.params.base_bits())
        check_status(st, "gpupoly_matrix_mul_decompose")
        return out

    def mul_decompose_small(self, other) -> "GpuDCRTPolyMatrix":
        k = -(-self.params.crt_bits() // self.params.base_bits())
        assert self.ncol == other.nrow * k
        ncol = other.ncol
        out = GpuDCRTPolyMatrix.new_empty(self.params, self.nrow, ncol)
        if self.nrow == 0 or ncol == 0:
            return out
        if not mul_decompose_column_chunk_width_is_set():
            lhs = self.ensure_eval()
            st = _ffi.lib().gpupoly_matrix_mul_decompose_small(out.raw, lhs.raw, other.raw, self.params.base_bits())
            check_status(st, "gpupoly_matrix_mul_decompose_small")
            return out
        width = min(mul_decompose_column_chunk_width(), ncol)
        for c0 in range(0, ncol, width):
            c1 = min(c0 + width, ncol)
            dec = other.slice(0, other.nrow, c0, c1).small_decompose_owned()
            prod = self._mul_internal(dec)
            out.copy_block_from(prod, 0, c0, 0, 0, self.nrow, c1 - c0)
        return out

    @classmethod
    def sample_distribution(cls, params, nrow, ncol, dist: int, sigma: float, seed: GpuRngSeed):
        out = cls.new_empty(params, nrow, ncol)
        if nrow == 0 or ncol == 0:
            return out
        check_status(_ffi.lib().gpu_matrix_sample_distribution(out.raw, dist, sigma, seed), "gpu_matrix_sample_distribution")
        return out

    @classmethod
    def sample_distribution_columns(cls, params, nrow, total_ncol, col_start, col_len, dist, sigma, seed):
        assert col_start + col_len <= total_ncol, "sample_distribution_columns range out of bounds"
        out = cls.new_empty(params, nrow, col_len)
        if nrow == 0 or col_len == 0:
            return out
        st = _ffi.lib().gpu_matrix_sample_distribution_columns(out.raw, dist, sigma, seed, total_ncol, col_start)
        check_status(st, "gpu_matrix_sample_distribution_columns")
        return out

    @classmethod
    def sample_distribution_decomposed(cls, params, nrow, ncol, dist: int, sigma: float, seed: GpuRngSeed, small=False):
        k = -(-params.crt_bits() // params.base_bits()) if small else params.modulus_digits()
        out = cls.new_empty(params, nrow * k, ncol)
        if nrow == 0 or ncol == 0:
            return out
        st = _ffi.lib().gpupoly_matrix_sample_decomposed(out.raw, dist, sigma, seed, params.base_bits(), 1 if small else 0)
        check_status(st, "gpupoly_matrix_sample_decomposed")
        return out

    @classmethod
    def sample_distribution_decomposed_window(cls, params, nrow, total_ncol, col_start, col_len, dist: int, sigma: float,
                                              seed: GpuRngSeed, small=False, row_start=0, row_end=None, is_ntt=True,
                                              level=None):
        assert col_start + col_len <= total_ncol, "sample_distribution_decomposed_window column range out of bounds"
        level = params.crt_depth() - 1 if level is None else level
        dpt = -(-params.crt_bits() // params.base_bits())
        k = dpt if small else dpt * (level + 1)
        if row_end is None:
            row_end = nrow * k
        assert 0 <= row_start <= row_end <= nrow * k, f"sample_distribution_decomposed_window rows [{row_start}, {row_end}) out of range: {nrow * k} digit rows"
        out = cls(params, row_end - row_start, col_len, level, is_ntt)
        st = _ffi.lib().gpupoly_matrix_sample_decomposed_window(out.raw, dist, sigma, seed, params.base_bits(), 1 if small else 0,
                                                                nrow, total_ncol, col_start, row_start)
        check_status(st, "gpupoly_matrix_sample_decomposed_window")
        if row_end == row_start or col_len == 0:
            out.is_ntt = True
        return out

    def gauss_samp_gq_arb_base(self, c: float, dgg_stddev: float, seed: GpuRngSeed, coeff_out: bool = False) -> "GpuDCRTPolyMatrix":
        out = GpuDCRTPolyMatrix(self.params, self.nrow * self.params.modulus_digits(), self.ncol, self.params.crt_depth() - 1,
                                not coeff_out)
        self.intt_all_in_place()
        self._touch()
        st = _ffi.lib().gpu_matrix_gauss_samp_gq_arb_base(self.raw, self.params.base_bits(), c, dgg_stddev, seed, out.raw)
        check_status(st, "gpu_matrix_gauss_samp_gq_arb_base")
        return out

    @staticmethod
    def create_p1_covariance_cache(a_mat, b_mat, d_mat, sigma, s, dgg_stddev) -> GpuP1CovarianceCache:
        raw = C.c_void_p()
        st = _ffi.lib().gpu_matrix_create_p1_covariance_cache(a_mat.raw, b_mat.raw, d_mat.raw, sigma, s, dgg_stddev, C.byref(raw))
        check_status(st, "gpu_matrix_create_p1_covariance_cache")
        return GpuP1CovarianceCache(raw, a_mat.params)

    @staticmethod
    def sample_p1_full_cached(cache: GpuP1CovarianceCache, tp2, seed: GpuRngSeed) -> "GpuDCRTPolyMatrix":
        out = GpuDCRTPolyMatrix.new_empty(tp2.params, tp2.nrow, tp2.ncol)
        if tp2.nrow == 0 or tp2.ncol == 0:
            return out
        tp2.intt_all_in_place()
        check_status(_ffi.lib().gpu_matrix_sample_p1_full_cached(cache.raw, tp2.raw, seed, out.raw), "gpu_matrix_sample_p1_full_cached")
        return out

    @staticmethod
    def _segment_args(seeds, seg_cols):
        assert len(seeds) == len(seg_cols) and seeds, "one seed per segment"
        return (GpuRngSeed * len(seeds))(*seeds), (C.c_size_t * len(seg_cols))(*seg_cols), len(seeds)

    @classmethod
    def sample_distribution_segments(cls, params, nrow, seg_cols, dist: int, sigma: float, seeds) -> "GpuDCRTPolyMatrix":
        out = cls.new_empty(params, nrow, sum(seg_cols))
        arr, cols, n = cls._segment_args(seeds, seg_cols)
        check_status(_ffi.lib().gpupoly_matrix_sample_distribution_segments(out.raw, dist, sigma, arr, cols, n),
                     "gpupoly_matrix_sample_distribution_segments")
        return out

    @classmethod
    def sample_distribution_blocks(cls, params, seeds, dist: int, *, block_polys=None, nrow=None, seg_cols=None) -> "GpuDCRTPolyMatrix":
        seeds = list(seeds)
        level = params.crt_depth() - 1
        arr = (GpuRngSeed * max(len(seeds), 1))(*seeds)
        if seg_cols is None:
            assert block_polys is not None and nrow is None, "sample_distribution_blocks: block_polys (stacked) or nrow and seg_cols (columns)"
            out = cls(params, len(seeds), block_polys, level, True)
            layout, cols = _ffi.GPUPOLY_BLOCKS_STACKED, None
        else:
            assert block_polys is None and nrow is not None, "sample_distribution_blocks: block_polys (stacked) or nrow and seg_cols (columns)"
            seg_cols = list(seg_cols)
            assert len(seg_cols) == len(seeds), "sample_distribution_blocks: one seed per block"
            out = cls(params, nrow, sum(seg_cols), level, True)
            layout, cols = _ffi.GPUPOLY_BLOCKS_COLUMNS, (C.c_size_t * max(len(seg_cols), 1))(*seg_cols)
        check_status(_ffi.lib().gpupoly_matrix_sample_distribution_blocks(out.raw, dist, arr, len(seeds), layout, cols),
                     "gpupoly_matrix_sample_distribution_blocks")
        return out

    @classmethod
    def sample_hash_blocks(cls, params, key: bytes, tags, dist: int, *, hash_name: str = "keccak256", block_polys=None, nrow=None,
                           seg_cols=None) -> "GpuDCRTPolyMatrix":
        arg, keep, count = hash_tags_arg(key, tags, hash_name)
        level = params.crt_depth() - 1
        if seg_cols is None:
            assert block_polys is not None and nrow is None, "sample_hash_blocks: block_polys (stacked) or nrow and seg_cols (columns)"
            out = cls(params, count, block_polys, level, True)
            layout, cols = _ffi.GPUPOLY_BLOCKS_STACKED, None
        else:
            assert block_polys is None and nrow is not None, "sample_hash_blocks: block_polys (stacked) or nrow and seg_cols (columns)"
            seg_cols = list(seg_cols)
            assert len(seg_cols) == count, "sample_hash_blocks: one tag per block"
            out = cls(params, nrow, sum(seg_cols), level, True)
            layout, cols = _ffi.GPUPOLY_BLOCKS_COLUMNS, (C.c_size_t * max(len(seg_cols), 1))(*seg_cols)
        check_status(_ffi.lib().gpupoly_matrix_sample_hash_blocks(out.raw, dist, C.byref(arg), count, layout, cols),
                     "gpupoly_matrix_sample_hash_blocks")
        del keep
        return out

    @classmethod
    def _blocks_out(cls, who, params, count, block_polys, nrow, seg_cols):
        level = params.crt_depth() - 1
        if seg_cols is None:
            assert block_polys is not None and nrow is None, f"{who}: block_polys (stacked) or nrow and seg_cols (columns)"
            return cls(params, count, block_polys, level, True), _ffi.GPUPOLY_BLOCKS_STACKED, None
        assert block_polys is None and nrow is not None, f"{who}: block_polys (stacked) or nrow and seg_cols (columns)"
        seg_cols = list(seg_cols)
        assert len(seg_cols) == count, f"{who}: one seed or tag per block"
        return cls(params, nrow, sum(seg_cols), level, True), _ffi.GPUPOLY_BLOCKS_COLUMNS, (C.c_size_t * max(len(seg_cols), 1))(*seg_cols)

    @classmethod
    def sample_gauss_blocks(cls, params, seeds, sigma: float, *, block_polys=None, nrow=None, seg_cols=None) -> "GpuDCRTPolyMatrix":
        seeds = list(seeds)
        arr = (GpuRngSeed * max(len(seeds), 1))(*seeds)
        out, layout, cols = cls._blocks_out("sample_gauss_blocks", params, len(seeds), block_polys, nrow, seg_cols)
        check_status(_ffi.lib().gpupoly_matrix_sample_gauss_blocks(out.raw, float(sigma), arr, len(seeds), layout, cols),
                     "gpupoly_matrix_sample_gauss_blocks")
        return out

    @classmethod
    def sample_hash_gauss_blocks(cls, params, key: bytes, tags, sigma: float, *, hash_name: str = "keccak256", block_polys=None,
                                 nrow=None, seg_cols=None) -> "GpuDCRTPolyMatrix":
        arg, keep, count = hash_tags_arg(key, tags, hash_name)
        out, layout, cols = cls._blocks_out("sample_hash_gauss_blocks", params, count, block_polys, nrow, seg_cols)
        check_status(_ffi.lib().gpupoly_matrix_sample_hash_gauss_blocks(out.raw, float(sigma), C.byref(arg), count, layout, cols),
                     "gpupoly_matrix_sample_hash_gauss_blocks")
        del keep
        return out

    @classmethod
    def _decomposed_blocks_out(cls, params, nblk, nrow, col_len, small, is_ntt, level):
        level = params.crt_depth() - 1 if level is None else level
        dpt = -(-params.crt_bits() // params.base_bits())
        k = dpt if small else dpt * (level + 1)
        return cls(params, nrow * k, nblk * col_len, level, is_ntt)

    @classmethod
    def sample_decomposed_blocks(cls, params, seeds, nrow, total_ncol, col_start, col_len, dist: int, small=False, is_ntt=True,
                                 level=None) -> "GpuDCRTPolyMatrix":
        seeds = list(seeds)
        out = cls._decomposed_blocks_out(params, len(seeds), nrow, col_len, small, is_ntt, level)
        arr = (GpuRngSeed * max(len(seeds), 1))(*seeds)
        st = _ffi.lib().gpupoly_matrix_sample_decomposed_blocks(out.raw, dist, arr, len(seeds), params.base_bits(), 1 if small else 0, nrow,
                                                                total_ncol, col_start)
        check_status(st, "gpupoly_matrix_sample_decomposed_blocks")
        if out.nrow == 0 or out.ncol == 0:
            out.is_ntt = True
        return out

    @classmethod
    def sample_hash_decomposed_blocks(cls, params, key: bytes, tags, nrow, total_ncol, col_start, col_len, dist: int, small=False,
                                      is_ntt=True, level=None, hash_name: str = "keccak256") -> "GpuDCRTPolyMatrix":
        arg, keep, count = hash_tags_arg(key, tags, hash_name)
        out = cls._decomposed_blocks_out(params, count, nrow, col_len, small, is_ntt, level)
        st = _ffi.lib().gpupoly_matrix_sample_hash_decomposed_blocks(out.raw, dist, C.byref(arg), count, params.base_bits(), 1 if small else 0,
                                                                     nrow, total_ncol, col_start)
        check_status(st, "gpupoly_matrix_sample_hash_decomposed_blocks")
        del keep
        if out.nrow == 0 or out.ncol == 0:
            out.is_ntt = True
        return out

    @staticmethod
    def _int_rows(values):
        words = [GpuDCRTPolyMatrix._int_words(v) for v in values]
        arr = np.zeros((len(words), max(len(w) for w in words)), dtype=np.uint64)
        for t, w in enumerate(words):
            arr[t, : len(w)] = w
        return arr, arr.shape[1]

    @staticmethod
    def _wee25_call(entry: str, t_bottom, nparts, secret_size, idxs, args) -> list:
        p = t_bottom.params
        outs = [GpuDCRTPolyMatrix(p, secret_size, t_bottom.nrow, t_bottom.level, True) for _ in range(len(idxs) * nparts)]
        if outs:
            i_arr = np.array(idxs, dtype=np.uint64)
            st = getattr(_ffi.lib(), entry)(GpuDCRTPolyMatrix._raw_array(outs), len(idxs), nparts, *args(i_arr.ctypes.data_as(C.POINTER(C.c_uint64))))
            check_status(st, entry)
        return [outs[t * nparts:(t + 1) * nparts] for t in range(len(idxs))]

    @staticmethod
    def lut_targets(w_identity, w_gy, w_v, w_vx, col_start, col_len, ys, idxs, key: bytes, tags, hash_name: str = "keccak256") -> list:
        ys, idxs = [int(y) for y in ys], [int(i) for i in idxs]
        arg, keep, count = hash_tags_arg(key, tags, hash_name)
        assert len(ys) == len(idxs) == count, "lut_targets: one y, one index and one tag per row"
        p = w_identity.params
        outs = [GpuDCRTPolyMatrix(p, w_identity.nrow, col_len, w_identity.level, True) for _ in range(count)]
        if count == 0:
            return outs
        y_arr, wpy = GpuDCRTPolyMatrix._int_rows(ys)
        i_arr = np.array(idxs, dtype=np.uint64)
        u64p = C.POINTER(C.c_uint64)
        st = _ffi.lib().gpupoly_matrix_lut_targets(GpuDCRTPolyMatrix._raw_array(outs), count, w_identity.raw, w_gy.raw, w_v.raw, w_vx.raw,
                                                   col_start, p.base_bits(), y_arr.ctypes.data_as(u64p), wpy, i_arr.ctypes.data_as(u64p),
                                                   C.byref(arg))
        check_status(st, "gpupoly_matrix_lut_targets")
        del keep
# ... 227 lines not shown
```

mxx_amd/trapdoor.py:

```python
from __future__ import annotations

import math
import threading
import weakref

from .matrix import GpuDCRTPolyMatrix
from .sampler import DistType, GpuDCRTPolyUniformSampler, random_gpu_rng_seed, sample_gpu_matrix_with_seed

SPECTRAL_CONSTANT = 1.8


def preimage_c(base: int, sigma: float) -> float:
    return (base + 1.0) * sigma


def preimage_smoothing_parameter(base: int, sigma: float, d: int, n: int, k: int) -> float:
    return SPECTRAL_CONSTANT * (base + 1.0) * sigma * sigma * (math.sqrt(d * n * k) + math.sqrt(2 * n) + 4.7)


def p1_covariance_parameters(params, d: int, dgg_stddev: float):
    base = 1 << params.base_bits()
    n, k = params.ring_dimension(), params.modulus_digits()
    return preimage_c(base, dgg_stddev), preimage_smoothing_parameter(base, dgg_stddev, d, n, k), dgg_stddev

# ... 53 lines not shown
                self.a_mat_coeff, self.b_mat_coeff, self.d_mat_coeff, c, s, dgg_stddev
            )
            self._p1_cache = ((c, s, dgg_stddev), cache)
            return cache

    get_or_create_p1_covariance_cache = p1_covariance_cache

    def public_matrix_parts(self, public_matrix: GpuDCRTPolyMatrix):
        with self._p1_lock:
            if self._stacked is not None and self._stacked[0]() is public_matrix and self._stacked[2] == public_matrix.content_version():
                return self._stacked[1]
            d, p1_rows, p2_rows = public_matrix.row_size(), self.re.row_size(), self.re.col_size()
            left = public_matrix.slice(0, d, 0, p1_rows)
            right = public_matrix.slice(0, d, p1_rows, p1_rows + p2_rows)
            parts = (left, right, self.re.concat_rows([right]))
            self._stacked = (weakref.ref(public_matrix), parts, public_matrix.content_version())
            return parts

    def clear_public_matrix_cache(self) -> None:
        with self._p1_lock:
            self._stacked = None
            self._replicas = {}

    def replica_for(self, params, public_matrix: GpuDCRTPolyMatrix):
        key = params.ctx_raw().value
        with self._p1_lock:
            hit = self._replicas.get(key)
            if hit is not None and hit[2]() is public_matrix and hit[3] == public_matrix.content_version():
                return hit[0], hit[1]
        td, a = self.to_params(params), public_matrix.to_params(params)
        with self._p1_lock:
            self._replicas[key] = (td, a, weakref.ref(public_matrix), public_matrix.content_version())
        return td, a

    def to_params(self, params) -> "GpuDCRTTrapdoor":
        return GpuDCRTTrapdoor(self.r.to_params(params), self.e.to_params(params))

    def to_compact_bytes(self) -> bytes:
        out = b""
        for m in (self.r, self.e):
            b = m.to_compact_bytes()
            out += len(b).to_bytes(8, "little") + b
        return out

    @classmethod
    def from_compact_bytes(cls, params, data: bytes):
        mats, off = [], 0
        for _ in range(2):
            if off + 8 > len(data):
                return None
            ln = int.from_bytes(data[off : off + 8], "little")
            off += 8
            if off + ln > len(data):
                return None
            mats.append(GpuDCRTPolyMatrix.from_compact_bytes(params, data[off : off + ln]))
            off += ln
        if off != len(data):
            return None
        return cls(mats[0], mats[1])

    def __eq__(self, other):
        return isinstance(other, GpuDCRTTrapdoor) and self.r == other.r and self.e == other.e

    __hash__ = None


WORKER_DNUM = 0x5700
_worker_params_cache: dict = {}
_worker_params_lock = threading.Lock()


def preimage_workers() -> int:
    import os

    try:
        return max(1, min(8, int(os.environ.get("MXX_PREIMAGE_WORKERS", "4"))))
    except ValueError:
        return 4


def worker_params(params, k: int):
    from .params import GpuDCRTPolyParams

    key = (params.ctx_raw().value, k)
    with _worker_params_lock:
        for dead in [kk for kk, (owner, _) in _worker_params_cache.items() if owner() is None]:
            del _worker_params_cache[dead]
        hit = _worker_params_cache.get(key)
        if hit is not None and hit[0]() is params.ctx():
            return hit[1]
        pw = GpuDCRTPolyParams(params.ring_dimension(), params.moduli(), params.base_bits(), gpu_ids=params.gpu_ids(), dnum=WORKER_DNUM + k)
        _worker_params_cache[key] = (weakref.ref(params.ctx()), pw)
        return pw


TRAFFIC_BOUND_BYTES = 32 << 20


def _traffic_bound(params, polys: int) -> bool:
    word = 4 if max(params.moduli()) < (1 << 31) else 8
    return polys * params.crt_depth() * params.ring_dimension() * word >= TRAFFIC_BOUND_BYTES


class GpuDCRTPolyTrapdoorSampler:
    def __init__(self, params, sigma: float):
        self.sigma = float(sigma)
        self.base = 1 << params.base_bits()
        self.c = preimage_c(self.base, self.sigma)

    @staticmethod
    def trapdoor_to_bytes(trapdoor: "GpuDCRTTrapdoor") -> bytes:
        return trapdoor.to_compact_bytes()

    @staticmethod
    def trapdoor_from_bytes(params, data: bytes):
        return GpuDCRTTrapdoor.from_compact_bytes(params, data)

    def trapdoor(self, params, size: int):
        u = GpuDCRTPolyUniformSampler()
        td = GpuDCRTTrapdoor.new(params, size, self.sigma)
        a_bar = u.sample_uniform(params, size, size, DistType.FinRingDist())
        g = GpuDCRTPolyMatrix.gadget_matrix(params, size)
        a0 = a_bar.concat_columns([GpuDCRTPolyMatrix.identity(params, size)])
        a1 = g - (a_bar * td.r + td.e)
        return td, a0.concat_columns([a1])

    def _sample_pert(self, params, td: GpuDCRTTrapdoor, s, c, dgg_stddev, sigma_large, total_ncol):
        return self._sample_pert_parts(params, td, s, c, dgg_stddev, sigma_large, total_ncol)[:2]

    def sample_pert_square_mat_gpu_native_parts(self, params, td, s, c, dgg_stddev, sigma_large, total_ncol):
        return GpuPerturbationSamples(*self._sample_pert(params, td, s, c, dgg_stddev, sigma_large, total_ncol))

    def sample_pert_square_mat_gpu_native(self, params, td, s, c, dgg_stddev, sigma_large, total_ncol):
        p1, p2 = self._sample_pert(params, td, s, c, dgg_stddev, sigma_large, total_ncol)
        assert p1.col_size() >= total_ncol and p2.col_size() >= total_ncol, "p1 / p2 must include the target columns"
        p_hat = GpuDCRTPolyMatrix(params, p1.row_size() + p2.row_size(), total_ncol, p1.level, p1.is_ntt)
        p_hat.copy_block_from(p1, 0, 0, 0, 0, p1.row_size(), total_ncol)
        p_hat.copy_block_from(p2, p1.row_size(), 0, 0, 0, p2.row_size(), total_ncol)
        return p_hat

    @staticmethod
    def _draw_seeds():
        return random_gpu_rng_seed(), random_gpu_rng_seed(), random_gpu_rng_seed()

    def _sample_pert_parts(self, params, td: GpuDCRTTrapdoor, s, c, dgg_stddev, sigma_large, total_ncol, stacked=None, seeds=None):
        d, dk = td.r.row_size(), td.r.col_size()
        padded = -(-total_ncol // d) * d
        seed_p2 = seeds[0] if seeds is not None else random_gpu_rng_seed()
        p2 = sample_gpu_matrix_with_seed(params, dk, padded, DistType.GaussDist(sigma_large), seed_p2)
        rp2 = tp2_eval = None
        if stacked is not None and _traffic_bound(params, dk * padded):
            t = stacked * p2
            re_rows = td.re.row_size()
            tp2 = t.slice(0, re_rows, 0, padded)
            tp2_eval = t.row_view(0, re_rows)
            rp2 = t.row_view(re_rows, t.row_size())
        else:
            tp2 = td.re * p2
            if _traffic_bound(params, dk * padded):
                tp2_eval = tp2.clone()
        cache = td.p1_covariance_cache(c, s, dgg_stddev)
        p1 = GpuDCRTPolyMatrix.sample_p1_full_cached(cache, tp2, seeds[1] if seeds is not None else random_gpu_rng_seed())
        return p1, p2, tp2_eval, rp2

    def preimage(self, params, td: GpuDCRTTrapdoor, public_matrix, target, _seeds=None) -> GpuDCRTPolyMatrix:
        d = public_matrix.row_size()
        target_cols = target.col_size()
        assert target.row_size() == d, "Target matrix should have the same number of rows as the public matrix"
        n, k = params.ring_dimension(), params.modulus_digits()
        s = preimage_smoothing_parameter(self.base, self.sigma, d, n, k)
        dgg_large_std = math.sqrt(s * s - self.c * self.c)
        p1_rows, p2_rows = td.re.row_size(), td.re.col_size()
        assert public_matrix.col_size() == p1_rows + p2_rows, "public matrix columns must match perturbation rows"
        left, right, stacked = td.public_matrix_parts(public_matrix)
        p1, p2, tp2, rp2 = self._sample_pert_parts(params, td, s, self.c, self.sigma, dgg_large_std, target_cols, stacked, _seeds)
        seed_z = _seeds[2] if _seeds is not None else None
        assert (p1.row_size(), p2.row_size()) == (p1_rows, p2_rows)
        p_hat_image = (left * p1) + (rp2 if rp2 is not None else right * p2)
        if p_hat_image.col_size() != target_cols:
            p_hat_image = p_hat_image.slice_columns(0, target_cols)
        perturbed = target - p_hat_image
        out = GpuDCRTPolyMatrix(params, p1_rows + p2_rows, target_cols, p1.level, p1.is_ntt)
        if p1.col_size() == target_cols and tp2 is not None:
            z = perturbed.gauss_samp_gq_arb_base(self.c, self.sigma, seed_z if seed_z is not None else random_gpu_rng_seed(), coeff_out=True)
            out.ntt_add_rows_from(p1_rows, z, p2, consume=True)
            re_x = td.re * out.row_view(p1_rows, p1_rows + p2_rows)
            out.add_rows_from(0, p1 - tp2, re_x)
            return out
        z_hat = perturbed.gauss_samp_gq_arb_base(self.c, self.sigma, seed_z if seed_z is not None else random_gpu_rng_seed())
        re_z = td.re * z_hat
        if p1.col_size() == target_cols:
            out.add_rows_from(0, p1, re_z)
            out.add_rows_from(p1_rows, p2, z_hat)
            return out
        out.copy_block_from(p1, 0, 0, 0, 0, p1_rows, target_cols)
        out.copy_block_from(p2, p1_rows, 0, 0, 0, p2_rows, target_cols)
        out.add_block_from(re_z, 0, 0, 0, 0, re_z.row_size(), target_cols)
        out.add_block_from(z_hat, 2 * d, 0, 0, 0, z_hat.row_size(), target_cols)
        return out

    def preimage_reference_sequence(self, params, td: GpuDCRTTrapdoor, public_matrix, target) -> GpuDCRTPolyMatrix:
        d = public_matrix.row_size()
        target_cols = target.col_size()
        assert target.row_size() == d, "Target matrix should have the same number of rows as the public matrix"
        n, k = params.ring_dimension(), params.modulus_digits()
        s = preimage_smoothing_parameter(self.base, self.sigma, d, n, k)
        dgg_large_std = math.sqrt(s * s - self.c * self.c)
        u = GpuDCRTPolyUniformSampler()
        dd, dk = td.r.row_size(), td.r.col_size()
        padded = -(-target_cols // dd) * dd
        p2 = u.sample_uniform(params, dk, padded, DistType.GaussDist(dgg_large_std))
        tp2 = td.r.concat_rows([td.e]) * p2
        cache = td.p1_covariance_cache(self.c, s, self.sigma)
        p1 = GpuDCRTPolyMatrix.sample_p1_full_cached(cache, tp2, random_gpu_rng_seed())
        p1_rows, p2_rows = p1.row_size(), p2.row_size()
        assert public_matrix.col_size() == p1_rows + p2_rows, "public matrix columns must match perturbation rows"
        public_left = public_matrix.slice(0, d, 0, p1_rows)
        public_right = public_matrix.slice(0, d, p1_rows, p1_rows + p2_rows)
        p_hat_image = (public_left * p1) + (public_right * p2)
        if p_hat_image.col_size() != target_cols:
            p_hat_image = p_hat_image.slice_columns(0, target_cols)
        perturbed = target - p_hat_image
        z_hat = perturbed.gauss_samp_gq_arb_base(self.c, self.sigma, random_gpu_rng_seed())
        r_z = td.r * z_hat
        out = GpuDCRTPolyMatrix(params, p1_rows + p2_rows, target_cols, p1.level, p1.is_ntt)
        out.copy_block_from(p1, 0, 0, 0, 0, p1_rows, target_cols)
        out.copy_block_from(p2, p1_rows, 0, 0, 0, p2_rows, target_cols)
        del p1, p2
        out.add_block_from(r_z, 0, 0, 0, 0, r_z.row_size(), target_cols)
        del r_z
        e_z = td.e * z_hat
        out.add_block_from(e_z, d, 0, 0, 0, e_z.row_size(), target_cols)
        del e_z
        out.add_block_from(z_hat, 2 * d, 0, 0, 0, z_hat.row_size(), target_cols)
        return out

    def preimage_extend(self, params, td, public_matrix, ext_matrix, target) -> GpuDCRTPolyMatrix:
        d = public_matrix.row_size()
        n, k = params.ring_dimension(), params.modulus_digits()
        s = preimage_smoothing_parameter(self.base, self.sigma, d, n, k)
        u = GpuDCRTPolyUniformSampler()
        right = u.sample_uniform(params, ext_matrix.col_size(), target.col_size(), DistType.GaussDist(s))
        t = target - (ext_matrix * right)
        left = self.preimage(params, td, public_matrix, t)
        return left.concat_rows([right])

    BATCH_BYTES = 1 << 30

    @staticmethod
    def _segments_supported(params, td: GpuDCRTTrapdoor) -> bool:
        import os

        dpt = -(-params.crt_bits() // params.base_bits())
        return (params.ring_dimension() % 128 == 0 and td.r.row_size() <= 4 and dpt <= 4
                and not os.environ.get("MXX_HIP_RNG_COMPAT", "").startswith("r")
                and not os.environ.get("MXX_HIP_P1", "").startswith("s")
                and os.environ.get("MXX_PREIMAGE_BATCH", "1") != "0")

    def preimage_many(self, params, td: GpuDCRTTrapdoor, public_matrix, targets, _seeds=None) -> list:
        targets = list(targets)
        seeds = list(_seeds) if _seeds is not None else [self._draw_seeds() for _ in targets]
        results = [None] * len(targets)
        dd, dk = td.r.row_size(), td.r.col_size()
        word = 4 if max(params.moduli()) < (1 << 31) else 8
        poly_bytes = params.crt_depth() * params.ring_dimension() * word
        batchable = []
        for j, t in enumerate(targets):
            pad = -(-t.col_size() // dd) * dd
            if t.col_size() == 0 or _traffic_bound(params, dk * pad) or not self._segments_supported(params, td):
                results[j] = self.preimage(params, td, public_matrix, t, _seeds=seeds[j])
            else:
                batchable.append(j)
        while batchable:
            group, size = [], 0
            while batchable and len(group) < 64:
                j = batchable[0]
                pad = -(-targets[j].col_size() // dd) * dd
                if group and size + dk * pad * poly_bytes > self.BATCH_BYTES:
                    break
                group.append(batchable.pop(0))
                size += dk * pad * poly_bytes
            if len(group) == 1:
                results[group[0]] = self.preimage(params, td, public_matrix, targets[group[0]], _seeds=seeds[group[0]])
                continue
            for j, x in zip(group, self._preimage_segments(params, td, public_matrix, [targets[j] for j in group], [seeds[j] for j in group])):
                results[j] = x
        return results

    @staticmethod
    def _drop_padding(m, cols, pads):
        if cols == pads:
            return m
        widths = []
        for c, p_ in zip(cols, pads):
            widths += [c, p_ - c]
        parts = m.split_columns(widths)
        return GpuDCRTPolyMatrix.concat_columns_of(parts[0::2])

    def _preimage_segments(self, params, td: GpuDCRTTrapdoor, public_matrix, targets, seeds) -> list:
        M = GpuDCRTPolyMatrix
        d = public_matrix.row_size()
        dd, dk = td.r.row_size(), td.r.col_size()
        cols = [t.col_size() for t in targets]
        pads = [-(-c // dd) * dd for c in cols]
        for t in targets:
            assert t.row_size() == d, "Target matrix should have the same number of rows as the public matrix"
        n, k = params.ring_dimension(), params.modulus_digits()
        s = preimage_smoothing_parameter(self.base, self.sigma, d, n, k)
        dgg_large_std = math.sqrt(s * s - self.c * self.c)
        p1_rows, p2_rows = td.re.row_size(), td.re.col_size()
        assert public_matrix.col_size() == p1_rows + p2_rows, "public matrix columns must match perturbation rows"
        left, right, _ = td.public_matrix_parts(public_matrix)
        gauss = DistType.GaussDist(dgg_large_std)
        p2_pad = M.sample_distribution_segments(params, dk, pads, gauss.as_ffi(), gauss.sigma, [sd[0] for sd in seeds])
        tp2 = td.re * p2_pad
        cache = td.p1_covariance_cache(self.c, s, self.sigma)
        p1_pad = M.sample_p1_full_cached_segments(cache, tp2, [sd[1] for sd in seeds], pads)
        p1, p2 = self._drop_padding(p1_pad, cols, pads), self._drop_padding(p2_pad, cols, pads)
        perturbed = M.concat_columns_of(targets) - ((left * p1) + (right * p2))
        z_hat = perturbed.gauss_samp_gq_arb_base_segments(self.c, self.sigma, [sd[2] for sd in seeds], cols)
        re_z = td.re * z_hat
        out = M(params, p1_rows + p2_rows, sum(cols), p1.level, True)
        out.add_rows_from(0, p1, re_z)
        out.add_rows_from(p1_rows, p2, z_hat)
        return out.split_columns(cols)

    def preimage_many_abi(self, params, td: GpuDCRTTrapdoor, public_matrix, targets, _seeds=None) -> list:
        from . import _ffi

        targets = list(targets)
        seeds = list(_seeds) if _seeds is not None else [self._draw_seeds() for _ in targets]
        if not targets:
            return []
        d = public_matrix.row_size()
        n, k = params.ring_dimension(), params.modulus_digits()
        s = preimage_smoothing_parameter(self.base, self.sigma, d, n, k)
        cache = td.p1_covariance_cache(self.c, s, self.sigma)
        rows = td.re.row_size() + td.re.col_size()
        outs = [GpuDCRTPolyMatrix(params, rows, t.col_size(), public_matrix.level, True) for t in targets]
        flat = (_ffi.GpuRngSeed * (3 * len(seeds)))(*[x for triple in seeds for x in triple])
        raw = GpuDCRTPolyMatrix._raw_array
        st = _ffi.lib().gpupoly_trapdoor_preimage_many(td.re.raw, cache.raw, public_matrix.raw, params.base_bits(),
                                                       raw(targets), len(targets), flat, raw(outs))
        if st != 0:
            msg = _ffi.last_error_string()
            if "unsupported" in msg:
                return [self.preimage(params, td, public_matrix, t, _seeds=sd) for t, sd in zip(targets, seeds)]
            raise _ffi.GpuPolyError(f"gpupoly_trapdoor_preimage_many failed: {msg}")
        return outs

    keyed_calls = 0

    def preimage_many_keys(self, params, keys, key_of, targets, _seeds=None) -> list:
        from . import _ffi

        keys, key_of, targets = list(keys), [int(k) for k in key_of], list(targets)
        assert len(key_of) == len(targets), "one key index per target"
        seeds = list(_seeds) if _seeds is not None else [self._draw_seeds() for _ in targets]
        if not targets:
            return []
        assert keys and all(0 <= k < len(keys) for k in key_of), "key_of must index keys"
        n, k_digits = params.ring_dimension(), params.modulus_digits()
        caches = []
        for td, a in keys:
            s = preimage_smoothing_parameter(self.base, self.sigma, a.row_size(), n, k_digits)
            caches.append(td.p1_covariance_cache(self.c, s, self.sigma))
        outs = [GpuDCRTPolyMatrix(params, keys[k][0].re.row_size() + keys[k][0].re.col_size(), t.col_size(), keys[k][1].level, True)
                for k, t in zip(key_of, targets)]
        flat = (_ffi.GpuRngSeed * (3 * len(seeds)))(*[x for triple in seeds for x in triple])
        raw = GpuDCRTPolyMatrix._raw_array
        type(self).keyed_calls += 1
        st = _ffi.lib().gpupoly_trapdoor_preimage_keyed(raw([td.re for td, _ in keys]), raw(caches), raw([a for _, a in keys]), len(keys),
                                                        params.base_bits(), (_ffi.C.c_uint32 * len(key_of))(*key_of), raw(targets),
                                                        len(targets), flat, raw(outs))
        if st != 0:
            msg = _ffi.last_error_string()
            if "unsupported" not in msg:
                raise _ffi.GpuPolyError(f"gpupoly_trapdoor_preimage_keyed failed: {msg}")
            for k, (td, a) in enumerate(keys):
                mine = [j for j, kk in enumerate(key_of) if kk == k]
                for j, x in zip(mine, self.preimage_many_abi(params, td, a, [targets[j] for j in mine], _seeds=[seeds[j] for j in mine])):
                    outs[j] = x
        return outs

    def preimage_batched_sharded(self, requests):
        import os
        from concurrent.futures import ThreadPoolExecutor

        groups: dict = {}
        for pos, req in enumerate(requests):
            groups.setdefault(req[1].ctx_raw().value, []).append((pos, req))
        results = [None] * len(requests)

        def run(items):
            drawn = {pos: self._draw_seeds() for pos, _ in items}
            by_key: dict = {}
            for pos, (idx, p, td, a, t) in items:
                by_key.setdefault((id(td), id(a)), []).append((pos, idx, p, td, a, t))
            groups_ = list(by_key.values())
            if len(groups_) > 1 and os.environ.get("MXX_PREIMAGE_MIXED", "") == "abi":
                p = groups_[0][0][2]
                members = [m for g in groups_ for m in g]
                key_of = [k for k, g in enumerate(groups_) for _ in g]
                outs = self.preimage_many_keys(p, [(g[0][3], g[0][4]) for g in groups_], key_of, [m[5] for m in members],
                                               _seeds=[drawn[m[0]] for m in members])
                for (pos, idx, *_), x in zip(members, outs):
                    results[pos] = (idx, x)
                return
            nworkers = min(preimage_workers(), len(groups_))
            if nworkers <= 1:
                for members in groups_:
                    _, _, p, td, a, _ = members[0]
                    outs = self.preimage_many(p, td, a, [m[5] for m in members], _seeds=[drawn[m[0]] for m in members])
                    for (pos, idx, *_), x in zip(members, outs):
                        results[pos] = (idx, x)
                return
            plan = []
            for g_i, members in enumerate(groups_):
                w = g_i % nworkers
                _, _, p, td, a, _ = members[0]
                if w == 0:
                    plan.append((w, members, p, td, a, [m[5] for m in members]))
                else:
                    pw = worker_params(p, w)
                    tdw, aw = td.replica_for(pw, a)
                    plan.append((w, members, pw, tdw, aw, [m[5].to_params(pw) for m in members]))
            outs_by_group = [self.preimage_many(pw, tdw, aw, targets, _seeds=[drawn[m[0]] for m in members])
                             for _, members, pw, tdw, aw, targets in plan]
            for (w, members, *_), outs in zip(plan, outs_by_group):
                p = members[0][2]
                for (pos, idx, *_), x in zip(members, outs):
                    results[pos] = (idx, x if w == 0 else x.to_params(p))

        if len(groups) <= 1:
            for items in groups.values():
                run(items)
            return results
        with ThreadPoolExecutor(max_workers=len(groups)) as pool:
            for f in [pool.submit(run, items) for items in groups.values()]:
                f.result()
        return results

    def preimage_column_sharded(self, comm, shards):
        from concurrent.futures import ThreadPoolExecutor

        assert len(shards) == len(comm), "one shard per context of the communicator"

        def run(item):
            p, td, a, t = item
            if t.col_size() == 0:
                k = p.modulus_digits()
                return GpuDCRTPolyMatrix(p, a.row_size() * (k + 2), 0, p.crt_depth() - 1, True)
            return self.preimage(p, td, a, t)

        if len(shards) == 1:
            blocks = [run(shards[0])]
        else:
            with ThreadPoolExecutor(max_workers=len(shards)) as pool:
                blocks = list(pool.map(run, shards))
        return comm.all_gather_columns(blocks)
```

Before: 7.810 million.

## Fuse preimage matmuls with addends and cache G-sampler tower tables

Adds a second addend, with an optional negation, to the matmul-sum kernel epilogue. The trapdoor preimage paths use it to fuse target minus (left*p1 + right*p2) and p1 + re*z into single mul_sum calls, which removes temporaries and separate elementwise add/sub passes. The per-call GPU tower kernel and its allocation are replaced by a host-computed, device-cached table keyed on base bits and c. The p1 sampler now accepts Eval-format tp2, so the clone and INTT round-trip can be skipped. The new paths add extra validation and an LRU-like cache bounded by kGqTowerTables.

```diff
diff --git a/include/gpupoly.h b/include/gpupoly.h
--- a/include/gpupoly.h
+++ b/include/gpupoly.h
@@ -295,6 +295,8 @@
                                 const uint64_t *shifts, size_t n, int negate);
 int gpupoly_matrix_mul_sum(GpuMatrix *out, size_t dst_col, size_t cols, const GpuMatrix *addend,
                            const GpuMatrix *const *lhss, const GpuMatrix *const *rhss, size_t n, int negate);
+int gpupoly_matrix_mul_sum2(GpuMatrix *out, size_t dst_col, size_t cols, const GpuMatrix *addend, const GpuMatrix *addend2,
+                            int negate2, const GpuMatrix *const *lhss, const GpuMatrix *const *rhss, size_t n, int negate);
 int gpupoly_matrix_mul_acc(GpuMatrix *out, const GpuMatrix *lhs, const GpuMatrix *rhs, int negate);
 int gpupoly_matrix_mul_gadget(GpuMatrix *out, size_t dst_col, const GpuMatrix *lhs, const GpuMatrix *scalar_1x1,
                               size_t gadget_col, size_t cols, const GpuMatrix *addend, int negate, uint32_t base_bits,
diff --git a/mxx_amd/_ffi.py b/mxx_amd/_ffi.py
--- a/mxx_amd/_ffi.py
+++ b/mxx_amd/_ffi.py
@@ -204,6 +204,7 @@
     "gpupoly_matrix_mul_monomial": (C.c_int, [_vp, _vp, C.c_uint64]),
     "gpupoly_matrix_monomial_sum": (C.c_int, [_vp, _vp, C.POINTER(C.c_void_p), C.POINTER(C.c_uint64), _sz, C.c_int]),
     "gpupoly_matrix_mul_sum": (C.c_int, [_vp, _sz, _sz, _vp, C.POINTER(C.c_void_p), C.POINTER(C.c_void_p), _sz, C.c_int]),
+    "gpupoly_matrix_mul_sum2": (C.c_int, [_vp, _sz, _sz, _vp, _vp, C.c_int, C.POINTER(C.c_void_p), C.POINTER(C.c_void_p), _sz, C.c_int]),
     "gpupoly_matrix_mul_acc": (C.c_int, [_vp, _vp, _vp, C.c_int]),
     "gpupoly_matrix_mul_gadget": (C.c_int, [_vp, _sz, _vp, _vp, _sz, _sz, _vp, C.c_int, C.c_uint32, C.c_int]),
     "gpupoly_matrix_gadget_mul": (C.c_int, [_vp, _vp, _vp, C.c_int, C.c_uint32, C.c_int]),
diff --git a/mxx_amd/csrc/common.h b/mxx_amd/csrc/common.h
--- a/mxx_amd/csrc/common.h
+++ b/mxx_amd/csrc/common.h
@@ -9,6 +9,7 @@
 #include <exception>
 #include <map>
 #include <unordered_map>
+#include <utility>
 #include <mutex>
 #include <string>
 #include <vector>
@@ -107,6 +108,7 @@
     std::map<uint32_t, void *> gadget_weights;
     std::map<std::vector<uint64_t>, void *> gadget_const_tables;
     std::map<std::vector<uint64_t>, void *> nested_rns_tables;
+    std::map<std::pair<uint32_t, uint64_t>, void *> gq_towers;
 };
 
 struct LayoutTag {
diff --git a/mxx_amd/csrc/matmul_sum.hip b/mxx_amd/csrc/matmul_sum.hip
--- a/mxx_amd/csrc/matmul_sum.hip
+++ b/mxx_amd/csrc/matmul_sum.hip
@@ -19,7 +19,8 @@
 template <typename W, int TR, int TC, int SV, bool NTB>
 __global__ void __launch_bounds__(256)
     matmul_sum_kernel(MulSumArgs args, uint32_t terms, W *out, const W *addend, const LimbConst *__restrict__ limbs, uint32_t rows,
-                      uint32_t cols, uint32_t out_cols, uint32_t dst_col, uint32_t L, uint32_t N, uint32_t row_tiles, int negate) {
+                      uint32_t cols, uint32_t out_cols, uint32_t dst_col, uint32_t L, uint32_t N, uint32_t row_tiles, int negate,
+                      const W *addend2, int negate2) {
     const uint32_t limb = blockIdx.z;
     const uint32_t ct = blockIdx.y / row_tiles, rt = blockIdx.y - ct * row_tiles;
     const uint32_t r0 = rt * TR, c0 = ct * TC;
@@ -74,6 +75,12 @@
                 *reinterpret_cast<VT *>(ad) = *reinterpret_cast<const VT *>(addend + off);
 #pragma unroll
                 for (int s = 0; s < SV; ++s) o[s] = add_mod<W>(ad[s], o[s], q);
+            }
+            if (addend2) {
+                W ad[SV];
+                *reinterpret_cast<VT *>(ad) = *reinterpret_cast<const VT *>(addend2 + off);
+#pragma unroll
+                for (int s = 0; s < SV; ++s) o[s] = negate2 ? sub_mod<W>(o[s], ad[s], q) : add_mod<W>(o[s], ad[s], q);
             }
             *reinterpret_cast<VT *>(out + off) = *reinterpret_cast<const VT *>(o);
         }
@@ -113,31 +120,38 @@
 
 template <typename W, int TR, int TC, int SV>
 int launch_sum_cfg(GpuContext *ctx, const MulSumArgs &args, uint32_t terms, size_t b_bytes, void *out, const void *addend,
-                   const SumBlock &blk, int negate) {
+                   const SumBlock &blk, int negate, const void *addend2, int negate2) {
     const uint32_t N = static_cast<uint32_t>(ctx->N);
     const TileGrid g = tile_grid<TR, TC, SV>(ctx, blk.rows, blk.cols, blk.L, b_bytes);
     W *o = static_cast<W *>(out);
-    const W *ad = static_cast<const W *>(addend);
+    const W *ad = static_cast<const W *>(addend), *ad2 = static_cast<const W *>(addend2);
+    auto label = [](bool nt_) {
+        return std::string("matmul_sum_kernel<") + (sizeof(W) == 4 ? "u32," : "u64,") + std::to_string(TR) + "," + std::to_string(TC) + "," +
+               std::to_string(SV) + (nt_ ? ",nt" : "") + "> (term-table register tile rows x cols x slots per lane, addends in the epilogue" +
+               (nt_ ? ", B streamed once with non-temporal loads" : "") + ")";
+    };
+    static const std::string name[2] = {label(false), label(true)};
     bool streamed = false;
     if constexpr (sizeof(W) == 4) {
         if (g.streamed) {
             streamed = true;
             MXX_LAUNCH((matmul_sum_kernel<W, TR, TC, SV, true>), g.grid, dim3(g.threads), 0, ctx->stream, args, terms, o, ad, ctx->d_limbs,
-                       blk.rows, blk.cols, blk.out_cols, blk.dst_col, blk.L, N, g.row_tiles, negate);
+                       blk.rows, blk.cols, blk.out_cols, blk.dst_col, blk.L, N, g.row_tiles, negate, ad2, negate2);
         }
     }
     if (!streamed)
         MXX_LAUNCH((matmul_sum_kernel<W, TR, TC, SV, false>), g.grid, dim3(g.threads), 0, ctx->stream, args, terms, o, ad, ctx->d_limbs,
-                   blk.rows, blk.cols, blk.out_cols, blk.dst_col, blk.L, N, g.row_tiles, negate);
+                   blk.rows, blk.cols, blk.out_cols, blk.dst_col, blk.L, N, g.row_tiles, negate, ad2, negate2);
+    ctx->last_kernel = name[streamed ? 1 : 0].c_str();
     HIP_TRY(hipGetLastError());
     return 0;
 }
 
 int launch_sum(GpuContext *ctx, const MulSumArgs &args, uint32_t terms, size_t b_bytes, void *out, const void *addend, const SumBlock &blk,
-               int negate) {
+               int negate, const void *addend2 = nullptr, int negate2 = 0) {
     return dispatch_stacked_tile(ctx, stacked_tile(ctx, blk.rows, blk.cols, blk.L), [&](auto cfg) {
         typedef decltype(cfg) T;
-        return launch_sum_cfg<typename T::W, T::TR, T::TC, T::SV>(ctx, args, terms, b_bytes, out, addend, blk, negate);
+        return launch_sum_cfg<typename T::W, T::TR, T::TC, T::SV>(ctx, args, terms, b_bytes, out, addend, blk, negate, addend2, negate2);
     });
 }
 
@@ -160,7 +174,7 @@
 }
 
 int mul_sum_impl(const char *who, GpuMatrix *out, size_t dst_col, size_t cols, const GpuMatrix *addend, const GpuMatrix *const *lhss,
-                 const GpuMatrix *const *rhss, size_t n, int negate) {
+                 const GpuMatrix *const *rhss, size_t n, int negate, const GpuMatrix *addend2 = nullptr, int negate2 = 0) {
     auto refuse = [&](const std::string &what) { return set_error(std::string(who) + ": " + what); };
     if (!out) return refuse("null output");
     if (n > 0 && (!lhss || !rhss)) return refuse("null array");
@@ -174,6 +188,7 @@
         return 0;
     };
     if (addend && same_ring(addend, " (addend)")) return 1;
+    if (addend2 && same_ring(addend2, " (second addend)")) return 1;
     for (size_t t = 0; t < n; ++t) {
         const std::string at = " (term " + std::to_string(t) + ")";
         if (same_ring(lhss[t], at) || same_ring(rhss[t], at)) return 1;
@@ -184,12 +199,15 @@
             return refuse("shape mismatch (term " + std::to_string(t) + ")");
     if (addend && (addend->rows != out->rows || addend->cols != out->cols)) return refuse("addend shape mismatch");
     if (addend && addend->format != GPU_POLY_FORMAT_EVAL) return refuse("requires Eval format (addend)");
+    if (addend2 && (addend2->rows != out->rows || addend2->cols != out->cols)) return refuse("second addend shape mismatch");
+    if (addend2 && addend2->format != GPU_POLY_FORMAT_EVAL) return refuse("requires Eval format (second addend)");
     for (size_t t = 0; t < n; ++t)
         if (lhss[t]->format != GPU_POLY_FORMAT_EVAL || rhss[t]->format != GPU_POLY_FORMAT_EVAL)
             return refuse("requires Eval format (term " + std::to_string(t) + ")");
     const bool whole = dst_col == 0 && cols == out->cols;
     if (!whole && out->format != GPU_POLY_FORMAT_EVAL) return refuse("a partial column block needs an output already in Eval format");
     if (addend && partial_overlap(out, addend)) return refuse("the addend overlaps the output without being the same block");
+    if (addend2 && partial_overlap(out, addend2)) return refuse("the second addend overlaps the output without being the same block");
     for (size_t t = 0; t < n; ++t)
         if (storage_overlaps(out, lhss[t]) || storage_overlaps(out, rhss[t]))
             return refuse("the output overlaps an operand (term " + std::to_string(t) + ")");
@@ -209,17 +227,24 @@
     if (ctx_activate(ctx)) return 1;
     void *const o = words_ptr(out);
     const void *src = addend ? words_ptr(addend) : nullptr;
+    const void *src2 = addend2 ? words_ptr(addend2) : nullptr;
     std::vector<const void *> a(n), b(n);
     for (size_t t = 0; t < n; ++t) {
         a[t] = words_ptr(lhss[t]);
         b[t] = words_ptr(rhss[t]);
     }
-    if (n == 0 && src == o) return 0;
+    if (n == 0 && src == o && !src2) return 0;
     const SumBlock blk{static_cast<uint32_t>(out->rows), static_cast<uint32_t>(cols), static_cast<uint32_t>(out->cols), static_cast<uint32_t>(dst_col),
                        static_cast<uint32_t>(L)};
     const double block_bytes = static_cast<double>(out->rows) * cols * L * ctx->N * ctx->word_bytes;
 
     if (out->rows > 8 && any_inner && ctx->env.mul_sum_path != 't') {
+        if (src2) {
+            MXX_TRACE_BYTES(block_bytes * (src ? 3 : 2));
+            const int rc0 = launch_sum(ctx, MulSumArgs{}, 0, 0, o, src, blk, 0, src2, negate2);
+            if (rc0) return rc0;
+            src = o;
+        }
         GpuMatrix *tmp = nullptr;
         int rc = gpu_matrix_create(ctx, level, out->rows, cols, GPU_POLY_FORMAT_EVAL, &tmp);
         for (size_t t = 0; !rc && t < n; ++t) {
@@ -236,7 +261,7 @@
     do {
         MulSumArgs args = {};
         const uint32_t terms = static_cast<uint32_t>(std::min(kMulSumMax, n - t0));
-        double bytes = block_bytes * (src ? 2 : 1);
+        double bytes = block_bytes * (1 + (src ? 1 : 0) + (src2 ? 1 : 0));
         size_t b_bytes = 0;
         for (uint32_t t = 0; t < terms; ++t) {
             args.item[t].a = a[t0 + t];
@@ -246,9 +271,10 @@
             b_bytes += rhss[t0 + t]->bytes;
         }
         MXX_TRACE_BYTES(bytes);
-        const int rc = launch_sum(ctx, args, terms, b_bytes, o, src, blk, negate);
+        const int rc = launch_sum(ctx, args, terms, b_bytes, o, src, blk, negate, src2, negate2);
         if (rc) return rc;
         src = o;
+        src2 = nullptr;
         t0 += terms;
     } while (t0 < n);
     return 0;
@@ -263,6 +289,13 @@
     ABI_GUARD_END
 }
 
+extern "C" int gpupoly_matrix_mul_sum2(GpuMatrix *out, size_t dst_col, size_t cols, const GpuMatrix *addend, const GpuMatrix *addend2,
+                                       int negate2, const GpuMatrix *const *lhss, const GpuMatrix *const *rhss, size_t n, int negate) {
+    ABI_GUARD_BEGIN
+    return mul_sum_impl("gpupoly_matrix_mul_sum2", out, dst_col, cols, addend, lhss, rhss, n, negate, addend2, negate2);
+    ABI_GUARD_END
+}
+
 extern "C" int gpupoly_matrix_mul_acc(GpuMatrix *out, const GpuMatrix *lhs, const GpuMatrix *rhs, int negate) {
     ABI_GUARD_BEGIN
     if (!out || !lhs || !rhs) return set_error("gpupoly_matrix_mul_acc: null matrix");
diff --git a/mxx_amd/csrc/runtime.hip b/mxx_amd/csrc/runtime.hip
--- a/mxx_amd/csrc/runtime.hip
+++ b/mxx_amd/csrc/runtime.hip
@@ -487,6 +487,7 @@
     for (auto &kv : ctx->gadget_weights) (void)hipFree(kv.second);
     for (auto &kv : ctx->gadget_const_tables) (void)hipFree(kv.second);
     for (auto &kv : ctx->nested_rns_tables) (void)hipFree(kv.second);
+    for (auto &kv : ctx->gq_towers) (void)hipFree(kv.second);
     if (ctx->timer_start) (void)hipEventDestroy(ctx->timer_start);
     if (ctx->timer_stop) (void)hipEventDestroy(ctx->timer_stop);
     for (hipEvent_t ev : ctx->marks)
diff --git a/mxx_amd/csrc/trapdoor.hip b/mxx_amd/csrc/trapdoor.hip
--- a/mxx_amd/csrc/trapdoor.hip
+++ b/mxx_amd/csrc/trapdoor.hip
@@ -4,6 +4,7 @@
 
 #include <algorithm>
 #include <cstdlib>
+#include <cstring>
 
 static constexpr uint64_t kTagGadget = 0x6761646765746731ull;
 static constexpr uint64_t kTagP1 = 0x7065727475726231ull;
@@ -133,14 +134,10 @@
     double cvec[4];
 };
 
-__global__ void gq_tower_kernel(GqTower *__restrict__ towers, const LimbConst *__restrict__ limbs, uint32_t L,
-                                uint32_t dpt, uint32_t base_bits, double c) {
-    const uint32_t t = blockIdx.x * blockDim.x + threadIdx.x;
-    if (t >= L) return;
+static GqTower gq_tower(uint64_t qt, uint32_t dpt, uint32_t base_bits, double c) {
     const uint64_t base = 1ull << base_bits;
     const double base_f = static_cast<double>(base);
     const double sigma = c / (base_f + 1.0);
-    const uint64_t qt = limbs[t].q;
     double c_last = 0.0;
     GqTower g;
     for (uint32_t d = 0; d < 4; ++d) g.cvec[d] = 0.0;
@@ -151,7 +148,38 @@
     g.c_last = c_last;
     g.sd = sigma / c_last;
     g.div = karney_divisor(g.sd);
-    towers[t] = g;
+    return g;
+}
+
+constexpr size_t kGqTowerTables = 16;
+
+static int gq_tower_table(GpuContext *ctx, uint32_t dpt, uint32_t base_bits, double c, const GqTower **out) {
+    uint64_t c_bits;
+    static_assert(sizeof(c_bits) == sizeof(c), "double as a key");
+    memcpy(&c_bits, &c, sizeof(c));
+    const std::pair<uint32_t, uint64_t> key(base_bits, c_bits);
+    std::lock_guard<std::mutex> lock(ctx->mutex);
+    auto it = ctx->gq_towers.find(key);
+    if (it != ctx->gq_towers.end()) {
+        *out = static_cast<const GqTower *>(it->second);
+        return 0;
+    }
+    if (ctx->gq_towers.size() >= kGqTowerTables) {
+        (void)hipFree(ctx->gq_towers.begin()->second);
+        ctx->gq_towers.erase(ctx->gq_towers.begin());
+    }
+    std::vector<GqTower> host(static_cast<size_t>(ctx->limb_count));
+    for (int l = 0; l < ctx->limb_count; ++l) host[l] = gq_tower(ctx->moduli[l], dpt, base_bits, c);
+    void *dev = nullptr;
+    HIP_TRY(hipMalloc(&dev, host.size() * sizeof(GqTower)));
+    const hipError_t e = hipMemcpy(dev, host.data(), host.size() * sizeof(GqTower), hipMemcpyHostToDevice);
+    if (e != hipSuccess) {
+        (void)hipFree(dev);
+        return set_error(e, "G-sampler tower table upload");
+    }
+    ctx->gq_towers.emplace(key, dev);
+    *out = static_cast<const GqTower *>(dev);
+    return 0;
 }
 
 struct GqPertConsts {
@@ -398,15 +426,13 @@
                                    uint32_t dpt, uint32_t base_bits, double c, size_t k, GpuRngSeed seed,
                                    const RngSegments *segs = nullptr) {
     if ((total >> ctx->logN) >> 32 || k >> 32) return set_error("gpu_matrix_gauss_samp_gq_arb_base: matrix too large");
-    CtxBlock stage(ctx), a_buf(ctx), towers(ctx);
-    if (towers.alloc(static_cast<size_t>(L) * sizeof(GqTower)) || a_buf.alloc(total * 8 * sizeof(uint64_t)) ||
-        stage.alloc(total * dpt * sizeof(int64_t)))
-        return 1;
+    const GqTower *d_towers = nullptr;
+    if (gq_tower_table(ctx, dpt, base_bits, c, &d_towers)) return 1;
+    CtxBlock stage(ctx), a_buf(ctx);
+    if (a_buf.alloc(total * 8 * sizeof(uint64_t)) || stage.alloc(total * dpt * sizeof(int64_t))) return 1;
     double *a_words = static_cast<double *>(a_buf.ptr);
     uint64_t *left_words = static_cast<uint64_t *>(a_buf.ptr) + total * dpt;
     const ChaChaKey key = chacha_subkey(seed, 0, kTagGadget);
-    MXX_LAUNCH(gq_tower_kernel, dim3(1), dim3(64), 0, ctx->stream, static_cast<GqTower *>(towers.ptr), ctx->d_limbs,
-                       L, dpt, base_bits, c);
     MXX_TRACE_BYTES(static_cast<double>(total) * (sizeof(W) + 8.0 * (8 - dpt)));
     if (segs)
         MXX_LAUNCH((gauss_samp_prep_kernel<W, MAXD, true>), item_grid(total, 256), dim3(256), 0,
@@ -422,7 +448,6 @@
     const double sigma = c / (static_cast<double>(1ull << base_bits) + 1.0);
     MXX_TRACE_BYTES(static_cast<double>(total) * (8.0 * (8 - dpt) + 8.0 * dpt));
     int64_t *digits = static_cast<int64_t *>(stage.ptr);
-    const GqTower *d_towers = static_cast<const GqTower *>(towers.ptr);
     const KarneyDivisor div = karney_divisor(sigma);
     if (segs)
         MXX_LAUNCH_LANES(plan, ctx->stream, (gauss_samp_lanes_kernel<W, MAXD, 1, true, true>),
@@ -909,14 +934,28 @@
         out->format = GPU_POLY_FORMAT_EVAL;
         return 0;
     }
-    if (tp2->format != GPU_POLY_FORMAT_COEFF)
-        return set_error("tp2 must be in Coeff format in gpu_matrix_sample_p1_full_cached");
+    if (tp2->format != GPU_POLY_FORMAT_COEFF && tp2->format != GPU_POLY_FORMAT_EVAL)
+        return set_error("tp2 must be in Coeff or Eval format in gpu_matrix_sample_p1_full_cached");
     const double denom = cache->s * cache->s - cache->sigma * cache->sigma;
     if (!(denom > 0.0)) return set_error("invalid cached Gaussian denominator");
     const double c_scale = -(cache->sigma * cache->sigma) / denom;
     if (ctx_activate(ctx)) return 1;
     const uint32_t L = static_cast<uint32_t>(matrix_limbs(out)), N = static_cast<uint32_t>(ctx->N);
     const size_t total = cols * static_cast<size_t>(N);
+    CtxBlock coeff(ctx);
+    const void *tp2_words = words_ptr(tp2);
+    if (tp2->format == GPU_POLY_FORMAT_EVAL) {
+        const size_t vectors = m * cols * L;
+        if (coeff.alloc(tp2->bytes)) return 1;
+        int rc = ctx->wide ? -1 : launch_intt_oop_u32(ctx, static_cast<uint32_t *>(coeff.ptr), static_cast<const uint32_t *>(tp2_words), vectors, L);
+        if (rc < 0) {
+            MXX_TRACED_COPY("copy (device to device)", ctx->stream, 2.0 * tp2->bytes,
+                            HIP_TRY(hipMemcpyAsync(coeff.ptr, tp2_words, tp2->bytes, hipMemcpyDeviceToDevice, ctx->stream)));
+            rc = launch_ntt(ctx, coeff.ptr, vectors, static_cast<int>(L), true);
+        }
+        if (rc) return rc;
+        tp2_words = coeff.ptr;
+    }
     if (m <= 8 && !ctx->env.p1_simple) {
         CtxBlock stage(ctx);
         if (stage.alloc(total * m * sizeof(int64_t))) return 1;
@@ -929,7 +968,7 @@
 #define P1_LANES(WT, MAXM, SEGARG, ...)                                                                                            \
     MXX_LAUNCH_LANES(plan, ctx->stream, (p1_sample_lanes_kernel<WT, MAXM, 1, __VA_ARGS__>),                                        \
                      (p1_sample_lanes_kernel<WT, MAXM, KARNEY_SERVICES, __VA_ARGS__>), static_cast<int64_t *>(stage.ptr),          \
-                     static_cast<const WT *>(words_ptr(tp2)), sqrt_var, update, kdiv, (uint32_t)m, (uint32_t)cols, L, ctx->logN,   \
+                     static_cast<const WT *>(tp2_words), sqrt_var, update, kdiv, (uint32_t)m, (uint32_t)cols, L, ctx->logN,   \
                      ctx->moduli[0], c_scale, key, total, plan.per_lane, plan.fill_every, SEGARG)
 #define LAUNCH_P1L(WT, MAXM)                                                                                                       \
     do {                                                                                                                           \
@@ -958,7 +997,7 @@
     if (m > 8 && ctx_alloc(ctx, total * m * sizeof(double), &mean_ws)) return 1;
 #define LAUNCH_P1(WT, MAXM)                                                                                       \
     MXX_LAUNCH((p1_sample_kernel<WT, MAXM>), dim3(blocks), dim3(128), 0, ctx->stream,                      \
-                       static_cast<WT *>(words_ptr(out)), static_cast<const WT *>(words_ptr(tp2)), ctx->d_limbs,             \
+                       static_cast<WT *>(words_ptr(out)), static_cast<const WT *>(tp2_words), ctx->d_limbs,             \
                        cache->sqrt_var, cache->update_coeff, (uint32_t)m, (uint32_t)cols, L, N, ctx->moduli[0],    \
                        c_scale, seed, static_cast<double *>(mean_ws))
     if (ctx->wide) {
diff --git a/mxx_amd/matrix.py b/mxx_amd/matrix.py
--- a/mxx_amd/matrix.py
+++ b/mxx_amd/matrix.py
@@ -1318,11 +1318,12 @@
         return out
 
     @staticmethod
-    def mul_sum(lhss, rhss, addend=None, negate: bool = False, out=None, dst_col: int = 0) -> "GpuDCRTPolyMatrix":
+    def mul_sum(lhss, rhss, addend=None, negate: bool = False, out=None, dst_col: int = 0, addend2=None,
+                negate2: bool = False) -> "GpuDCRTPolyMatrix":
         lhss, rhss = list(lhss), list(rhss)
         n = len(lhss)
         assert len(rhss) == n, "mul_sum: one right operand per left operand"
-        first = out if out is not None else (addend if addend is not None else (lhss[0] if n else None))
+        first = out if out is not None else (addend if addend is not None else (lhss[0] if n else addend2))
         if first is None:
             raise ValueError("mul_sum: no operand to take the shape from")
         cols = rhss[0].ncol if n else first.ncol - dst_col
@@ -1338,10 +1339,17 @@
             out._touch()
         if addend is not None:
             assert addend.is_ntt and (addend.nrow, addend.ncol) == (out.nrow, out.ncol), "mul_sum: the addend has out's shape, NTT domain"
+        if addend2 is not None:
+            assert addend2.is_ntt and (addend2.nrow, addend2.ncol) == (out.nrow, out.ncol), "mul_sum: the second addend has out's shape, NTT domain"
         larr = (C.c_void_p * max(n, 1))(*[m.raw.value for m in lhss])
         rarr = (C.c_void_p * max(n, 1))(*[m.raw.value for m in rhss])
-        st = _ffi.lib().gpupoly_matrix_mul_sum(out.raw, dst_col, cols, None if addend is None else addend.raw, larr, rarr, n, 1 if negate else 0)
-        check_status(st, "gpupoly_matrix_mul_sum")
+        if addend2 is None:
+            st = _ffi.lib().gpupoly_matrix_mul_sum(out.raw, dst_col, cols, None if addend is None else addend.raw, larr, rarr, n, 1 if negate else 0)
+            check_status(st, "gpupoly_matrix_mul_sum")
+        else:
+            st = _ffi.lib().gpupoly_matrix_mul_sum2(out.raw, dst_col, cols, None if addend is None else addend.raw, addend2.raw,
+                                                    1 if negate2 else 0, larr, rarr, n, 1 if negate else 0)
+            check_status(st, "gpupoly_matrix_mul_sum2")
         out.is_ntt = True
         return out
 
@@ -1919,11 +1927,12 @@
         return GpuP1CovarianceCache(raw, a_mat.params)
 
     @staticmethod
-    def sample_p1_full_cached(cache: GpuP1CovarianceCache, tp2, seed: GpuRngSeed) -> "GpuDCRTPolyMatrix":
+    def sample_p1_full_cached(cache: GpuP1CovarianceCache, tp2, seed: GpuRngSeed, keep_eval: bool = False) -> "GpuDCRTPolyMatrix":
         out = GpuDCRTPolyMatrix.new_empty(tp2.params, tp2.nrow, tp2.ncol)
         if tp2.nrow == 0 or tp2.ncol == 0:
             return out
-        tp2.intt_all_in_place()
+        if not (keep_eval and tp2.is_ntt):
+            tp2.intt_all_in_place()
         check_status(_ffi.lib().gpu_matrix_sample_p1_full_cached(cache.raw, tp2.raw, seed, out.raw), "gpu_matrix_sample_p1_full_cached")
         return out
 
diff --git a/mxx_amd/trapdoor.py b/mxx_amd/trapdoor.py
--- a/mxx_amd/trapdoor.py
+++ b/mxx_amd/trapdoor.py
@@ -229,15 +229,15 @@
         if stacked is not None and _traffic_bound(params, dk * padded):
             t = stacked * p2
             re_rows = td.re.row_size()
-            tp2 = t.slice(0, re_rows, 0, padded)
-            tp2_eval = t.row_view(0, re_rows)
+            tp2 = tp2_eval = t.row_view(0, re_rows)
             rp2 = t.row_view(re_rows, t.row_size())
         else:
             tp2 = td.re * p2
             if _traffic_bound(params, dk * padded):
-                tp2_eval = tp2.clone()
+                tp2_eval = tp2
         cache = td.p1_covariance_cache(c, s, dgg_stddev)
-        p1 = GpuDCRTPolyMatrix.sample_p1_full_cached(cache, tp2, seeds[1] if seeds is not None else random_gpu_rng_seed())
+        p1 = GpuDCRTPolyMatrix.sample_p1_full_cached(cache, tp2, seeds[1] if seeds is not None else random_gpu_rng_seed(),
+                                                     keep_eval=tp2_eval is not None)
         return p1, p2, tp2_eval, rp2
 
     def preimage(self, params, td: GpuDCRTTrapdoor, public_matrix, target, _seeds=None) -> GpuDCRTPolyMatrix:
@@ -253,23 +253,26 @@
         p1, p2, tp2, rp2 = self._sample_pert_parts(params, td, s, self.c, self.sigma, dgg_large_std, target_cols, stacked, _seeds)
         seed_z = _seeds[2] if _seeds is not None else None
         assert (p1.row_size(), p2.row_size()) == (p1_rows, p2_rows)
-        p_hat_image = (left * p1) + (rp2 if rp2 is not None else right * p2)
-        if p_hat_image.col_size() != target_cols:
-            p_hat_image = p_hat_image.slice_columns(0, target_cols)
-        perturbed = target - p_hat_image
-        out = GpuDCRTPolyMatrix(params, p1_rows + p2_rows, target_cols, p1.level, p1.is_ntt)
+        M = GpuDCRTPolyMatrix
+        if p1.col_size() != target_cols:
+            p_hat_image = (left * p1) + (rp2 if rp2 is not None else right * p2)
+            perturbed = target - p_hat_image.slice_columns(0, target_cols)
+        elif rp2 is not None:
+            perturbed = M.mul_sum([left], [p1], addend=target, negate=True, addend2=rp2, negate2=True)
+        else:
+            perturbed = M.mul_sum([left, right], [p1, p2], addend=target, negate=True)
+        out = M(params, p1_rows + p2_rows, target_cols, p1.level, p1.is_ntt)
         if p1.col_size() == target_cols and tp2 is not None:
             z = perturbed.gauss_samp_gq_arb_base(self.c, self.sigma, seed_z if seed_z is not None else random_gpu_rng_seed(), coeff_out=True)
             out.ntt_add_rows_from(p1_rows, z, p2, consume=True)
-            re_x = td.re * out.row_view(p1_rows, p1_rows + p2_rows)
-            out.add_rows_from(0, p1 - tp2, re_x)
+            M.mul_sum([td.re], [out.row_view(p1_rows, p1_rows + p2_rows)], addend=p1, out=out.row_view(0, p1_rows), addend2=tp2, negate2=True)
             return out
         z_hat = perturbed.gauss_samp_gq_arb_base(self.c, self.sigma, seed_z if seed_z is not None else random_gpu_rng_seed())
-        re_z = td.re * z_hat
         if p1.col_size() == target_cols:
-            out.add_rows_from(0, p1, re_z)
+            M.mul_sum([td.re], [z_hat], addend=p1, out=out.row_view(0, p1_rows))
             out.add_rows_from(p1_rows, p2, z_hat)
             return out
+        re_z = td.re * z_hat
         out.copy_block_from(p1, 0, 0, 0, 0, p1_rows, target_cols)
         out.copy_block_from(p2, p1_rows, 0, 0, 0, p2_rows, target_cols)
         out.add_block_from(re_z, 0, 0, 0, 0, re_z.row_size(), target_cols)
@@ -394,11 +397,10 @@
         cache = td.p1_covariance_cache(self.c, s, self.sigma)
         p1_pad = M.sample_p1_full_cached_segments(cache, tp2, [sd[1] for sd in seeds], pads)
         p1, p2 = self._drop_padding(p1_pad, cols, pads), self._drop_padding(p2_pad, cols, pads)
-        perturbed = M.concat_columns_of(targets) - ((left * p1) + (right * p2))
+        perturbed = M.mul_sum([left, right], [p1, p2], addend=M.concat_columns_of(targets), negate=True)
         z_hat = perturbed.gauss_samp_gq_arb_base_segments(self.c, self.sigma, [sd[2] for sd in seeds], cols)
-        re_z = td.re * z_hat
         out = M(params, p1_rows + p2_rows, sum(cols), p1.level, True)
-        out.add_rows_from(0, p1, re_z)
+        M.mul_sum([td.re], [z_hat], addend=p1, out=out.row_view(0, p1_rows))
         out.add_rows_from(p1_rows, p2, z_hat)
         return out.split_columns(cols)
 
```

Measured after the change: 7.794 million. Within noise of the previous version (-0.2%).
